# twitu/genome-assembly

Hardware: NVIDIA B200
Metric: canonical k-mers binned+pruned per second (higher is better)
Workload: dtype u64

## Files before the change

### genome-assembly_b200/binding.py

```python
from __future__ import annotations

import ctypes as C
import os
from dataclasses import dataclass

import numpy as np

_HERE = os.path.dirname(os.path.abspath(__file__))
LIB_PATH = os.path.join(_HERE, "libgbin.so")

GBIN_OK = 0
GBIN_E_INVALID_CONFIG = -1
GBIN_E_CUDA = -2
GBIN_E_NOMEM = -3
GBIN_E_NON_ACGT = -4
GBIN_E_STATE = -5
GBIN_E_TOO_LARGE = -6
GBIN_E_INVALID_ARG = -7
GBIN_E_IO = -8


class GbinError(RuntimeError):
    def __init__(self, code: int, msg: str):
        super().__init__(f"gbin error {code}: {msg}")
        self.code = code


class Config(C.Structure):
    _fields_ = [("kmer_size", C.c_int32), ("mmer_size", C.c_int32), ("abundance_cutoff", C.c_int32), ("device", C.c_int32)]


class CTable(C.Structure):
    _fields_ = [("kmer_size", C.c_int32), ("mmer_size", C.c_int32), ("abundance_cutoff", C.c_int32), ("kmer_words", C.c_int32),
                ("on_device", C.c_int32), ("ctx_owned", C.c_int32),
                ("n_instances", C.c_uint64), ("n_distinct", C.c_uint64), ("n_buckets", C.c_uint64), ("n_kmers", C.c_uint64),
                ("n_ids", C.c_uint64),
                ("mmer_codes", C.c_void_p), ("mmer_kmer_off", C.c_void_p), ("kmer_codes", C.c_void_p),
                ("kmer_id_off", C.c_void_p), ("read_ids", C.c_void_p)]


class CExpanded(C.Structure):
    _fields_ = [("kmer_size", C.c_int32), ("on_device", C.c_int32), ("n_lists", C.c_uint64), ("n_ids", C.c_uint64),
                ("list_off", C.c_void_p), ("ids", C.c_void_p)]


class CReads(C.Structure):
    _fields_ = [("data", C.c_void_p), ("data_bytes", C.c_uint64), ("n_reads", C.c_uint64), ("stride", C.c_uint64),
                ("read_len", C.c_uint32), ("id_base", C.c_int32), ("starts", C.c_void_p), ("lens", C.c_void_p),
                ("read_ids", C.c_void_p), ("max_read_len", C.c_uint32), ("reserved", C.c_uint32)]


class Timings(C.Structure):
    _fields_ = [("h2d_ms", C.c_float), ("scan_ms", C.c_float), ("sort_ms", C.c_float), ("group_ms", C.c_float),
                ("d2h_ms", C.c_float), ("total_ms", C.c_float), ("kernel_launches", C.c_uint32), ("sort_passes", C.c_uint32)]

    def as_dict(self):
        return {n: getattr(self, n) for n, _ in self._fields_}


class KernelProfile(C.Structure):
    _fields_ = [("ms", C.c_float * 12), ("launches", C.c_uint32 * 12)]


EXPORTS = [
    "gbin_strerror", "gbin_last_error", "gbin_version", "gbin_create", "gbin_destroy", "gbin_get_config",
    "gbin_bin_reads_host", "gbin_table_clone", "gbin_table_free", "gbin_pinned_alloc", "gbin_pinned_free",
    "gbin_bin_reads_device", "gbin_table_to_host", "gbin_table_to_pinned", "gbin_get_timings", "gbin_record_bytes",
    "gbin_set_kernel_profiling", "gbin_get_kernel_profile", "gbin_kernel_kind_name", "gbin_max_read_len", "gbin_multi_create", "gbin_multi_destroy", "gbin_multi_devices", "gbin_multi_context", "gbin_multi_last_error", "gbin_multi_bin_reads_host", "gbin_table_digest", "gbin_set_pipeline", "gbin_set_tuning", "gbin_donate_scratch", "gbin_get_pipeline_info", "gbin_get_run_stats",
    "gbin_count_instances_device", "gbin_scan_reads_device", "gbin_partition_records_device",
    "gbin_group_records_device", "gbin_owner_of", "gbin_xchg_create", "gbin_xchg_attach", "gbin_xchg_exchange_skr", "gbin_xchg_detach", "gbin_xchg_destroy", "gbin_skr_record_bytes", "gbin_scan_skr_device", "gbin_partition_skr_device", "gbin_group_skr_device",
    "gbin_split_reads_device", "gbin_copy_to_host", "gbin_bin_file_host", "gbin_read_file_fgets", "gbin_table_dump", "gbin_table_dump_reference_format", "gbin_table_dump_expanded_format",
    "gbin_expand_read_ids_device", "gbin_expanded_to_host", "gbin_expanded_free", "gbin_table_dump_expanded_lists",
    "getval", "getbp", "getscore", "process_read", "prune_data", "gbin_ref_configure", "gbin_ref_last_status",
    "gbin_ref_reset", "gbin_table_to_zhash", "gbin_zhash_release",
]

_lib = None


def load_library() -> C.CDLL:
    global _lib
    if _lib is not None:
        return _lib
    if not os.path.exists(LIB_PATH):
        raise ImportError(f"{LIB_PATH} is missing: build it with `make -C genome-assembly_b200` "
                          "(there is no CPU or PyTorch fallback for the binning path)")
    L = C.CDLL(LIB_PATH)
    vp, u64, u32, i32 = C.c_void_p, C.c_uint64, C.c_uint32, C.c_int32
    L.gbin_strerror.restype = C.c_char_p
    L.gbin_strerror.argtypes = [C.c_int]
    L.gbin_last_error.restype = C.c_char_p
    L.gbin_last_error.argtypes = [vp]
    L.gbin_create.argtypes = [C.POINTER(Config), C.POINTER(vp)]
    L.gbin_destroy.argtypes = [vp]
    L.gbin_destroy.restype = None
    L.gbin_get_config.argtypes = [vp, C.POINTER(Config)]
    L.gbin_bin_reads_host.argtypes = [vp, C.POINTER(CReads), C.POINTER(CTable)]
    L.gbin_bin_reads_device.argtypes = [vp, C.POINTER(CReads), vp, C.POINTER(CTable)]
    L.gbin_table_to_host.argtypes = [vp, C.POINTER(CTable), C.POINTER(CTable)]
    L.gbin_table_to_pinned.argtypes = [vp, C.POINTER(CTable), vp, C.POINTER(CTable)]
    L.gbin_table_clone.argtypes = [C.POINTER(CTable), C.POINTER(CTable)]
    L.gbin_table_free.argtypes = [C.POINTER(CTable)]
    L.gbin_table_free.restype = None
    L.gbin_pinned_alloc.argtypes = [C.c_size_t]
    L.gbin_pinned_alloc.restype = vp
    L.gbin_pinned_free.argtypes = [vp]
    L.gbin_pinned_free.restype = None
    L.gbin_get_timings.argtypes = [vp, C.POINTER(Timings)]
    L.gbin_get_run_stats.argtypes = [vp, C.POINTER(u64 * 6)]
    L.gbin_set_pipeline.argtypes = [vp, C.c_int]
    L.gbin_table_digest.argtypes = [vp, C.POINTER(CTable), vp, C.POINTER(u64)]
    L.gbin_set_tuning.argtypes = [vp, C.c_char_p, C.c_int]
    L.gbin_donate_scratch.argtypes = [vp, vp, C.c_uint64]
    L.gbin_get_pipeline_info.argtypes = [vp, C.POINTER(C.c_int), C.POINTER(C.c_int), C.POINTER(C.c_uint32)]
    L.gbin_set_kernel_profiling.argtypes = [vp, C.c_int]
    L.gbin_get_kernel_profile.argtypes = [vp, C.POINTER(KernelProfile)]
    L.gbin_kernel_kind_name.argtypes = [C.c_int]
    L.gbin_kernel_kind_name.restype = C.c_char_p
    L.gbin_record_bytes.argtypes = [vp]
    L.gbin_record_bytes.restype = u32
    L.gbin_max_read_len.restype = u32
    L.gbin_max_read_len.argtypes = []
    L.gbin_count_instances_device.argtypes = [vp, C.POINTER(CReads), vp, C.POINTER(u64)]
    L.gbin_scan_reads_device.argtypes = [vp, C.POINTER(CReads), u32, vp, u64, vp, C.POINTER(u64)]
    L.gbin_partition_records_device.argtypes = [vp, vp, u64, u32, vp, vp, C.POINTER(u64)]
    L.gbin_group_records_device.argtypes = [vp, vp, u64, vp, i32, vp, C.POINTER(CTable)]
    L.gbin_skr_record_bytes.argtypes = [vp]
    L.gbin_skr_record_bytes.restype = u32
    L.gbin_scan_skr_device.argtypes = [vp, C.POINTER(CReads), u32, vp, u64, vp, C.POINTER(u64), C.POINTER(u64)]
    L.gbin_partition_skr_device.argtypes = [vp, vp, u64, u32, vp, vp, C.POINTER(u64)]
    L.gbin_group_skr_device.argtypes = [vp, vp, u64, vp, i32, vp, C.POINTER(CTable), C.POINTER(C.c_int)]
    L.gbin_owner_of.argtypes = [u32, u32]
    L.gbin_owner_of.restype = u32
    L.gbin_xchg_create.argtypes = [vp, u32, u32, u64, vp]
    L.gbin_xchg_attach.argtypes = [vp, vp]
    L.gbin_xchg_exchange_skr.argtypes = [vp, vp, u64, vp, C.POINTER(vp), C.POINTER(u64), C.POINTER(u64)]
    L.gbin_xchg_destroy.argtypes = [vp]
    L.gbin_xchg_destroy.restype = None
    L.gbin_xchg_detach.argtypes = [vp]
    L.gbin_xchg_detach.restype = None
    L.gbin_split_reads_device.argtypes = [vp, vp, u64, C.c_int, vp, C.POINTER(CReads)]
    L.gbin_copy_to_host.argtypes = [vp, vp, vp, u64]
    L.gbin_bin_file_host.argtypes = [vp, C.c_char_p, C.c_int, C.POINTER(CTable)]
    L.gbin_read_file_fgets.argtypes = [C.c_char_p, C.c_int, C.POINTER(vp), C.POINTER(u64), C.POINTER(vp), C.POINTER(vp),
                                       C.POINTER(u64)]
    L.gbin_table_dump.argtypes = [C.POINTER(CTable), C.c_char_p]
    L.gbin_table_dump_reference_format.argtypes = [C.POINTER(CTable), C.c_char_p]
    L.gbin_table_dump_expanded_format.argtypes = [C.POINTER(CTable), C.c_char_p]
    L.gbin_expand_read_ids_device.argtypes = [C.c_void_p, C.POINTER(CTable), C.c_void_p, C.POINTER(CExpanded)]
    L.gbin_expanded_to_host.argtypes = [C.c_void_p, C.POINTER(CExpanded), C.POINTER(CExpanded)]
    L.gbin_expanded_free.argtypes = [C.POINTER(CExpanded)]
    L.gbin_expanded_free.restype = None
    L.gbin_table_dump_expanded_lists.argtypes = [C.POINTER(CTable), C.POINTER(CExpanded), C.c_char_p]
    L.getval.argtypes = [C.c_char]
    L.getval.restype = C.c_int
    L.getbp.argtypes = [C.c_int]
    L.getbp.restype = C.c_char
    L.getscore.argtypes = [C.c_char_p]
    L.getscore.restype = C.c_int
    L.process_read.argtypes = [vp, C.c_char_p, C.c_int]
    L.process_read.restype = vp
    L.prune_data.argtypes = [vp]
    L.prune_data.restype = vp
    L.gbin_ref_configure.argtypes = [C.c_int, C.c_int, C.c_int, C.c_int]
    L.gbin_ref_last_status.restype = C.c_int
    L.gbin_ref_reset.argtypes = [vp]
    L.gbin_ref_reset.restype = None
    L.gbin_table_to_zhash.argtypes = [C.POINTER(CTable), vp]
    L.gbin_zhash_release.argtypes = [vp]
    L.gbin_zhash_release.restype = None
    _lib = L
    return L


@dataclass
class HostTable:
    K: int
    M: int
    cutoff: int
    kw: int
    n_instances: int
    n_distinct: int
    mmer_codes: np.ndarray
    mmer_kmer_off: np.ndarray
    kmer_codes: np.ndarray
    kmer_id_off: np.ndarray
    read_ids: np.ndarray

    @property
    def n_buckets(self):
        return len(self.mmer_codes)

    @property
    def n_kmers(self):
        return len(self.kmer_id_off) - 1

    @property
    def n_ids(self):
        return len(self.read_ids)


def _np_from(ptr, n, dtype):
    if n == 0 or not ptr:
        return np.zeros(0, dtype=dtype)
    buf = (C.c_char * (n * np.dtype(dtype).itemsize)).from_address(ptr)
    return np.frombuffer(buf, dtype=dtype, count=n).copy()


def host_table_from_c(t: CTable) -> HostTable:
    assert not t.on_device
    return HostTable(K=t.kmer_size, M=t.mmer_size, cutoff=t.abundance_cutoff, kw=t.kmer_words,
                     n_instances=int(t.n_instances), n_distinct=int(t.n_distinct),
                     mmer_codes=_np_from(t.mmer_codes, t.n_buckets, np.uint32),
                     mmer_kmer_off=_np_from(t.mmer_kmer_off, t.n_buckets + 1, np.uint64),
                     kmer_codes=_np_from(t.kmer_codes, t.n_kmers * t.kmer_words, np.uint64),
                     kmer_id_off=_np_from(t.kmer_id_off, t.n_kmers + 1, np.uint64),
                     read_ids=_np_from(t.read_ids, t.n_ids, np.int32))


def owner_of(mmer_codes, parts: int) -> np.ndarray:
    m = np.asarray(mmer_codes).astype(np.uint64)
    return ((((m * np.uint64(0x9E3779B1)) & np.uint64(0xFFFFFFFF)) * np.uint64(parts)) >> np.uint64(32)).astype(np.int64)


CUDA_STREAM_LEGACY = 1


def stream_handle(torch_stream) -> int:
    h = int(torch_stream.cuda_stream)
    return h if h else CUDA_STREAM_LEGACY


def _ptr(x):
    if x is None:
        return None
    if isinstance(x, int):
        return x
    if isinstance(x, np.ndarray):
        return x.ctypes.data
    if hasattr(x, "data_ptr"):
        return x.data_ptr()
    raise TypeError(type(x))


class Binner:

    def __init__(self, k: int = 31, m: int = 4, cutoff: int = 1, device: int = 0, pipeline: int | None = None):
        self.lib = load_library()
        self.cfg = Config(k, m, cutoff, device)
        h = C.c_void_p()
        rc = self.lib.gbin_create(C.byref(self.cfg), C.byref(h))
        if rc != GBIN_OK:
            raise GbinError(rc, self.lib.gbin_strerror(rc).decode())
        self.h = h
        self.k, self.m, self.cutoff, self.device = k, m, cutoff, device
        if pipeline is not None:
            self.set_pipeline(pipeline)

    def close(self):
        if getattr(self, "h", None):
            self.lib.gbin_destroy(self.h)
            self.h = None

    def __del__(self):
        try:
            self.close()
        except Exception:
            pass

    def _check(self, rc):
        if rc != GBIN_OK:
            raise GbinError(rc, f"{self.lib.gbin_strerror(rc).decode()}: {self.lib.gbin_last_error(self.h).decode()}")

    @property
    def record_bytes(self) -> int:
        return int(self.lib.gbin_record_bytes(self.h))

    def timings(self) -> dict:
        t = Timings()
        self.lib.gbin_get_timings(self.h, C.byref(t))
        return t.as_dict()

    def set_pipeline(self, pipeline: int):
        self._check(self.lib.gbin_set_pipeline(self.h, pipeline))

    def table_digest(self, table: CTable, stream=None) -> int:
        d = C.c_uint64()
        self._check(self.lib.gbin_table_digest(self.h, C.byref(table), stream, C.byref(d)))
        return int(d.value)

    def expand_read_ids_device(self, dev_table: CTable, stream=None) -> CExpanded:
        x = CExpanded()
        self._check(self.lib.gbin_expand_read_ids_device(self.h, C.byref(dev_table), stream, C.byref(x)))
        return x

    def expanded_to_host(self, dev: CExpanded) -> CExpanded:
        h = CExpanded()
        self._check(self.lib.gbin_expanded_to_host(self.h, C.byref(dev), C.byref(h)))
        return h

    def donate_scratch(self, d_buf, nbytes: int):
        self._check(self.lib.gbin_donate_scratch(self.h, _ptr(d_buf), int(nbytes)))

    def set_tuning(self, name: str, value: int):
        self._check(self.lib.gbin_set_tuning(self.h, name.encode(), int(value)))

    def pipeline_info(self) -> dict:
        a, b, c = C.c_int(), C.c_int(), C.c_uint32()
        self._check(self.lib.gbin_get_pipeline_info(self.h, C.byref(a), C.byref(b), C.byref(c)))
        return {"configured": a.value, "last_used": b.value, "fallbacks": c.value}

    def run_stats(self) -> dict:
        a = (C.c_uint64 * 6)()
        self._check(self.lib.gbin_get_run_stats(self.h, C.byref(a)))
        return {"n_super_kmers": int(a[0]), "n_mmer_runs": int(a[1]), "n_units": int(a[2]), "n_lsd_kmers": int(a[3]),
                "key_nc": int(a[4]) & 0xffffffff, "key_h": int(a[4]) >> 32, "n_passes": int(a[5]) & 0xffffffff}

    def set_kernel_profiling(self, enable: bool):
        self._check(self.lib.gbin_set_kernel_profiling(self.h, int(enable)))

    def kernel_profile(self) -> dict:
        p = KernelProfile()
        self._check(self.lib.gbin_get_kernel_profile(self.h, C.byref(p)))
        out = {}
        for i in range(12):
            name = self.lib.gbin_kernel_kind_name(i).decode()
            if name:
                out[name] = {"ms": float(p.ms[i]), "launches": int(p.launches[i])}
        return out

    @staticmethod
    def _reads(data, data_bytes, n_reads, stride=0, read_len=0, starts=None, lens=None, read_ids=None, id_base=0, max_read_len=0):
        return CReads(_ptr(data), data_bytes, n_reads, stride, read_len, id_base, _ptr(starts), _ptr(lens), _ptr(read_ids),
                      max_read_len, 0)

    def bin_host_raw(self, reads: CReads) -> CTable:
        t = CTable()
        self._check(self.lib.gbin_bin_reads_host(self.h, C.byref(reads), C.byref(t)))
        return t

    def bin_host(self, data, n_reads, *, stride=0, read_len=0, starts=None, lens=None, read_ids=None, id_base=0) -> HostTable:
        if isinstance(data, (bytes, bytearray)):
            data = np.frombuffer(data, dtype=np.uint8)
        data = np.ascontiguousarray(data, dtype=np.uint8)
        keep = [data]
        if starts is not None:
            starts = np.ascontiguousarray(starts, dtype=np.uint64)
            lens = np.ascontiguousarray(lens, dtype=np.uint32)
            keep += [starts, lens]
        if read_ids is not None:
            read_ids = np.ascontiguousarray(read_ids, dtype=np.int32)
            keep.append(read_ids)
        rd = self._reads(data, data.size, n_reads, stride, read_len, starts, lens, read_ids, id_base)
        return host_table_from_c(self.bin_host_raw(rd))

    def bin_device_raw(self, reads: CReads, stream: int | None = None) -> CTable:
        t = CTable()
        self._check(self.lib.gbin_bin_reads_device(self.h, C.byref(reads), stream, C.byref(t)))
        return t

    def table_to_host(self, dev: CTable) -> HostTable:
        h = CTable()
        self._check(self.lib.gbin_table_to_host(self.h, C.byref(dev), C.byref(h)))
        try:
            return host_table_from_c(h)
        finally:
            self.lib.gbin_table_free(C.byref(h))

    def table_to_pinned_raw(self, dev: CTable, stream=None) -> CTable:
        h = CTable()
        self._check(self.lib.gbin_table_to_pinned(self.h, C.byref(dev), stream, C.byref(h)))
        return h

    def split_reads_device(self, d_data, data_bytes: int, read_length_define: int, stream=None) -> CReads:
        rd = CReads()
        self._check(self.lib.gbin_split_reads_device(self.h, _ptr(d_data), data_bytes, read_length_define, stream, C.byref(rd)))
        return rd

    def device_array(self, dev_ptr, n: int, dtype) -> np.ndarray:
        out = np.zeros(n, dtype=dtype)
        if n:
            self._check(self.lib.gbin_copy_to_host(self.h, out.ctypes.data, int(dev_ptr), out.nbytes))
        return out

    def bin_file_host(self, path: str, read_length_define: int) -> HostTable:
        t = CTable()
        self._check(self.lib.gbin_bin_file_host(self.h, path.encode(), read_length_define, C.byref(t)))
        return host_table_from_c(t)

    def count_instances_device(self, reads: CReads, stream=None) -> int:
        n = C.c_uint64()
        self._check(self.lib.gbin_count_instances_device(self.h, C.byref(reads), stream, C.byref(n)))
        return int(n.value)

    def scan_device(self, reads: CReads, arrival_base: int, d_records, capacity: int, stream=None) -> int:
        n = C.c_uint64()
        self._check(self.lib.gbin_scan_reads_device(self.h, C.byref(reads), arrival_base, _ptr(d_records), capacity, stream, C.byref(n)))
        return int(n.value)

    def partition_device(self, d_records, n: int, n_parts: int, d_out, stream=None) -> list[int]:
        counts = (C.c_uint64 * n_parts)()
        self._check(self.lib.gbin_partition_records_device(self.h, _ptr(d_records), n, n_parts, _ptr(d_out), stream, counts))
        return [int(c) for c in counts]

    @property
    def skr_record_bytes(self) -> int:
        return int(self.lib.gbin_skr_record_bytes(self.h))

    def scan_skr_device(self, reads: CReads, arrival_base: int, d_skr, capacity: int, stream=None):
        n, ni = C.c_uint64(), C.c_uint64()
        self._check(self.lib.gbin_scan_skr_device(self.h, C.byref(reads), arrival_base, _ptr(d_skr), capacity, stream, C.byref(n), C.byref(ni)))
        return int(n.value), int(ni.value)

    def partition_skr_device(self, d_skr, n: int, n_parts: int, d_out, stream=None) -> list[int]:
        counts = (C.c_uint64 * n_parts)()
        self._check(self.lib.gbin_partition_skr_device(self.h, _ptr(d_skr), n, n_parts, _ptr(d_out), stream, counts))
        return [int(c) for c in counts]

    def group_skr_device(self, d_skr, n_skr: int, d_ids_by_arrival=None, id_base: int = 0, stream=None) -> CTable:
        t = CTable()
        fb = C.c_int()
        self._check(self.lib.gbin_group_skr_device(self.h, _ptr(d_skr), n_skr, _ptr(d_ids_by_arrival), id_base, stream, C.byref(t), C.byref(fb)))
        return t

    XCHG_HANDLE_BYTES = 192

    def xchg_create(self, rank: int, world: int, capacity_records: int) -> bytes:
        buf = C.create_string_buffer(self.XCHG_HANDLE_BYTES)
        self._check(self.lib.gbin_xchg_create(self.h, rank, world, capacity_records, buf))
        return buf.raw

    def xchg_attach(self, all_handles: bytes):
        self._check(self.lib.gbin_xchg_attach(self.h, C.c_char_p(all_handles)))

    def xchg_exchange_skr(self, d_skr, n: int, world: int, stream=None):
        recv, n_in = C.c_void_p(), C.c_uint64()
        sent = (C.c_uint64 * 16)()
        self._check(self.lib.gbin_xchg_exchange_skr(self.h, _ptr(d_skr), n, stream, C.byref(recv), C.byref(n_in), sent))
        return int(recv.value or 0), int(n_in.value), [int(sent[i]) for i in range(world)]

    def xchg_detach(self):
        self.lib.gbin_xchg_detach(self.h)

    def xchg_destroy(self):
        self.lib.gbin_xchg_destroy(self.h)

    def group_device(self, d_records, n: int, d_ids_by_arrival=None, id_base: int = 0, stream=None) -> CTable:
        t = CTable()
        self._check(self.lib.gbin_group_records_device(self.h, _ptr(d_records), n, _ptr(d_ids_by_arrival), id_base, stream, C.byref(t)))
        return t


def read_file_fgets(path: str, read_length_define: int):
    L = load_library()
    data, starts, lens = C.c_void_p(), C.c_void_p(), C.c_void_p()
    nbytes, n = C.c_uint64(), C.c_uint64()
    rc = L.gbin_read_file_fgets(path.encode(), read_length_define, C.byref(data), C.byref(nbytes), C.byref(starts), C.byref(lens),
                                C.byref(n))
    if rc != GBIN_OK:
        raise GbinError(rc, L.gbin_strerror(rc).decode())
    libc = C.CDLL(None)
    libc.free.argtypes = [C.c_void_p]
    try:
        return (_np_from(data.value, nbytes.value, np.uint8), _np_from(starts.value, n.value, np.uint64),
                _np_from(lens.value, n.value, np.uint32))
    finally:
        for p in (data, starts, lens):
            libc.free(p)
```

### genome-assembly_b200/csrc/bin3.cu

```cuda
#include "bin3.cuh"
#include "gbin_device.cuh"
#include "gbin_internal.h"
#include "prefix_scan.cuh"

namespace gbin {


__device__ __forceinline__ uint32_t payload_bases(const uint32_t *pl, uint32_t nwords, uint32_t j, uint32_t h, bool rev) {
    const uint32_t bit = 2 * j, wi = bit >> 5, sh = bit & 31;
    const uint32_t a = wi < nwords ? pl[wi] : 0u, b = wi + 1 < nwords ? pl[wi + 1] : 0u;
    uint32_t x = __funnelshift_l(b, a, sh);
    if (rev) x = ~x;
    return h ? (x >> (32 - 2 * h)) : 0u;
}

template <int PW>
__global__ void __launch_bounds__(256)
    make_entries_kernel(const uint32_t *__restrict__ skr, uint64_t n_rec, KeyLayout kl, uint64_t *__restrict__ ent, uint16_t *__restrict__ piece_info,
                        unsigned long long *__restrict__ n_real) {
    constexpr int NW = SkrLayout<PW>::WORDS;
    const uint64_t i = (uint64_t)blockIdx.x * blockDim.x + threadIdx.x;
    uint32_t real = 0;
    if (i < n_rec) {
        const uint4 h = *reinterpret_cast<const uint4 *>(skr + i * NW);
// ... 43 lines not shown
    else make_entries_kernel<4><<<grid, 256, 0, st>>>(static_cast<const uint32_t *>(skr), n_rec, kl, ent, piece_info, n_real_dev);
    return 1;
}


struct EntCountAndHead {
    const uint64_t *ent;
    const uint16_t *info;
    __device__ __forceinline__ uint64_t operator()(uint64_t i) const {
        const uint64_t e = ent[i];
        const uint64_t head = (i == 0 || (e >> 32) != (ent[i - 1] >> 32)) ? 1ull : 0ull;
        return (uint64_t)(info[i] & 0xffu) | (head << 32);
    }
};

struct EntRunSink {
    const uint64_t *ent;
    uint32_t *inst_prefix, *run_start;
    __device__ __forceinline__ void operator()(uint64_t i, uint64_t b) const {
        inst_prefix[i] = (uint32_t)b;
        if (i == 0 || (ent[i] >> 32) != (ent[i - 1] >> 32)) run_start[b >> 32] = (uint32_t)i;
    }
};

__global__ void v3_run_totals_kernel(const uint64_t *__restrict__ total, uint64_t n, uint32_t *__restrict__ inst_prefix, uint32_t *__restrict__ run_start,
                                     uint32_t *__restrict__ n_inst_out, uint32_t *__restrict__ n_runs_out) {
    const uint64_t t = *total;
    inst_prefix[n] = (uint32_t)t;
    run_start[t >> 32] = (uint32_t)n;
    *n_inst_out = (uint32_t)t;
    *n_runs_out = (uint32_t)(t >> 32);
}

int v3_plan_runs(const uint64_t *ent, const uint16_t *sorted_info, uint64_t n_ent, uint32_t *inst_prefix, uint64_t *both64, uint32_t *run_start,
                 uint64_t *scratch64, uint32_t *n_inst_dev, uint32_t *n_runs_dev, cudaStream_t st) {
    if (n_ent == 0) {
        cudaMemsetAsync(n_inst_dev, 0, 4, st);
        cudaMemsetAsync(n_runs_dev, 0, 4, st);
        return 0;
    }
    int l = exclusive_scan_to<uint64_t, EntCountAndHead, EntRunSink>(EntCountAndHead{ent, sorted_info}, EntRunSink{ent, inst_prefix, run_start}, n_ent, scratch64,
                                                                     both64, st);
    v3_run_totals_kernel<<<1, 1, 0, st>>>(both64, n_ent, inst_prefix, run_start, n_inst_dev, n_runs_dev);
    return l + 1;
}

constexpr int PLAN_BLOCK = 64;
struct Plan3 {
    uint32_t cap, nb_max, ecap, max_rounds;
    uint32_t cap_s, nb_s, ecap_s;
};
struct RunView3 {
    const uint32_t *run_start;
    const uint32_t *inst_prefix;
    __device__ __forceinline__ uint32_t size(uint64_t r) const { return inst_prefix[run_start[r + 1]] - inst_prefix[run_start[r]]; }
};
__host__ __device__ inline uint32_t rounds_of(uint32_t c, const Plan3 &pp) {
    uint32_t r = 2 * ((c + pp.cap - 1) / pp.cap) + 1;
    return r < pp.max_rounds ? r : pp.max_rounds;
}

__global__ void v3_atoms_kernel(RunView3 rv, const uint64_t *__restrict__ ent, uint64_t n_runs, int mshift, uint32_t *__restrict__ atom_c,
                                uint32_t *__restrict__ atom_e, uint32_t *__restrict__ atom_mm) {
    const uint64_t r = (uint64_t)blockIdx.x * blockDim.x + threadIdx.x;
    if (r >= n_runs) return;
    const uint32_t a = rv.run_start[r], b = rv.run_start[r + 1];
    atom_c[r] = rv.inst_prefix[b] - rv.inst_prefix[a];
    atom_e[r] = b - a;
    atom_mm[r] = (uint32_t)(ent[a] >> 32) >> mshift;
}

constexpr uint64_t ATOM_ROUNDS = 1ull << 32;
constexpr uint32_t SPAN_MEMBER = 0xfffffffeu;
constexpr uint32_t SPAN_MEMBER_LONG = 0xffffffffu;
constexpr uint32_t SPAN_SHORT_MAX = 17;
__global__ void __launch_bounds__(128)
    v3_pack_kernel(const uint32_t *__restrict__ atom_c, const uint32_t *__restrict__ atom_e, const uint32_t *__restrict__ atom_mm, uint64_t n_runs, Plan3 pp,
                   uint64_t *__restrict__ nunits, uint32_t *__restrict__ spanlen) {
    const uint64_t t = (uint64_t)blockIdx.x * blockDim.x + threadIdx.x;
    uint64_t r = t * PLAN_BLOCK;
    const uint64_t stop = r + PLAN_BLOCK < n_runs ? r + PLAN_BLOCK : n_runs;
    if (r >= n_runs) return;
    if (r > 0)
        while (r < n_runs && atom_mm[r] == atom_mm[r - 1]) r++;
    uint32_t cur_c = 0, cur_e = 0, cur_b = 0;
    while (r < stop) {
        const uint32_t mm = atom_mm[r];
        uint64_t q = r;
        uint64_t cb = 0, eb = 0;
        do {
            cb += atom_c[q];
            eb += atom_e[q];
            q++;
        } while (q < n_runs && atom_mm[q] == mm);
        if (cb <= pp.cap && eb <= pp.ecap) {
            if (cb > pp.cap_s || eb > pp.ecap_s) {
                nunits[r] = 1ull;
                cur_b = 0;
            } else if (cur_b == 0 || cur_c + cb > pp.cap_s || cur_e + eb > pp.ecap_s || cur_b + 1 > pp.nb_s) {
                nunits[r] = 1ull;
                cur_c = (uint32_t)cb;
                cur_e = (uint32_t)eb;
                cur_b = 1;
            } else {
                nunits[r] = 0ull;
                cur_c += (uint32_t)cb;
                cur_e += (uint32_t)eb;
                cur_b++;
            }
            spanlen[r] = 0;
            for (uint64_t a = r + 1; a < q; a++) {
                nunits[a] = 0ull;
                spanlen[a] = 0;
            }
        } else {
            cur_b = 0;
            uint32_t L = 0, sc = 0, se = 0;
            bool open = false;
            for (uint64_t a = r; a < q; a++) {
                const uint32_t c = atom_c[a], e = atom_e[a];
                if (c > pp.cap) {
                    const uint32_t R = rounds_of(c, pp);
                    nunits[a] = (uint64_t)R | ATOM_ROUNDS;
                    L += R;
                    open = false;
                } else if (!open || sc + c > pp.cap || se + e > pp.ecap) {
                    nunits[a] = 1ull;
                    L++;
                    sc = c;
                    se = e;
                    open = true;
                } else {
                    nunits[a] = 0ull;
                    sc += c;
                    se += e;
                }
                spanlen[a] = SPAN_MEMBER;
            }
            spanlen[r] = L;
            if (L > SPAN_SHORT_MAX)
                for (uint64_t a = r + 1; a < q; a++) spanlen[a] = SPAN_MEMBER_LONG;
        }
        r = q;
    }
}

struct G3Counters {
    unsigned long long distinct;
    unsigned long long total_kmers, total_ids;
    unsigned int overflow;
    unsigned int n_units, n_spans;
    unsigned int pad;
    unsigned long long lsd_kmers, lsd_ids;
};

__global__ void v3_head_runs_kernel(const uint64_t *__restrict__ nunits, const uint64_t *__restrict__ base, uint64_t n_runs, uint32_t *__restrict__ head_run) {
    const uint64_t r = (uint64_t)blockIdx.x * blockDim.x + threadIdx.x;
    if (r >= n_runs) return;
    const uint32_t nu = (uint32_t)nunits[r];
    const uint32_t ub = (uint32_t)base[r];
    for (uint32_t j = 0; j < nu; j++) head_run[ub + j] = (uint32_t)r;
}

__global__ void v3_fill_units_kernel(RunView3 rv, const uint64_t *__restrict__ nunits, const uint32_t *__restrict__ spanlen, const uint64_t *__restrict__ base,
                                     const uint64_t *__restrict__ totals, uint64_t n_runs, const uint32_t *__restrict__ head_run, Unit3 *__restrict__ units,
                                     G3Counters *__restrict__ gc) {
    const uint32_t n_units = (uint32_t)*totals;
    const uint32_t u = blockIdx.x * blockDim.x + threadIdx.x;
    if (u == 0) {
        gc->n_units = n_units;
        gc->n_spans = (uint32_t)(*totals >> 32);
    }
    if (u >= n_units) return;
    const uint32_t r0 = head_run[u];
    const uint64_t nu = nunits[r0];
    const uint32_t ub = (uint32_t)base[r0];
    Unit3 un;
    un.drange = 0u | (63u << 8);
    un.ent_begin = rv.run_start[r0];
    un.ibase = rv.inst_prefix[un.ent_begin];
    if (nu & ATOM_ROUNDS) {
        un.ent_end = rv.run_start[r0 + 1];
        un.n_inst = rv.inst_prefix[un.ent_end] - un.ibase;
        un.round = u - ub;
        un.rounds = (uint32_t)nu;
    } else {
        const uint32_t r1 = (u + 1 < n_units) ? head_run[u + 1] : (uint32_t)n_runs;
        un.ent_end = rv.run_start[r1];
        un.n_inst = rv.inst_prefix[un.ent_end] - un.ibase;
        un.round = 0;
        un.rounds = 0;
    }
    const uint32_t sl = spanlen[r0];
    if (sl == 0 || sl == SPAN_MEMBER || sl == SPAN_MEMBER_LONG) un.span_len = sl;
    else un.span_len = u == ub ? sl : (sl > SPAN_SHORT_MAX ? SPAN_MEMBER_LONG : SPAN_MEMBER);
    units[u] = un;
}

__global__ void __launch_bounds__(128)
    v3_round_cuts_kernel(const uint16_t *__restrict__ info, Unit3 *__restrict__ units, G3Counters *__restrict__ gc, uint32_t cap) {
    __shared__ int s_hist[4][68];
    const uint32_t lane = threadIdx.x & 31, warp = threadIdx.x >> 5;
    int *dhist = s_hist[warp];
    const uint32_t n_units = gc->n_units;
    for (uint32_t u = blockIdx.x * 4 + warp; u < n_units; u += gridDim.x * 4) {
        const Unit3 un = units[u];
        if (un.rounds == 0 || un.round != 0) continue;
        dhist[lane] = 0;
        dhist[lane + 32] = 0;
        if (lane < 4) dhist[64 + lane] = 0;
        __syncwarp();
        const uint32_t n_ent = un.ent_end - un.ent_begin;
        for (uint32_t e = lane; e < n_ent; e += 32) {
            const uint32_t pi = info[un.ent_begin + e];
            const uint32_t np = pi & 0xffu, dlo = pi >> 8;
            if (np) {
                atomicAdd(&dhist[dlo], 1);
                atomicAdd(&dhist[dlo + np], -1);
            }
        }
        __syncwarp();
        const int a = dhist[2 * lane], b = dhist[2 * lane + 1];
        int incl = a + b;
#pragma unroll
        for (int d = 1; d < 32; d <<= 1) {
            const int o = __shfl_up_sync(0xffffffffu, incl, d);
            if (lane >= (uint32_t)d) incl += o;
        }
        __syncwarp();
        dhist[2 * lane] = incl - b;
        dhist[2 * lane + 1] = incl;
        __syncwarp();
        if (lane == 0) {
            uint32_t rnd = 0, acc = 0, before = 0;
            int lo = 0;
            bool bad = false;
            auto emit = [&](int hi) {
                if (rnd < un.rounds) {
                    Unit3 &w = units[u + rnd];
                    w.drange = (uint32_t)lo | ((uint32_t)hi << 8);
                    w.ibase = un.ibase + before;
                    w.n_inst = acc;
                } else {
                    bad = true;
                }
            };
            for (int d = 0; d < 64; d++) {
                const uint32_t c = (uint32_t)dhist[d];
                if (c > cap) bad = true;
                if (acc + c > cap) {
                    emit(d - 1);
                    rnd++;
                    lo = d;
                    before += acc;
                    acc = 0;
                }
                acc += c;
            }
            emit(63);
            for (uint32_t j = rnd + 1; j < un.rounds; j++) {
                units[u + j].n_inst = 0;
                units[u + j].ibase = un.ibase + un.n_inst;
            }
            if (bad) atomicExch(&gc->overflow, 1u);
        }
        __syncwarp();
    }
}


struct UnitOut3 {
    uint32_t ibase;
    uint32_t S, N;
    uint32_t pad;
};

struct G3Stage {
    uint64_t *codes;
    uint32_t *mmer;
    uint32_t *loff;
    int32_t *ids;
    UnitOut3 *unit_out;
    uint64_t kmer_cap, id_cap;
    uint32_t kdiv;
};

template <int PW>
struct Payload {
    uint64_t w[PW];
    __device__ __forceinline__ void set(const uint4 &a, const uint4 &b) {
        w[0] = ((uint64_t)a.x << 32) | a.y;
        w[1] = ((uint64_t)a.z << 32) | a.w;
        if (PW == 4) {
            w[PW - 2] = ((uint64_t)b.x << 32) | b.y;
            w[PW - 1] = ((uint64_t)b.z << 32) | b.w;
        }
    }
    __device__ __forceinline__ void advance(uint32_t bases) {
        const uint32_t sh = 2 * bases;
#pragma unroll
        for (int q = 0; q < PW - 1; q++) w[q] = (w[q] << sh) | (w[q + 1] >> (64 - sh));
        w[PW - 1] <<= sh;
    }
    __device__ __forceinline__ void skip(uint32_t bases) {
        while (bases >= 31) {
            advance(31);
// ... 312 lines not shown
            for (int j = 0; j < U; j++) {
                const uint32_t p = b0 + j * 32 + lane;
                const bool sv = leader[j] && (cutoff < 0 || c[j] > (uint32_t)cutoff);
                const unsigned lm = __ballot_sync(0xffffffffu, leader[j]), sm = __ballot_sync(0xffffffffu, sv);
                if (sv) surv[S + __popc(sm & lt_mask)] = (uint16_t)p;
                else if (leader[j]) cnt16[p] = 0xffffu;
                S += __popc(sm);
                D += __popc(lm);
                N += sv ? c[j] : 0u;
            }
        }
#pragma unroll
        for (int d = 16; d > 0; d >>= 1) N += __shfl_xor_sync(0xffffffffu, N, d);
        const uint64_t kbase = ibase / out.kdiv;
        const bool oob = (uint64_t)ibase + N > out.id_cap || kbase + S > out.kmer_cap;
        if (lane == 0) {
            out.unit_out[u_cur] = UnitOut3{ibase, oob ? 0u : S, oob ? 0u : N, 0u};
            atomicAdd(&gc->distinct, (unsigned long long)D);
            if (oob) atomicExch(&gc->overflow, 2u);
        }
        __syncwarp();
        if (oob) {
            u = __shfl_sync(0xffffffffu, u_next, 0);
            continue;
        }

        for (uint32_t x0 = 0; x0 < S; x0 += 32) {
            const uint32_t x = x0 + lane;
            if (x < S) {
                const uint32_t p = surv[x];
                uint32_t a = 0, a2 = S;
                if (n_bkt > 1) {
                    const uint32_t o = ebk[eix[p]];
                    const uint32_t blo = bstart[o], bhi = bstart[o + 1];
                    uint32_t b = S;
                    while (a < b) {
                        const uint32_t m = (a + b) >> 1;
                        if (surv[m] < blo) a = m + 1;
                        else b = m;
                    }
                    uint32_t b2 = S;
                    a2 = a;
                    while (a2 < b2) {
                        const uint32_t m = (a2 + b2) >> 1;
                        if (surv[m] < bhi) a2 = m + 1;
                        else b2 = m;
                    }
                }
                const uint64_t k0 = key0[p], k1 = (KW == 2) ? key1[p] : 0ull;
                uint32_t rank = a;
                for (uint32_t t = a; t < a2; t++) {
                    const uint32_t q = surv[t];
                    const uint64_t q0 = key0[q];
                    bool less = q0 < k0;
                    if constexpr (KW == 2) less = less || (q0 == k0 && key1[q] < k1);
                    rank += less ? 1u : 0u;
                }
                sorted[rank] = (uint16_t)p;
            }
        }
        __syncwarp();

        {
            uint32_t carry = 0;
            for (uint32_t x0 = 0; x0 < S; x0 += 32) {
                const uint32_t x = x0 + lane;
                const uint32_t p = x < S ? sorted[x] : 0u;
                const uint32_t c = x < S ? cnt16[p] : 0u;
                const uint32_t inc = warp_incl_scan_u32(c, lane);
                if (x < S) cnt16[p] = (uint16_t)(carry + inc);
                carry += __shfl_sync(0xffffffffu, inc, 31);
            }
        }
        __syncwarp();

        for (uint32_t x0 = 0; x0 < S; x0 += 32) {
            const uint32_t x = x0 + lane;
            if (x < S) {
                const uint32_t p = sorted[x];
                const uint32_t beg = x ? cnt16[sorted[x - 1]] : 0u;
                const uint64_t g = kbase + x;
                out.codes[g * KW] = key0[p];
                if (KW == 2) out.codes[g * KW + 1] = key1[p];
                out.mmer[g] = bmm[n_bkt > 1 ? ebk[eix[p]] : 0u];
                out.loff[g] = beg;
            }
        }
        __syncwarp();

        if (N) {
            if (packed) {
                for (uint32_t b0 = 0; b0 < n_inst; b0 += 32 * U) {
                    uint32_t end[U], r[U];
                    int32_t id[U];
#pragma unroll
                    for (int j = 0; j < U; j++) {
                        const uint32_t p = b0 + j * 32 + lane;
                        end[j] = 0xffffu;
                        r[j] = 0;
                        id[j] = 0;
                        if (p < n_inst) {
                            end[j] = cnt16[grp[p]];
                            r[j] = rk[p];
                            id[j] = eid[eix[p]];
                        }
                    }
#pragma unroll
                    for (int j = 0; j < U; j++)
                        if (end[j] != 0xffffu) idbuf[end[j] - 1u - r[j]] = id[j];
                }
            } else {
                uint32_t carry_pos = 0;
                for (uint32_t e0 = 0; e0 < n_ent; e0 += 32) {
                    const uint32_t e = e0 + lane;
                    uint32_t np = 0, arrival = 0;
                    if (e < n_ent) {
                        const uint32_t slot = (uint32_t)ent[un.ent_begin + e];
                        const uint32_t *rec = skr + (uint64_t)(slot >> kl.cshift) * NW;
                        const uint32_t meta = rec[2];
                        arrival = rec[0];
                        uint32_t t0;
                        piece_of(meta, slot & cls_mask, kl, &t0, &np);
                        if (is_round && np) {
                            const int so = (int)((meta >> 16) & 0xffu);
                            int a = so - dhi, b = so - dlo;
                            if (a < (int)t0) a = (int)t0;
                            if (b > (int)(t0 + np - 1)) b = (int)(t0 + np - 1);
                            np = (dlo > dhi || b < a) ? 0u : (uint32_t)(b - a + 1);
                        }
                    }
                    const uint32_t ps = warp_incl_scan_u32(np, lane);
                    const uint32_t pos0 = carry_pos + ps - np;
                    carry_pos += __shfl_sync(0xffffffffu, ps, 31);
                    if (np) {
                        const int32_t id = ids_by_arrival ? ids_by_arrival[arrival] : id_base + (int32_t)arrival;
                        for (uint32_t i = 0; i < np; i++) {
                            const uint32_t p = pos0 + i;
                            const uint32_t end = cnt16[grp[p]];
                            if (end != 0xffffu) idbuf[end - 1u - rk[p]] = id;
                        }
                    }
                }
            }
            __syncwarp();
            int32_t *dst = out.ids + ibase;
            for (uint32_t i = lane; i < N; i += 32) dst[i] = idbuf[i];
        }
        __syncwarp();
        u = __shfl_sync(0xffffffffu, u_next, 0);
    }
}


struct UnitSN {
    const UnitOut3 *uo;
    const uint32_t *chunk_bounds;
    uint32_t chunk;
    __device__ __forceinline__ uint64_t operator()(uint64_t u) const {
        if (u < chunk_bounds[chunk] || u >= chunk_bounds[chunk + 1]) return 0ull;
        return ((uint64_t)uo[u].S << 32) | uo[u].N;
    }
};

__global__ void v3_chunk_total_kernel(const uint64_t *__restrict__ chunk_sum, uint32_t chunk, unsigned long long *__restrict__ totals, G3Counters *__restrict__ gc,
                                      uint32_t n_chunks, int which) {
    const unsigned long long t = (chunk ? totals[chunk - 1] : 0ull) + *chunk_sum;
    totals[chunk] = t;
    if (chunk + 1 == n_chunks) {
        if (which == 0) {
            gc->total_kmers = t >> 32;
            gc->total_ids = t & 0xffffffffull;
        } else {
            gc->lsd_kmers = t >> 32;
            gc->lsd_ids = t & 0xffffffffull;
        }
    }
}

struct G3Final {
    uint64_t *kmer_codes;
    uint32_t *kmer_mmer;
    uint64_t *kmer_id_off;
    int32_t *read_ids;
    uint64_t id_off_base;
};

struct G3Lsd {
    const uint64_t *excl;
    void *rec;
    uint32_t *src_off;
    uint32_t *cnt;
    uint32_t *fidx;
    uint32_t *nadj;
    uint64_t cap;
};

struct UnitSNLong {
    const UnitOut3 *uo;
    const Unit3 *units;
    const uint32_t *chunk_bounds;
    uint32_t chunk;
    __device__ __forceinline__ uint64_t operator()(uint64_t u) const {
        if (u < chunk_bounds[chunk] || u >= chunk_bounds[chunk + 1]) return 0ull;
        const uint32_t sl = units[u].span_len;
        if (sl != SPAN_MEMBER_LONG && (sl <= SPAN_SHORT_MAX || sl == SPAN_MEMBER)) return 0ull;
        return ((uint64_t)uo[u].S << 32) | uo[u].N;
    }
};

template <int KW>
__device__ __forceinline__ void finalize3_unit(const Unit3 *__restrict__ units, const uint64_t *__restrict__ unit_excl, unsigned long long base,
                                               unsigned long long lsd_base, const G3Stage &st, const G3Final &fin, const G3Lsd &ls, G3Counters *gc, uint32_t u,
                                               uint32_t lane, bool only_long) {
    const uint32_t span_len = units[u].span_len;
    if (only_long && span_len != SPAN_MEMBER_LONG && (span_len <= SPAN_SHORT_MAX || span_len == SPAN_MEMBER)) return;
    const uint64_t ex = unit_excl[u];
    const UnitOut3 uo = st.unit_out[u];
    const uint64_t Sb = (base >> 32) + (ex >> 32), Nb = (base & 0xffffffffull) + (ex & 0xffffffffull);
    if (span_len == 0) {
        const uint64_t kb = uo.ibase / st.kdiv;
        for (uint32_t x0 = 0; x0 < uo.S; x0 += 128) {
            uint64_t c0[4], c1[4];
            uint32_t mm[4], lo[4];
#pragma unroll
            for (int q = 0; q < 4; q++) {
                const uint32_t x = x0 + q * 32 + lane;
                if (x < uo.S) {
                    c0[q] = st.codes[(kb + x) * KW];
                    if (KW == 2) c1[q] = st.codes[(kb + x) * KW + 1];
                    mm[q] = st.mmer[kb + x];
                    lo[q] = st.loff[kb + x];
                }
            }
#pragma unroll
            for (int q = 0; q < 4; q++) {
                const uint32_t x = x0 + q * 32 + lane;
                if (x < uo.S) {
                    fin.kmer_codes[(Sb + x) * KW] = c0[q];
                    if (KW == 2) fin.kmer_codes[(Sb + x) * KW + 1] = c1[q];
                    fin.kmer_mmer[Sb + x] = mm[q];
                    fin.kmer_id_off[Sb + x] = fin.id_off_base + Nb + lo[q];
                }
            }
        }
        const int32_t *src = st.ids + uo.ibase;
        int32_t *dst = fin.read_ids + Nb;
        for (uint32_t i0 = 0; i0 < uo.N; i0 += 256) {
            int32_t v[8];
#pragma unroll
            for (int q = 0; q < 8; q++) {
                const uint32_t i = i0 + q * 32 + lane;
                if (i < uo.N) v[q] = __ldcs(src + i);
            }
#pragma unroll
            for (int q = 0; q < 8; q++) {
                const uint32_t i = i0 + q * 32 + lane;
                if (i < uo.N) dst[i] = v[q];
            }
        }
        return;
    }
    if (span_len == SPAN_MEMBER_LONG || (span_len > SPAN_SHORT_MAX && span_len != SPAN_MEMBER)) {
        const uint64_t lx = ls.excl[u];
        const uint64_t q0 = (lsd_base >> 32) + (lx >> 32), nq0 = (lsd_base & 0xffffffffull) + (lx & 0xffffffffull);
        if (q0 + uo.S > ls.cap) {
            if (lane == 0) atomicExch(&gc->overflow, 6u);
            return;
        }
        const uint64_t kb = uo.ibase / st.kdiv;
        Rec<KW> *rec = static_cast<Rec<KW> *>(ls.rec);
        for (uint32_t x = lane; x < uo.S; x += 32) {
            const uint64_t p = q0 + x;
            Rec<KW> r;
            r.k[0] = st.codes[(kb + x) * KW];
            if (KW == 2) r.k[KW - 1] = st.codes[(kb + x) * KW + 1];
            r.mmer = st.mmer[kb + x];
            r.arrival = (uint32_t)p;
            store_rec<KW>(rec + p, r);
            const uint32_t lo = st.loff[kb + x];
            ls.src_off[p] = uo.ibase + lo;
            ls.cnt[p] = (x + 1 < uo.S ? st.loff[kb + x + 1] : uo.N) - lo;
            ls.fidx[p] = (uint32_t)(Sb + x);
            ls.nadj[p] = (uint32_t)(Nb - nq0);
        }
        return;
    }
    uint32_t h = u;
    while (units[h].span_len == SPAN_MEMBER) h--;
    const uint32_t R = units[h].span_len;
    const uint64_t exh = unit_excl[h];
    const uint64_t Sh = (base >> 32) + (exh >> 32), Nh = (base & 0xffffffffull) + (exh & 0xffffffffull);
    if (uo.S == 0) return;
    const uint32_t j = u - h;
    const uint64_t kbj = uo.ibase / st.kdiv;
    const uint32_t mmer = st.mmer[kbj];
    for (uint32_t x0 = 0; x0 < uo.S; x0 += 32) {
        const uint32_t x = x0 + lane;
        uint32_t lo = 0, cnt = 0;
        uint64_t idoff = 0;
        if (x < uo.S) {
            const uint64_t k0 = st.codes[(kbj + x) * KW], k1 = KW == 2 ? st.codes[(kbj + x) * KW + 1] : 0ull;
            lo = st.loff[kbj + x];
            cnt = (x + 1 < uo.S ? st.loff[kbj + x + 1] : uo.N) - lo;
            uint32_t rank = x;
            idoff = lo;
            for (uint32_t j2 = 0; j2 < R; j2++) {
                if (j2 == j) continue;
                const UnitOut3 u2 = st.unit_out[h + j2];
                const uint64_t kb2 = u2.ibase / st.kdiv;
                uint32_t a = 0, b = u2.S;
                while (a < b) {
                    const uint32_t m = (a + b) >> 1;
                    const uint64_t q0 = st.codes[(kb2 + m) * KW];
                    bool less = q0 < k0;
                    if constexpr (KW == 2) less = less || (q0 == k0 && st.codes[(kb2 + m) * KW + 1] < k1);
                    if (less) a = m + 1;
                    else b = m;
                }
                rank += a;
                idoff += a < u2.S ? st.loff[kb2 + a] : u2.N;
            }
            fin.kmer_codes[(Sh + rank) * KW] = k0;
            if (KW == 2) fin.kmer_codes[(Sh + rank) * KW + 1] = k1;
            fin.kmer_mmer[Sh + rank] = mmer;
            fin.kmer_id_off[Sh + rank] = fin.id_off_base + Nh + idoff;
        }
        const uint32_t nl = min(32u, uo.S - x0);
        for (uint32_t l0 = 0; l0 < nl; l0 += 4) {
            const uint32_t l = l0 + (lane >> 3);
            const uint32_t c = __shfl_sync(0xffffffffu, cnt, l & 31);
            const uint32_t so = __shfl_sync(0xffffffffu, lo, l & 31);
            const uint64_t d = __shfl_sync(0xffffffffu, idoff, l & 31);
            if (l < nl) {
                const int32_t *src = st.ids + uo.ibase + so;
                int32_t *dst = fin.read_ids + Nh + d;
                for (uint32_t i = lane & 7u; i < c; i += 8) dst[i] = src[i];
            }
        }
    }
}

template <int KW>
__global__ void __launch_bounds__(128, 12)
    finalize3_kernel(const Unit3 *__restrict__ units, const uint64_t *__restrict__ unit_excl, const unsigned long long *__restrict__ totals,
                     const unsigned long long *__restrict__ lsd_totals, G3Stage st, G3Final fin, G3Lsd ls, G3Counters *__restrict__ gc,
                     const uint32_t *__restrict__ chunk_bounds, uint32_t chunk, bool only_long) {
    const uint32_t lane = threadIdx.x & 31;
    const uint32_t unit_begin = chunk_bounds[chunk], unit_end = chunk_bounds[chunk + 1];
    const unsigned long long base = chunk ? totals[chunk - 1] : 0ull;
    const unsigned long long lsd_base = chunk ? lsd_totals[chunk - 1] : 0ull;
    for (uint32_t u = unit_begin + blockIdx.x * 4 + (threadIdx.x >> 5); u < unit_end; u += gridDim.x * 4)
        finalize3_unit<KW>(units, unit_excl, base, lsd_base, st, fin, ls, gc, u, lane, only_long);
}

template <int KW>
struct LsdCnt {
    const Rec<KW> *rec;
    const uint32_t *cnt;
    __device__ __forceinline__ uint64_t operator()(uint64_t q) const { return cnt[rec[q].arrival]; }
};

template <int KW>
__global__ void lsd_place_kernel(const Rec<KW> *__restrict__ rec, uint64_t n, const uint64_t *__restrict__ dnew, G3Lsd ls, G3Final fin) {
    const uint64_t q = (uint64_t)blockIdx.x * blockDim.x + threadIdx.x;
    if (q >= n) return;
    const Rec<KW> r = load_rec<KW>(rec + q);
    const uint64_t f = ls.fidx[q];
    fin.kmer_codes[f * KW] = r.k[0];
    if (KW == 2) fin.kmer_codes[f * KW + 1] = r.k[KW - 1];
    fin.kmer_mmer[f] = r.mmer;
    fin.kmer_id_off[f] = fin.id_off_base + dnew[q] + ls.nadj[q];
}

template <int KW>
__global__ void __launch_bounds__(256)
    lsd_lists_kernel(const Rec<KW> *__restrict__ rec, uint64_t n, const uint64_t *__restrict__ dnew, G3Lsd ls, const int32_t *__restrict__ stg_ids, G3Final fin) {
    const uint64_t q = ((uint64_t)blockIdx.x * blockDim.x + threadIdx.x) >> 3;
    if (q >= n) return;
    const uint32_t p = rec[q].arrival;
    const uint32_t c = ls.cnt[p];
    const int32_t *src = stg_ids + ls.src_off[p];
    int32_t *dst = fin.read_ids + dnew[q] + ls.nadj[q];
    for (uint32_t i = threadIdx.x & 7u; i < c; i += 8) dst[i] = src[i];
}

__global__ void v3_chunk_bounds_kernel(const Unit3 *__restrict__ units, const G3Counters *__restrict__ gc, uint32_t n_chunks, uint32_t *__restrict__ chunk_bounds) {
    const uint32_t nu = gc->n_units;
    for (uint32_t c = 0; c <= n_chunks; c++) {
        uint32_t b = (uint32_t)(((uint64_t)nu * c) / n_chunks);
        if (c == n_chunks) b = nu;
        else {
            while (b > 0 && b < nu && (units[b].span_len == SPAN_MEMBER || units[b].span_len == SPAN_MEMBER_LONG)) b--;
        }
        chunk_bounds[c] = b;
    }
}


static bool v3_hybrid(const KeyLayout &kl, int cap_i) {
    static int on = -1;
    if (on < 0) {
        const char *e = getenv("GBIN_V3_HYBRID");
        on = e ? atoi(e) : 1;
    }
    return on && cap_i != 512 && kl.K <= 32;
}
static Plan3 v3_plan_params(const KeyLayout &kl, int cap_i) {
    const uint32_t cap = cap_i == 512 ? 512u : 1024u;
    Plan3 pp{cap, cap / 8, cap / 4, (uint32_t)(kl.K - kl.M + 1), cap, cap / 8, cap / 4};
    if (v3_hybrid(kl, cap_i)) {
        pp.cap_s = G3_SMALL_INST;
        pp.nb_s = G3_SMALL_NB;
        pp.ecap_s = G3_SMALL_ENT;
    }
    return pp;
}

uint64_t v3_max_units(uint64_t n_inst, uint64_t n_runs, int cap) {
    const uint64_t c = cap == 512 ? 512 : 1024;
    return n_runs + 5 * (n_inst / c) + 16;
}
size_t v3_unit_bytes() { return sizeof(Unit3); }
size_t v3_unit_out_bytes() { return sizeof(UnitOut3); }

struct PtrIn64 {
    const uint64_t *p;
    __device__ __forceinline__ uint64_t operator()(uint64_t j) const { return p[j]; }
};

int v3_plan_units(const uint16_t *sorted_info, const uint64_t *ent, const KeyLayout &kl, int cap, const uint32_t *inst_prefix, const uint32_t *run_start, uint64_t n_runs,
                  uint64_t *nunits64, uint64_t *base64, uint32_t *atom3, uint32_t *spanlen, uint32_t *head_run, void *scratch, void *units, uint64_t max_units,
                  void *gc_dev, uint32_t n_chunks, uint32_t *chunk_bounds, cudaStream_t st) {
    RunView3 rv{run_start, inst_prefix};
    const Plan3 pp = v3_plan_params(kl, cap);
    G3Counters *gc = static_cast<G3Counters *>(gc_dev);
    cudaMemsetAsync(gc, 0, sizeof(G3Counters), st);
    int l = 0;
    if (n_runs) {
        uint32_t *atom_c = atom3, *atom_e = atom3 + n_runs, *atom_mm = atom3 + 2 * n_runs;
        v3_atoms_kernel<<<(unsigned)((n_runs + 255) / 256), 256, 0, st>>>(rv, ent, n_runs, kl.mshift, atom_c, atom_e, atom_mm);
        const uint64_t walkers = (n_runs + PLAN_BLOCK - 1) / PLAN_BLOCK;
        v3_pack_kernel<<<(unsigned)((walkers + 127) / 128), 128, 0, st>>>(atom_c, atom_e, atom_mm, n_runs, pp, nunits64, spanlen);
        l += 2 + exclusive_scan<uint64_t, PtrIn64>(PtrIn64{nunits64}, base64, n_runs, static_cast<uint64_t *>(scratch), base64 + n_runs, st);
        v3_head_runs_kernel<<<(unsigned)((n_runs + 255) / 256), 256, 0, st>>>(nunits64, base64, n_runs, head_run);
        v3_fill_units_kernel<<<(unsigned)((max_units + 255) / 256), 256, 0, st>>>(rv, nunits64, spanlen, base64, base64 + n_runs, n_runs, head_run, static_cast<Unit3 *>(units), gc);
        v3_round_cuts_kernel<<<592, 128, 0, st>>>(sorted_info, static_cast<Unit3 *>(units), gc, pp.cap);
        l += 3;
    }
    v3_chunk_bounds_kernel<<<1, 1, 0, st>>>(static_cast<const Unit3 *>(units), gc, n_chunks, chunk_bounds);
    return l + 1;
}

size_t v3_group_smem_bytes(int KW, int cap) {
    const size_t per_warp = cap == 512 ? (KW == 1 ? WarpLayout<512, 1>::BYTES : WarpLayout<512, 2>::BYTES)
                                       : (KW == 1 ? WarpLayout<1024, 1>::BYTES : WarpLayout<1024, 2>::BYTES);
    return per_warp * G3_WARPS;
}

int v3_group_launch(const void *skr, const uint64_t *ent, const void *units, const KeyLayout &kl, int cap, int cutoff, const int32_t *ids_by_arrival, int32_t id_base,
                    const V3Out &o, uint64_t max_units, uint64_t *unit_excl, uint64_t *lsd_excl, void *scan_scratch, void *gc_dev, const V3Chunks &ch, const V3Lsd &lsd,
                    bool finalize_only, int sm_count, KernelProf *prof, cudaStream_t st) {
    const int KW = kl.K <= 32 ? 1 : 2;
    constexpr int WARPS = G3_WARPS;
    const size_t smem = v3_group_smem_bytes(KW, cap);
    cudaMemsetAsync(ch.tickets, 0, sizeof(uint32_t) * 2 * ch.n, st);
    const uint32_t kdiv = cutoff >= 0 ? (uint32_t)cutoff + 1u : 1u;
    G3Stage stg{o.stg_codes, o.stg_mmer, o.stg_loff, o.stg_ids, static_cast<UnitOut3 *>(o.unit_out), o.kmer_cap, o.id_cap, kdiv};
    G3Final fin{o.kmer_codes, o.kmer_mmer, o.kmer_id_off, o.read_ids, o.id_off_base};
    G3Lsd ls{lsd_excl, lsd.rec, lsd.src_off, lsd.cnt, lsd.fidx, lsd.nadj, lsd.cap};
    G3Counters *gc = static_cast<G3Counters *>(gc_dev);
    const uint32_t *sk = static_cast<const uint32_t *>(skr);
    const Unit3 *un = static_cast<const Unit3 *>(units);
    int per_sm = (int)((size_t)(227 * 1024) / (smem + 1024));
    if (per_sm < 1) per_sm = 1;
    const bool hybrid = v3_hybrid(kl, cap);
    const size_t smem_s = v3_group_smem_bytes(KW, 512);
    int per_sm_s = (int)((size_t)(227 * 1024) / (smem_s + 1024));
    if (per_sm_s < 1) per_sm_s = 1;
    int launches = 0;
    static int sbs = -1, l_per_sm = 2;
    if (sbs < 0) {
        const char *e = getenv("GBIN_V3_SBS");
        sbs = e ? atoi(e) : 1;
        const char *f = getenv("GBIN_V3_LPS");
        l_per_sm = f ? atoi(f) : 2;
        if (l_per_sm < 1 || l_per_sm > 2) l_per_sm = 2;
    }
    const bool side_by_side = sbs && ch.aux && ch.ev_fork && ch.ev_join;
    auto launch = [&](auto kern, auto kern_small, auto fin_kern) {
        cudaFuncSetAttribute(kern, cudaFuncAttributeMaxDynamicSharedMemorySize, (int)smem);
        if (hybrid) cudaFuncSetAttribute(kern_small, cudaFuncAttributeMaxDynamicSharedMemorySize, (int)smem_s);
        for (uint32_t c = 0; c < ch.n; c++) {
            if (!finalize_only) {
                bool on = prof && prof->begin(KK_SKR_GROUP, st);
                if (!hybrid) {
                    kern<<<sm_count * per_sm, WARPS * 32, smem, st>>>(sk, ent, un, kl, cutoff, ids_by_arrival, id_base, stg, gc, ch.bounds, c, ch.tickets, 0u);
                } else if (!side_by_side) {
                    kern<<<sm_count * per_sm, WARPS * 32, smem, st>>>(sk, ent, un, kl, cutoff, ids_by_arrival, id_base, stg, gc, ch.bounds, c, ch.tickets, 2u);
                    kern_small<<<sm_count * per_sm_s, WARPS * 32, smem_s, st>>>(sk, ent, un, kl, cutoff, ids_by_arrival, id_base, stg, gc, ch.bounds, c, ch.tickets + ch.n, 1u);
                } else {
                    cudaEventRecord(ch.ev_fork, st);
                    cudaStreamWaitEvent(ch.aux, ch.ev_fork, 0);
                    kern<<<sm_count * l_per_sm, WARPS * 32, smem, st>>>(sk, ent, un, kl, cutoff, ids_by_arrival, id_base, stg, gc, ch.bounds, c, ch.tickets, 2u);
                    kern_small<<<sm_count * per_sm_s, WARPS * 32, smem_s, ch.aux>>>(sk, ent, un, kl, cutoff, ids_by_arrival, id_base, stg, gc, ch.bounds, c, ch.tickets + ch.n, 1u);
                    cudaEventRecord(ch.ev_join, ch.aux);
                    cudaStreamWaitEvent(st, ch.ev_join, 0);
                }
                if (prof) prof->end(on, hybrid ? 2 : 1, st);
                launches += hybrid ? 2 : 1;
            }
            bool on = prof && prof->begin(KK_V3_SPAN, st);
            int l = exclusive_scan<uint64_t, UnitSN>(UnitSN{stg.unit_out, ch.bounds, c}, unit_excl, max_units, static_cast<uint64_t *>(scan_scratch), ch.chunk_sum, st);
            v3_chunk_total_kernel<<<1, 1, 0, st>>>(ch.chunk_sum, c, ch.totals_dev, gc, ch.n, 0);
            l += exclusive_scan<uint64_t, UnitSNLong>(UnitSNLong{stg.unit_out, un, ch.bounds, c}, lsd_excl, max_units, static_cast<uint64_t *>(scan_scratch), ch.chunk_sum, st);
            v3_chunk_total_kernel<<<1, 1, 0, st>>>(ch.chunk_sum, c, ch.lsd_totals_dev, gc, ch.n, 1);
            fin_kern<<<sm_count * 12, 128, 0, st>>>(un, unit_excl, ch.totals_dev, ch.lsd_totals_dev, stg, fin, ls, gc, ch.bounds, c, finalize_only);
            if (prof) prof->end(on, l + 3, st);
            launches += l + 3;
            if (ch.totals_host) {
                cudaMemcpyAsync(ch.totals_host + c, ch.totals_dev + c, sizeof(unsigned long long), cudaMemcpyDeviceToHost, st);
                cudaMemcpyAsync(ch.lsd_totals_host + c, ch.lsd_totals_dev + c, sizeof(unsigned long long), cudaMemcpyDeviceToHost, st);
            }
            if (ch.done) cudaEventRecord(ch.done[c], st);
        }
    };
    static int uu = 0;
    if (!uu) {
        const char *e = getenv("GBIN_V3_U");
        uu = e ? atoi(e) : 0;
        if (uu != 1 && uu != 2 && uu != 4) uu = -1;
    }
    const int u_sel = uu > 0 ? uu : (cap == 512 ? 2 : 4);
#define G3_LAUNCH(PW_, KW_, CAP_) \
    (u_sel == 1 ? launch(group3_kernel<PW_, KW_, CAP_, WARPS, 1>, group3_kernel<PW_, KW_, 512, WARPS, 2>, finalize3_kernel<KW_>) \
             : (u_sel == 2 ? launch(group3_kernel<PW_, KW_, CAP_, WARPS, 2>, group3_kernel<PW_, KW_, 512, WARPS, 2>, finalize3_kernel<KW_>) \
                           : launch(group3_kernel<PW_, KW_, CAP_, WARPS, 4>, group3_kernel<PW_, KW_, 512, WARPS, 2>, finalize3_kernel<KW_>)))
    if (KW == 1) {
        if (cap == 512) G3_LAUNCH(2, 1, 512);
        else G3_LAUNCH(2, 1, 1024);
    } else {
        if (cap == 512) G3_LAUNCH(4, 2, 512);
        else G3_LAUNCH(4, 2, 1024);
    }
#undef G3_LAUNCH
    return launches;
}

template <int KW>
struct RecHead {
    const Rec<KW> *rec;
    __device__ __forceinline__ uint32_t operator()(uint64_t p) const { return (p == 0 || rec[p].mmer != rec[p - 1].mmer) ? 1u : 0u; }
};
template <int KW>
__global__ void span_starts_kernel(const Rec<KW> *__restrict__ rec, uint64_t n, const uint32_t *__restrict__ idx, uint32_t *__restrict__ starts,
                                   uint32_t *__restrict__ n_spans, uint32_t *__restrict__ flag) {
    const uint64_t p = (uint64_t)blockIdx.x * blockDim.x + threadIdx.x;
    if (p >= n) return;
    const bool head = p == 0 || rec[p].mmer != rec[p - 1].mmer;
    if (head) starts[idx[p]] = (uint32_t)p;
    if (p == n - 1) {
        const uint32_t total = idx[p] + (head ? 1u : 0u);
        starts[total] = (uint32_t)n;
        *n_spans = total;
        *flag = 0u;
    }
}

constexpr int SS_RMAX = 1024;
template <int KW, int CAP, int THREADS>
__global__ void __launch_bounds__(THREADS)
    span_sort_kernel(Rec<KW> *__restrict__ rec, const uint32_t *__restrict__ starts, const uint32_t *__restrict__ n_spans_ptr, uint32_t m_min, uint32_t m_max,
                     uint32_t *__restrict__ too_big) {
    extern __shared__ __align__(16) uint8_t ss_smem[];
    uint64_t *ka = reinterpret_cast<uint64_t *>(ss_smem);
    uint64_t *kb = ka + KW * CAP;
    uint16_t *sa = reinterpret_cast<uint16_t *>(kb + KW * CAP);
    uint16_t *sb = sa + CAP;
    uint16_t *ra = sb + CAP;
    uint16_t *rb = ra + SS_RMAX + 2;
    __shared__ uint32_t s_nruns;
    const uint32_t tid = threadIdx.x, lane = tid & 31;
    const uint32_t n_spans = *n_spans_ptr;
    for (uint32_t s = blockIdx.x; s < n_spans; s += gridDim.x) {
        const uint32_t b = starts[s], m = starts[s + 1] - b;
        if (m < m_min) continue;
        if (m > m_max) continue;
        const uint32_t mmer = rec[b].mmer;
        for (uint32_t i = tid; i < m; i += THREADS) {
            const Rec<KW> r = load_rec<KW>(rec + b + i);
            ka[i] = r.k[0];
            if (KW == 2) ka[CAP + i] = r.k[KW - 1];
            sa[i] = (uint16_t)i;
        }
        __syncthreads();
        if (tid < 32) {
            uint32_t nr = 0;
            for (uint32_t i0 = 0; i0 < m; i0 += 32) {
                const uint32_t i = i0 + lane;
                bool head = false;
                if (i < m) {
                    head = i == 0 || ka[i] < ka[i - 1];
                    if (KW == 2 && i && ka[i] == ka[i - 1]) head = ka[CAP + i] < ka[CAP + i - 1];
                }
                const unsigned bal = __ballot_sync(0xffffffffu, head);
                if (head) {
                    const uint32_t pos = nr + __popc(bal & ((1u << lane) - 1u));
                    if (pos < (uint32_t)SS_RMAX) ra[pos] = (uint16_t)i;
                }
                nr += __popc(bal);
            }
            if (lane == 0) {
                s_nruns = nr;
                if (nr <= (uint32_t)SS_RMAX) ra[nr] = (uint16_t)m;
            }
        }
        __syncthreads();
        uint32_t nr = s_nruns;
        if (nr > (uint32_t)SS_RMAX) {
            if (tid == 0) atomicExch(too_big, 1u);
            __syncthreads();
            continue;
        }
        uint64_t *src_k = ka, *dst_k = kb;
        uint16_t *src_s = sa, *dst_s = sb, *src_r = ra, *dst_r = rb;
        while (nr > 1) {
            for (uint32_t i = tid; i < m; i += THREADS) {
                uint32_t lo = 0, hi = nr;
                while (hi - lo > 1) {
                    const uint32_t mid = (lo + hi) >> 1;
                    if (src_r[mid] <= i) lo = mid;
                    else hi = mid;
                }
                const uint32_t a = lo, sib = a ^ 1u;
                const uint32_t pair0 = src_r[a & ~1u];
                uint32_t place;
                if (sib >= nr) {
                    place = i;
                } else {
                    const uint64_t k0 = src_k[i], k1 = KW == 2 ? src_k[CAP + i] : 0ull;
                    uint32_t l = src_r[sib], h = src_r[sib + 1];
                    const uint32_t sib0 = l;
                    while (l < h) {
                        const uint32_t mid = (l + h) >> 1;
                        const uint64_t q0 = src_k[mid];
                        bool less = q0 < k0;
                        if constexpr (KW == 2) less = less || (q0 == k0 && src_k[CAP + mid] < k1);
                        if (less) l = mid + 1;
                        else h = mid;
                    }
                    place = pair0 + (i - src_r[a]) + (l - sib0);
                }
                dst_k[place] = src_k[i];
                if (KW == 2) dst_k[CAP + place] = src_k[CAP + i];
                dst_s[place] = src_s[i];
            }
            const uint32_t nr2 = (nr + 1) >> 1;
            for (uint32_t a = tid; a <= nr2; a += THREADS) dst_r[a] = a < nr2 ? src_r[2 * a] : (uint16_t)m;
            __syncthreads();
            uint64_t *tk = src_k;
            src_k = dst_k;
            dst_k = tk;
            uint16_t *ts = src_s;
            src_s = dst_s;
            dst_s = ts;
            uint16_t *tr = src_r;
            src_r = dst_r;
            dst_r = tr;
            nr = nr2;
        }
        if (s_nruns > 1) {
            for (uint32_t i = tid; i < m; i += THREADS) {
                Rec<KW> r;
                r.k[0] = src_k[i];
                if (KW == 2) r.k[KW - 1] = src_k[CAP + i];
                r.mmer = mmer;
                r.arrival = b + src_s[i];
                store_rec<KW>(rec + b + i, r);
            }
        }
        __syncthreads();
    }
}

constexpr int SS_RMAX_G = 8192;
template <int KW>
__device__ __forceinline__ bool rec_less(const Rec<KW> *a, uint64_t k0, uint64_t k1) {
    const uint64_t q0 = __ldcg(reinterpret_cast<const unsigned long long *>(&a->k[0]));
    if (KW == 1) return q0 < k0;
    if (q0 != k0) return q0 < k0;
    return __ldcg(reinterpret_cast<const unsigned long long *>(&a->k[KW - 1])) < k1;
}
template <int KW>
__global__ void __launch_bounds__(1024)
    span_sort_global_kernel(Rec<KW> *__restrict__ rec, Rec<KW> *__restrict__ rec2, const uint32_t *__restrict__ starts, const uint32_t *__restrict__ n_spans_ptr,
                            uint32_t m_min, uint32_t *__restrict__ too_big) {
    extern __shared__ __align__(16) uint8_t ssg_smem[];
    uint32_t *ra = reinterpret_cast<uint32_t *>(ssg_smem);
    uint32_t *rb = ra + SS_RMAX_G + 2;
    __shared__ uint32_t s_cnt[33];
    const uint32_t tid = threadIdx.x, lane = tid & 31, warp = tid >> 5;
    const uint32_t n_spans = *n_spans_ptr;
    for (uint32_t s = blockIdx.x; s < n_spans; s += gridDim.x) {
        const uint32_t b = starts[s], m = starts[s + 1] - b;
        if (m < m_min) continue;
        const uint32_t per = (m + 31) / 32, c0 = warp * per, c1 = min(m, c0 + per);
        auto is_head = [&](uint32_t i) {
            if (i == 0) return true;
            const Rec<KW> *pr = rec + b + i - 1;
            const uint64_t k0 = __ldcg(reinterpret_cast<const unsigned long long *>(&rec[b + i].k[0]));
            const uint64_t k1 = KW == 2 ? __ldcg(reinterpret_cast<const unsigned long long *>(&rec[b + i].k[KW - 1])) : 0ull;
            return !rec_less<KW>(pr, k0, k1);
        };
        uint32_t cnt = 0;
        for (uint32_t i0 = c0; i0 < c1; i0 += 32) {
            const uint32_t i = i0 + lane;
            cnt += __popc(__ballot_sync(0xffffffffu, i < c1 && is_head(i)));
        }
        if (lane == 0) s_cnt[warp] = cnt;
        __syncthreads();
        if (tid == 0) {
            uint32_t acc = 0;
            for (int w = 0; w < 32; w++) {
                const uint32_t c = s_cnt[w];
                s_cnt[w] = acc;
                acc += c;
            }
            s_cnt[32] = acc;
        }
        __syncthreads();
        uint32_t nr = s_cnt[32];
        if (nr > (uint32_t)SS_RMAX_G) {
            if (tid == 0) atomicExch(too_big, 1u);
            __syncthreads();
            continue;
        }
        {
            uint32_t at = s_cnt[warp];
            for (uint32_t i0 = c0; i0 < c1; i0 += 32) {
                const uint32_t i = i0 + lane;
                const bool head = i < c1 && is_head(i);
                const unsigned bal = __ballot_sync(0xffffffffu, head);
                if (head) ra[at + __popc(bal & ((1u << lane) - 1u))] = i;
                at += __popc(bal);
            }
            if (tid == 0) ra[nr] = m;
        }
        __syncthreads();
        Rec<KW> *src = rec + b, *dst = rec2 + b;
        uint32_t *src_r = ra, *dst_r = rb;
        const uint32_t nr0 = nr;
        while (nr > 1) {
            for (uint32_t i = tid; i < m; i += 1024) {
                uint32_t lo = 0, hi = nr;
                while (hi - lo > 1) {
                    const uint32_t mid = (lo + hi) >> 1;
                    if (src_r[mid] <= i) lo = mid;
                    else hi = mid;
                }
                const uint32_t a = lo, sib = a ^ 1u;
                Rec<KW> r;
                r.k[0] = __ldcg(reinterpret_cast<const unsigned long long *>(&src[i].k[0]));
                if (KW == 2) r.k[KW - 1] = __ldcg(reinterpret_cast<const unsigned long long *>(&src[i].k[KW - 1]));
                r.mmer = __ldcg(&src[i].mmer);
                r.arrival = __ldcg(&src[i].arrival);
                uint32_t place = i;
                if (sib < nr) {
                    uint32_t l = src_r[sib], h = src_r[sib + 1];
                    const uint32_t sib0 = l;
                    while (l < h) {
                        const uint32_t mid = (l + h) >> 1;
                        if (rec_less<KW>(src + mid, r.k[0], KW == 2 ? r.k[KW - 1] : 0ull)) l = mid + 1;
                        else h = mid;
                    }
                    place = src_r[a & ~1u] + (i - src_r[a]) + (l - sib0);
                }
                dst[place] = r;
            }
            const uint32_t nr2 = (nr + 1) >> 1;
            for (uint32_t a = tid; a <= nr2; a += 1024) dst_r[a] = a < nr2 ? src_r[2 * a] : m;
            __threadfence();
            __syncthreads();
            Rec<KW> *t = src;
            src = dst;
            dst = t;
            uint32_t *tr = src_r;
            src_r = dst_r;
            dst_r = tr;
            nr = nr2;
        }
        if (nr0 > 1 && src != rec + b) {
            for (uint32_t i = tid; i < m; i += 1024) {
                Rec<KW> r;
                r.k[0] = __ldcg(reinterpret_cast<const unsigned long long *>(&src[i].k[0]));
                if (KW == 2) r.k[KW - 1] = __ldcg(reinterpret_cast<const unsigned long long *>(&src[i].k[KW - 1]));
                r.mmer = __ldcg(&src[i].mmer);
                r.arrival = __ldcg(&src[i].arrival);
                rec[b + i] = r;
            }
        }
        __threadfence();
        __syncthreads();
    }
}

constexpr int SS_CAP_SMALL = 2048, SS_CAP_BIG = 8192;
template <int KW, int CAP>
constexpr size_t ss_smem_bytes() {
    return (size_t)2 * KW * CAP * 8 + (size_t)2 * CAP * 2 + (size_t)2 * (SS_RMAX + 2) * 2;
}

template <int KW>
static int v3_span_sort(void *rec_v, void *rec2_v, uint64_t n, uint32_t *work32, void *scan_scratch, int sm_count, cudaStream_t st) {
    Rec<KW> *rec = static_cast<Rec<KW> *>(rec_v);
    uint32_t *idx = work32, *starts = work32 + n, *n_spans = work32 + 2 * n + 2, *flag = work32 + 2 * n + 3;
    int l = exclusive_scan<uint32_t, RecHead<KW>>(RecHead<KW>{rec}, idx, n, static_cast<uint32_t *>(scan_scratch), nullptr, st);
    span_starts_kernel<KW><<<(unsigned)((n + 255) / 256), 256, 0, st>>>(rec, n, idx, starts, n_spans, flag);
    constexpr int CS = SS_CAP_SMALL / KW, CB = SS_CAP_BIG / KW;
    constexpr size_t smem_s = ss_smem_bytes<KW, CS>(), smem_b = ss_smem_bytes<KW, CB>();
    cudaFuncSetAttribute(span_sort_kernel<KW, CS, 256>, cudaFuncAttributeMaxDynamicSharedMemorySize, (int)smem_s);
    cudaFuncSetAttribute(span_sort_kernel<KW, CB, 1024>, cudaFuncAttributeMaxDynamicSharedMemorySize, (int)smem_b);
    const int per_sm = (int)((size_t)(227 * 1024) / (smem_s + 1024));
    span_sort_kernel<KW, CS, 256><<<sm_count * (per_sm < 1 ? 1 : per_sm), 256, smem_s, st>>>(rec, starts, n_spans, 2u, (uint32_t)CS, flag);
    span_sort_kernel<KW, CB, 1024><<<sm_count, 1024, smem_b, st>>>(rec, starts, n_spans, (uint32_t)CS + 1u, (uint32_t)CB, flag);
    constexpr size_t smem_g = (size_t)2 * (SS_RMAX_G + 2) * 4;
    cudaFuncSetAttribute(span_sort_global_kernel<KW>, cudaFuncAttributeMaxDynamicSharedMemorySize, (int)smem_g);
    span_sort_global_kernel<KW><<<sm_count * 2, 1024, smem_g, st>>>(rec, static_cast<Rec<KW> *>(rec2_v), starts, n_spans, (uint32_t)CB + 1u, flag);
    return l + 4;
}

int v3_lsd_finish(const KeyLayout &kl, uint64_t n, void *rec_a, void *rec_b, void *radix_scratch, uint64_t *dnew, void *scan_scratch, const V3Out &o, const V3Lsd &lsd,
                  int sm_count, KernelProf *prof, cudaStream_t st) {
    if (n == 0) return 0;
    const int KW = kl.K <= 32 ? 1 : 2;
    bool in_b = false;
    int passes = 0;
    int l = 0;
    static int span_sort_on = -1;
    if (span_sort_on < 0) {
        const char *e = getenv("GBIN_V3_SPAN_SORT");
        span_sort_on = e ? atoi(e) : 1;
    }
    bool need_global = true;
    if (span_sort_on && n < (1ull << 31)) {
        uint32_t *work32 = reinterpret_cast<uint32_t *>(dnew);
        bool on = prof && prof->begin(KK_V3_SPAN, st);
        const int ls_ = KW == 1 ? v3_span_sort<1>(rec_a, rec_b, n, work32, scan_scratch, sm_count, st) : v3_span_sort<2>(rec_a, rec_b, n, work32, scan_scratch, sm_count, st);
        if (prof) prof->end(on, ls_, st);
        l += ls_;
        uint32_t flag = 1;
        cudaMemcpyAsync(&flag, work32 + 2 * n + 3, sizeof flag, cudaMemcpyDeviceToHost, st);
        if (cudaStreamSynchronize(st) == cudaSuccess) need_global = flag != 0;
    }
    if (need_global) l += radix_sort_records(rec_a, rec_b, n, KW, kl.K, kl.M, radix_scratch, &in_b, &passes, prof, st);
    const void *sorted = in_b ? rec_b : rec_a;
    G3Final fin{o.kmer_codes, o.kmer_mmer, o.kmer_id_off, o.read_ids, o.id_off_base};
    G3Lsd ls{nullptr, nullptr, lsd.src_off, lsd.cnt, lsd.fidx, lsd.nadj, lsd.cap};
    bool on = prof && prof->begin(KK_V3_SPAN, st);
    int l2 = 0;
    if (KW == 1) {
        const Rec<1> *r = static_cast<const Rec<1> *>(sorted);
        l2 += exclusive_scan<uint64_t, LsdCnt<1>>(LsdCnt<1>{r, lsd.cnt}, dnew, n, static_cast<uint64_t *>(scan_scratch), nullptr, st);
        lsd_place_kernel<1><<<(unsigned)((n + 255) / 256), 256, 0, st>>>(r, n, dnew, ls, fin);
        lsd_lists_kernel<1><<<(unsigned)((n * 8 + 255) / 256), 256, 0, st>>>(r, n, dnew, ls, o.stg_ids, fin);
    } else {
        const Rec<2> *r = static_cast<const Rec<2> *>(sorted);
        l2 += exclusive_scan<uint64_t, LsdCnt<2>>(LsdCnt<2>{r, lsd.cnt}, dnew, n, static_cast<uint64_t *>(scan_scratch), nullptr, st);
        lsd_place_kernel<2><<<(unsigned)((n + 255) / 256), 256, 0, st>>>(r, n, dnew, ls, fin);
        lsd_lists_kernel<2><<<(unsigned)((n * 8 + 255) / 256), 256, 0, st>>>(r, n, dnew, ls, o.stg_ids, fin);
    }
    if (prof) prof->end(on, l2 + 2, st);
    return l + l2 + 2;
}

constexpr uint32_t PASS_TILE = 1u << 16;
__global__ void pass_tile_sums_kernel(const uint16_t *__restrict__ info, uint64_t n_ent, unsigned long long *__restrict__ sums) {
    const uint64_t base = (uint64_t)blockIdx.x * PASS_TILE;
    unsigned long long acc = 0;
    for (uint64_t i = base + threadIdx.x; i < base + PASS_TILE && i < n_ent; i += blockDim.x) acc += info[i] & 0xffu;
#pragma unroll
    for (int d = 16; d > 0; d >>= 1) acc += __shfl_xor_sync(0xffffffffu, acc, d);
    __shared__ unsigned long long s[8];
    if ((threadIdx.x & 31) == 0) s[threadIdx.x >> 5] = acc;
    __syncthreads();
    if (threadIdx.x == 0) {
        unsigned long long t = 0;
        for (int w = 0; w < (int)(blockDim.x >> 5); w++) t += s[w];
        sums[blockIdx.x] = t;
    }
}
__global__ void pass_bounds_kernel(const uint64_t *__restrict__ ent, uint64_t n_ent, int mshift, unsigned long long *__restrict__ bounds, uint32_t n_bounds) {
    const uint32_t i = blockIdx.x * blockDim.x + threadIdx.x;
    if (i >= n_bounds) return;
    unsigned long long b = bounds[i];
    if (b == 0 || b >= n_ent) return;
    const uint32_t mm = (uint32_t)(ent[b - 1] >> 32) >> mshift;
    while (b < n_ent && ((uint32_t)(ent[b] >> 32) >> mshift) == mm) b++;
    bounds[i] = b;
}
uint32_t v3_pass_tiles(uint64_t n_ent) { return (uint32_t)((n_ent + PASS_TILE - 1) / PASS_TILE); }
uint32_t v3_pass_tile_entries() { return PASS_TILE; }
int v3_pass_tile_sums(const uint16_t *sorted_info, uint64_t n_ent, unsigned long long *sums_dev, cudaStream_t st) {
    if (n_ent == 0) return 0;
    pass_tile_sums_kernel<<<v3_pass_tiles(n_ent), 256, 0, st>>>(sorted_info, n_ent, sums_dev);
    return 1;
}
int v3_pass_bounds(const uint64_t *ent, uint64_t n_ent, int mshift, unsigned long long *bounds_dev, uint32_t n_bounds, cudaStream_t st) {
    if (n_bounds == 0) return 0;
    pass_bounds_kernel<<<(n_bounds + 63) / 64, 64, 0, st>>>(ent, n_ent, mshift, bounds_dev, n_bounds);
    return 1;
}

__global__ void mmer_bitmap_kernel(const uint32_t *__restrict__ skr, int skr_words, uint64_t n_rec, uint32_t *__restrict__ bitmap) {
    const uint64_t i = (uint64_t)blockIdx.x * blockDim.x + threadIdx.x;
    if (i >= n_rec) return;
    const uint32_t mm = skr[i * skr_words + 1];
    const uint32_t bit = 1u << (mm & 31u);
    if (!(bitmap[mm >> 5] & bit)) atomicOr(&bitmap[mm >> 5], bit);
}
__global__ void bitmap_count_kernel(const uint32_t *__restrict__ bitmap, uint64_t words, unsigned long long *__restrict__ count) {
    uint32_t c = 0;
    for (uint64_t i = (uint64_t)blockIdx.x * blockDim.x + threadIdx.x; i < words; i += (uint64_t)gridDim.x * blockDim.x) c += __popc(bitmap[i]);
#pragma unroll
    for (int d = 16; d > 0; d >>= 1) c += __shfl_xor_sync(0xffffffffu, c, d);
    if ((threadIdx.x & 31) == 0 && c) atomicAdd(count, (unsigned long long)c);
}
size_t v3_mmer_bitmap_bytes(int M) { return ((size_t)1 << (2 * M)) / 8 + 64; }
int v3_count_mmers(const void *skr, int skr_words, uint64_t n_rec, int M, uint32_t *bitmap, unsigned long long *count_dev, cudaStream_t st) {
    const uint64_t words = ((uint64_t)1 << (2 * M)) / 32;
    cudaMemsetAsync(bitmap, 0, words * 4, st);
    cudaMemsetAsync(count_dev, 0, sizeof(unsigned long long), st);
    if (n_rec == 0) return 0;
    mmer_bitmap_kernel<<<(unsigned)((n_rec + 255) / 256), 256, 0, st>>>(static_cast<const uint32_t *>(skr), skr_words, n_rec, bitmap);
    bitmap_count_kernel<<<592, 256, 0, st>>>(bitmap, words, count_dev);
    return 2;
}

}
```

### genome-assembly_b200/csrc/capi.cu

```cuda
#include <cstdarg>
#include <cstdio>
#include <cstdlib>
#include <cstring>
#include <condition_variable>
#include <mutex>
#include <new>
#include <string>
#include <thread>
#include <vector>

#include "../../include/gbin.h"
#include "gbin_internal.h"
#include "prefix_scan.cuh"

using namespace gbin;

namespace {

struct DevBuf {
    void *p = nullptr;
    size_t cap = 0;
    DevBuf() = default;
    DevBuf(const DevBuf &) = delete;
    DevBuf &operator=(const DevBuf &) = delete;
    ~DevBuf() { release(); }
    cudaError_t ensure(size_t bytes) {
        if (bytes <= cap) return cudaSuccess;
        if (p) cudaFree(p);
        p = nullptr;
        cap = 0;
        size_t want = bytes + bytes / 16 + 256;
        cudaError_t e = cudaMalloc(&p, want);
        if (e != cudaSuccess) {
            (void)cudaGetLastError();
            e = cudaMalloc(&p, bytes);
            want = bytes;
        }
        if (e == cudaSuccess) cap = want;
        return e;
    }
    cudaError_t ensure_keep(size_t bytes, size_t keep, cudaStream_t st) {
        if (bytes <= cap) return cudaSuccess;
        if (!p || keep == 0) return ensure(bytes);
        void *q = nullptr;
        const size_t want = bytes + bytes / 16 + 256;
        cudaError_t e = cudaMalloc(&q, want);
        if (e != cudaSuccess) return e;
        e = cudaMemcpyAsync(q, p, keep, cudaMemcpyDeviceToDevice, st);
        if (e == cudaSuccess) e = cudaStreamSynchronize(st);
        cudaFree(p);
        p = q;
        cap = want;
        return e;
    }
    void release() {
        if (p) cudaFree(p);
        p = nullptr;
        cap = 0;
    }
    template <typename T>
    T *as() const { return static_cast<T *>(p); }
};

struct HostBuf {
    void *p = nullptr;
    size_t cap = 0;
    HostBuf() = default;
    HostBuf(const HostBuf &) = delete;
    HostBuf &operator=(const HostBuf &) = delete;
    ~HostBuf() { release(); }
    cudaError_t ensure(size_t bytes) {
        if (bytes <= cap) return cudaSuccess;
        if (p) cudaFreeHost(p);
        p = nullptr;
        cap = 0;
        const size_t want = bytes + bytes / 8 + 4096;
        cudaError_t e = cudaMallocHost(&p, want);
        if (e == cudaSuccess) cap = want;
        return e;
    }
    void release() {
        if (p) cudaFreeHost(p);
        p = nullptr;
        cap = 0;
    }
};

struct Misc {
    struct {
        GroupCounts counts;
        unsigned long long bad_bases;
    } grp;
    struct {
        unsigned long long total_windows;
        unsigned int max_len;
    } reads;
    uint64_t part_counts[256];
    unsigned long long skr_counters[4];
    uint32_t skr_ticket, n_buckets_dev;
    struct {
        uint32_t n_inst, n_runs;
    } plan;
    unsigned long long chunk_totals[SKR_MAX_CHUNKS];
    SkrGroupCounters gc;
    uint32_t chunk_tickets[SKR_MAX_CHUNKS];
    V3Counters gc3;
    unsigned long long n_mmers;
    unsigned long long n_real_entries;
    uint32_t chunk_bounds[SKR_MAX_CHUNKS + 1];
    uint32_t v3_tickets[2 * SKR_MAX_CHUNKS];
    unsigned long long lsd_totals[SKR_MAX_CHUNKS];
    uint64_t v3_chunk_sum;
    uint32_t split_n_nl, split_n_reads;
    char last_byte;
    unsigned long long digest;
};

struct HostFeed {
    const char *src;
    char *dst;
    uint64_t bytes;
    int chunks;
};
struct HostSink {
    uint64_t *kmer_codes, *kmer_id_off;
    int32_t *read_ids;
    uint64_t kmer_cap, id_cap;
    uint64_t kmers_done, ids_done;
    int chunks;
};

enum : int { EV_START, EV_READS_ON_DEVICE, EV_SCANNED, EV_SORTED, EV_GROUPED, EV_TABLE_ON_HOST, EV_COUNT };

}

struct gbin_ctx {
    gbin_config cfg;
    int KW;
    int sm_count;
    cudaStream_t stream;
    cudaStream_t st_h2d, st_d2h;
    cudaEvent_t ev_feed[SKR_MAX_CHUNKS], ev_chunk[SKR_MAX_CHUNKS], ev_copy;
    cudaStream_t st_aux;
    cudaEvent_t ev_fork, ev_join;
    int host_chunks;
    char err[512];
    gbin_timings tm;
    cudaEvent_t ev[EV_COUNT];
    DevBuf d_reads, d_starts, d_lens, d_ids;
    DevBuf rec_a, rec_b, radix_scratch, win_counts, rec_off, scan_scratch;
    DevBuf group_of, run_start, surv_index, id_offset, surv_group, bucket_of;
    DevBuf misc;
    DevBuf skr_a, skr_b, tile_state, inst_prefix, run_excl, skr_run_start, small_prefix, unit_base, units, unit_state, o_kmer_mmer, bucket_excl, big_list, big_k0, big_k1, big_arr, stg_ids, stg_codes, stg_mmer, stg_off, skr_side;
    DevBuf ent_a, ent_b, piece_n, sorted_info, v3_base64, v3_head_run, v3_unit_out, v3_unit_excl, v3_atoms, v3_lsd_aux, v3_bitmap;
    DevBuf x_list_off, x_ids;
    void *donated = nullptr;
    uint64_t donated_bytes = 0;
    bool v3_lsd_seen = false;
    uint64_t v3_lsd_cap_seen = 0;
    uint64_t v3_pass_max = 2000000000ull;
    uint64_t v3_auto_n = 0;
    int v3_auto_h = 0, v3_auto_nc = 1;
    int v3_h, v3_nc, v3_cap;
    int v3_cap_eff;
    int xchg_timeout_ms = 120000;
    int pipeline;
    int last_pipeline;
    uint32_t fallbacks;
    gbin_run_stats rs;
    struct {
        bool created = false, attached = false;
        uint32_t rank = 0, world = 0, epoch = 0;
        uint64_t cap = 0;
        void *recv = nullptr;
        XchgShared *sh = nullptr;
        char **dst_tab = nullptr;
        XchgResult *result = nullptr;
        XchgPlan plan;
        void *opened[2 * XCHG_MAX_WORLD];
        int n_opened = 0;
    } xg;
    DevBuf o_mmer_codes, o_mmer_kmer_off, o_kmer_codes, o_kmer_id_off, o_read_ids;
    HostBuf h_misc, h_result, h_kmer_codes, h_kmer_id_off, h_read_ids, h_file;
    DevBuf split_nl, split_tiles_buf, split_base;
    KernelProf prof;
};

namespace {

int fail(gbin_ctx *ctx, int code, const char *fmt, ...) {
    if (ctx) {
        va_list ap;
        va_start(ap, fmt);
        vsnprintf(ctx->err, sizeof ctx->err, fmt, ap);
        va_end(ap);
    }
    return code;
}

#define CU(call)                                                                                              \
    do {                                                                                                      \
        cudaError_t e__ = (call);                                                                             \
        if (e__ != cudaSuccess) {                                                                             \
            (void)cudaGetLastError();                                                                         \
            return fail(ctx, e__ == cudaErrorMemoryAllocation ? GBIN_E_NOMEM : GBIN_E_CUDA, "%s: %s (%s:%d)", \
                        #call, cudaGetErrorString(e__), __FILE__, __LINE__);                                  \
        }                                                                                                     \
    } while (0)

int check_config(const gbin_config *c) {
    if (!c) return GBIN_E_INVALID_ARG;
    const int K = c->kmer_size, M = c->mmer_size;
    if (M < 2 || M > 15) return GBIN_E_INVALID_CONFIG;
    if (K < 2 * M || K > 64) return GBIN_E_INVALID_CONFIG;
    return GBIN_OK;
}

cudaError_t begin_call(gbin_ctx *ctx, void *stream, cudaStream_t *st) {
    *st = stream ? static_cast<cudaStream_t>(stream) : ctx->stream;
    return cudaSetDevice(ctx->cfg.device);
}

template <typename T>
cudaError_t read_back(gbin_ctx *ctx, T Misc::*field, cudaStream_t st) {
    Misc *dm = ctx->misc.as<Misc>();
    Misc *hm = static_cast<Misc *>(ctx->h_misc.p);
    const cudaError_t e = cudaMemcpyAsync(&(hm->*field), &(dm->*field), sizeof(T), cudaMemcpyDeviceToHost, st);
    return e == cudaSuccess ? cudaStreamSynchronize(st) : e;
}

gbin_table device_table(const gbin_ctx *ctx, uint64_t n_instances, uint64_t n_distinct, uint64_t S, uint64_t NS, uint64_t B) {
    gbin_table t;
    memset(&t, 0, sizeof t);
    t.kmer_size = ctx->cfg.kmer_size;
    t.mmer_size = ctx->cfg.mmer_size;
    t.abundance_cutoff = ctx->cfg.abundance_cutoff;
    t.kmer_words = ctx->KW;
    t.on_device = 1;
    t.ctx_owned = 1;
    t.n_instances = n_instances;
    t.n_distinct = n_distinct;
    t.n_kmers = S;
    t.n_ids = NS;
    t.n_buckets = B;
    t.mmer_codes = ctx->o_mmer_codes.as<uint32_t>();
    t.mmer_kmer_off = ctx->o_mmer_kmer_off.as<uint64_t>();
    t.kmer_codes = ctx->o_kmer_codes.as<uint64_t>();
    t.kmer_id_off = ctx->o_kmer_id_off.as<uint64_t>();
    t.read_ids = ctx->o_read_ids.as<int32_t>();
    return t;
}

int emit_bucket_directory(gbin_ctx *ctx, uint64_t S, uint64_t NS, cudaStream_t st, int *launches, uint64_t *B) {
    Misc *dm = ctx->misc.as<Misc>();
    Misc *hm = static_cast<Misc *>(ctx->h_misc.p);
    CU(ctx->bucket_excl.ensure((S + 1) * 4));
    CU(ctx->o_mmer_codes.ensure((S + 1) * sizeof(uint32_t)));
    CU(ctx->o_mmer_kmer_off.ensure((S + 2) * sizeof(uint64_t)));
    CU(ctx->scan_scratch.ensure(group_scan_scratch_bytes(S + 1024)));
    const bool on = ctx->prof.begin(KK_EMIT, st);
    const int lp = skr_emit_buckets(ctx->o_kmer_mmer.as<uint32_t>(), S, NS, ctx->bucket_excl.as<uint32_t>(), ctx->scan_scratch.as<uint32_t>(),
                                    ctx->o_mmer_codes.as<uint32_t>(), ctx->o_mmer_kmer_off.as<uint64_t>(), ctx->o_kmer_id_off.as<uint64_t>(),
                                    &dm->n_buckets_dev, st);
    ctx->prof.end(on, lp, st);
    *launches += lp;
    CU(cudaGetLastError());
    CU(read_back(ctx, &Misc::n_buckets_dev, st));
    *B = hm->n_buckets_dev;
    return GBIN_OK;
}

int stream_finished_chunks(gbin_ctx *ctx, HostSink *sink, uint32_t n, const unsigned long long *totals_host, int shift,
                           const unsigned long long *lsd_totals_host) {
    const int KW = ctx->KW;
    for (uint32_t c = 0; c < n; c++) {
        CU(cudaEventSynchronize(ctx->ev_chunk[c]));
        if (lsd_totals_host && lsd_totals_host[c]) break;
        const unsigned long long tot = totals_host[c];
        const uint64_t s1 = tot >> shift, n1 = tot & ((1ull << shift) - 1);
        if (s1 > sink->kmer_cap || n1 > sink->id_cap || s1 < sink->kmers_done || n1 < sink->ids_done) break;
        const uint64_t s0 = sink->kmers_done, n0 = sink->ids_done;
        if (s1 > s0) {
            CU(cudaMemcpyAsync(sink->kmer_codes + s0 * KW, ctx->o_kmer_codes.as<uint64_t>() + s0 * KW, (s1 - s0) * KW * sizeof(uint64_t), cudaMemcpyDeviceToHost, ctx->st_d2h));
            CU(cudaMemcpyAsync(sink->kmer_id_off + s0, ctx->o_kmer_id_off.as<uint64_t>() + s0, (s1 - s0) * sizeof(uint64_t), cudaMemcpyDeviceToHost, ctx->st_d2h));
        }
        if (n1 > n0) CU(cudaMemcpyAsync(sink->read_ids + n0, ctx->o_read_ids.as<int32_t>() + n0, (n1 - n0) * sizeof(int32_t), cudaMemcpyDeviceToHost, ctx->st_d2h));
        sink->kmers_done = s1;
        sink->ids_done = n1;
    }
    return GBIN_OK;
}

int abandon_sink(gbin_ctx *ctx, HostSink *sink) {
    if (!sink) return GBIN_OK;
    CU(cudaStreamSynchronize(ctx->st_d2h));
    sink->kmers_done = sink->ids_done = 0;
    return GBIN_OK;
}

template <typename Launch>
int partition_by_owner(gbin_ctx *ctx, uint64_t n, uint32_t n_parts, void *stream, uint64_t *counts_host, Launch launch) {
    if (!ctx || !counts_host || n_parts == 0 || n_parts > 256) return GBIN_E_INVALID_ARG;
    if (n >= (1ull << 32) - 8192) return fail(ctx, GBIN_E_TOO_LARGE, "too many records in one partition call");
    cudaStream_t st;
    CU(begin_call(ctx, stream, &st));
    CU(ctx->radix_scratch.ensure(radix_scratch_bytes(n)));
    const int launches = launch(ctx->radix_scratch.p, ctx->misc.as<Misc>()->part_counts, st);
// ... 216 lines not shown
    CU(cudaEventRecord(ctx->ev[EV_SORTED], st));

    CU(ctx->inst_prefix.ensure((n_skr + 2) * 4));
    CU(ctx->run_excl.ensure((n_skr + 2) * 8));
    CU(ctx->skr_run_start.ensure((n_skr + 2) * 4));
    CU(ctx->scan_scratch.ensure(group_scan_scratch_bytes(n_skr)));
    bool on = ctx->prof.begin(KK_SKR_PLAN, st);
    int lp = skr_plan_runs(ctx->skr_side.as<uint64_t>(), n_skr, ctx->inst_prefix.as<uint32_t>(), ctx->run_excl.as<uint64_t>(), ctx->skr_run_start.as<uint32_t>(),
                           ctx->scan_scratch.as<uint64_t>(), &dm->plan.n_inst, &dm->plan.n_runs, st);
    ctx->prof.end(on, lp, st);
    *launches += lp;
    CU(cudaGetLastError());
    CU(read_back(ctx, &Misc::plan, st));
    const uint64_t n_runs = hm->plan.n_runs, n = hm->plan.n_inst;
    *n_inst_out = n;
    ctx->rs.n_super_kmers = n_skr;
    ctx->rs.n_mmer_runs = n_runs;
    const uint64_t max_units = skr_max_units(n, n_runs);
    CU(ctx->small_prefix.ensure((n_runs + 1) * 4));
    CU(ctx->unit_base.ensure((n_runs + 1) * 4));
    CU(ctx->units.ensure(max_units * skr_unit_bytes()));
    CU(ctx->unit_state.ensure(max_units * 8));
    CU(ctx->big_list.ensure(skr_max_big_runs(n) * 8));
    CU(ctx->big_k0.ensure((n + 1) * 8));
    if (KW == 2) CU(ctx->big_k1.ensure((n + 1) * 8));
    CU(ctx->big_arr.ensure((n + 1) * 4));
    CU(ctx->scan_scratch.ensure(group_scan_scratch_bytes(n / 2 + n_runs + 1024)));
    on = ctx->prof.begin(KK_SKR_PLAN, st);
    lp = skr_plan_units(sorted, K, ctx->inst_prefix.as<uint32_t>(), ctx->skr_run_start.as<uint32_t>(), n_runs, ctx->small_prefix.as<uint32_t>(),
                        ctx->unit_base.as<uint32_t>(), ctx->scan_scratch.as<uint32_t>(), ctx->units.p, max_units, &dm->gc, ctx->big_list.as<uint32_t>(),
                        ctx->big_k0.as<uint64_t>(), ctx->big_k1.as<uint64_t>(), ctx->big_arr.as<uint32_t>(), ctx->sm_count, st);
    ctx->prof.end(on, lp, st);
    *launches += lp;
    CU(cudaGetLastError());

    const uint64_t kmer_cap = cutoff >= 0 ? n / ((uint64_t)cutoff + 1) + 1 : n + 1;
    CU(ctx->o_kmer_codes.ensure((kmer_cap * KW + 1) * sizeof(uint64_t)));
    CU(ctx->o_kmer_mmer.ensure((kmer_cap + 1) * sizeof(uint32_t)));
    CU(ctx->o_kmer_id_off.ensure((kmer_cap + 2) * sizeof(uint64_t)));
    CU(ctx->o_read_ids.ensure((n + 1) * sizeof(int32_t)));
    CU(ctx->stg_ids.ensure((n + 1) * sizeof(int32_t)));
    CU(ctx->stg_codes.ensure((kmer_cap * KW + 1) * sizeof(uint64_t)));
    CU(ctx->stg_mmer.ensure((kmer_cap + 1) * sizeof(uint32_t)));
    CU(ctx->stg_off.ensure((kmer_cap + 1) * sizeof(uint32_t)));
    on = ctx->prof.begin(KK_SKR_GROUP, st);
    SkrGroupChunks ch{1u, dm->chunk_tickets, nullptr, nullptr, nullptr};
    if (sink && sink->chunks > 1) {
        ch.n = (uint32_t)sink->chunks;
        ch.totals_dev = dm->chunk_totals;
        ch.totals_host = hm->chunk_totals;
        ch.done = ctx->ev_chunk;
    }
    lp = skr_group_launch(sorted, K, cutoff, ctx->inst_prefix.as<uint32_t>(), ctx->units.p, ctx->unit_state.as<unsigned long long>(), max_units, ch,
                          &dm->gc, ctx->big_k0.as<uint64_t>(), ctx->big_k1.as<uint64_t>(), ctx->big_arr.as<uint32_t>(), d_ids, id_base, ctx->o_kmer_codes.as<uint64_t>(), ctx->o_kmer_mmer.as<uint32_t>(),
                          ctx->o_kmer_id_off.as<uint64_t>(), ctx->o_read_ids.as<int32_t>(), kmer_cap, n, ctx->stg_ids.as<int32_t>(), ctx->stg_codes.as<uint64_t>(),
                          ctx->stg_mmer.as<uint32_t>(), ctx->stg_off.as<uint32_t>(), ctx->sm_count, st);
    ctx->prof.end(on, lp, st);
    *launches += lp;
    CU(cudaGetLastError());
    if (ch.done) {
        const int rc = stream_finished_chunks(ctx, sink, ch.n, hm->chunk_totals, 31, nullptr);
        if (rc) return rc;
    }
    CU(read_back(ctx, &Misc::gc, st));
    ctx->rs.n_units = hm->gc.n_units;
    if (hm->gc.overflow) {
        ctx->fallbacks++;
        return GBIN_OK;
    }
    const uint64_t S = hm->gc.total_kmers, NS = hm->gc.total_ids;
    uint64_t B = 0;
    const int rc = emit_bucket_directory(ctx, S, NS, st, launches, &B);
    if (rc) return rc;
    *out = device_table(ctx, n, hm->gc.distinct, S, NS, B);
    *done = true;
    return GBIN_OK;
}


int v3_choose_layout(gbin_ctx *ctx, const void *skr, uint64_t n_skr, cudaStream_t st, KeyLayout *out, int *launches) {
    const int K = ctx->cfg.kmer_size, M = ctx->cfg.mmer_size;
    auto set_cap = [&](const KeyLayout &kl) { ctx->v3_cap_eff = ctx->v3_cap ? ctx->v3_cap : ((ctx->KW == 2 || kl.nc == 2) ? 512 : 1024); };
    if (ctx->v3_nc != 0) {
        *out = make_key_layout(K, M, ctx->v3_h, ctx->v3_nc);
        set_cap(*out);
        return GBIN_OK;
    }
    if (2 * M + 2 > 31 || M > 13 || n_skr == 0) {
        *out = make_key_layout(K, M, 0, 1);
        set_cap(*out);
        return GBIN_OK;
    }
    if (ctx->v3_auto_n && n_skr >= ctx->v3_auto_n / 2 && n_skr <= ctx->v3_auto_n * 2) {
        *out = make_key_layout(K, M, ctx->v3_auto_h, ctx->v3_auto_nc);
        set_cap(*out);
        return GBIN_OK;
    }
    Misc *dm = ctx->misc.as<Misc>();
    Misc *hm = static_cast<Misc *>(ctx->h_misc.p);
    CU(ctx->v3_bitmap.ensure(v3_mmer_bitmap_bytes(M)));
    *launches += v3_count_mmers(skr, K <= 32 ? 8 : 12, n_skr, M, ctx->v3_bitmap.as<uint32_t>(), &dm->n_mmers, st);
    CU(cudaGetLastError());
    CU(read_back(ctx, &Misc::n_mmers, st));
    const double buckets = hm->n_mmers ? (double)hm->n_mmers : 1.0;
    const double mean_inst = (double)n_skr / buckets * ((K - M + 2) / 2.0);
    int nc = 1, h = 0;
    const int cap1 = ctx->v3_cap ? ctx->v3_cap : 1024, cap2 = ctx->v3_cap ? ctx->v3_cap : 512;
    if (mean_inst > cap1 / 2.5) {
        nc = 2;
        double per = mean_inst / 2.0;
        while (per > cap2 / 8.0 && h < 15) {
            per /= 4.0;
            h++;
        }
    }
    *out = make_key_layout(K, M, h, nc);
    set_cap(*out);
    ctx->v3_auto_n = n_skr;
    ctx->v3_auto_h = out->h;
    ctx->v3_auto_nc = out->nc;
    return GBIN_OK;
}

int run_v3_pass(gbin_ctx *ctx, const void *skr, const uint64_t *ent, const uint16_t *sorted_info, uint64_t n_ent, const KeyLayout &kl, const int32_t *d_ids, int32_t id_base, cudaStream_t st,
                uint64_t S_off, uint64_t N_off, bool single_pass, HostSink *sink, int *launches, bool *ok, uint64_t *n_inst, uint64_t *distinct, uint64_t *S_out,
                uint64_t *N_out) {
    *ok = false;
    const int cutoff = ctx->cfg.abundance_cutoff, KW = ctx->KW;
    Misc *dm = ctx->misc.as<Misc>();
    Misc *hm = static_cast<Misc *>(ctx->h_misc.p);
    CU(ctx->inst_prefix.ensure((n_ent + 2) * 4));
    CU(ctx->run_excl.ensure((n_ent + 2) * 8));
    CU(ctx->skr_run_start.ensure((n_ent + 2) * 4));
    CU(ctx->scan_scratch.ensure(group_scan_scratch_bytes(n_ent)));
    bool on = ctx->prof.begin(KK_SKR_PLAN, st);
    int lp = v3_plan_runs(ent, sorted_info, n_ent, ctx->inst_prefix.as<uint32_t>(), ctx->run_excl.as<uint64_t>(), ctx->skr_run_start.as<uint32_t>(),
                          ctx->scan_scratch.as<uint64_t>(), &dm->plan.n_inst, &dm->plan.n_runs, st);
    ctx->prof.end(on, lp, st);
    *launches += lp;
    CU(cudaGetLastError());
    CU(read_back(ctx, &Misc::plan, st));
    const uint64_t n_runs = hm->plan.n_runs, n = hm->plan.n_inst;
    *n_inst = n;
    ctx->rs.n_mmer_runs += n_runs;
    const uint64_t max_units = v3_max_units(n, n_runs, ctx->v3_cap_eff);
    CU(ctx->small_prefix.ensure((n_runs + 2) * 8));
    CU(ctx->v3_base64.ensure((n_runs + 2) * 8));
    CU(ctx->v3_atoms.ensure((4 * n_runs + 8) * 4));
    CU(ctx->v3_head_run.ensure((max_units + 1) * 4));
    CU(ctx->units.ensure(max_units * v3_unit_bytes()));
    CU(ctx->v3_unit_out.ensure(max_units * v3_unit_out_bytes()));
    CU(ctx->v3_unit_excl.ensure((2 * max_units + 2) * 8));
    CU(ctx->scan_scratch.ensure(group_scan_scratch_bytes(n_runs + max_units + 1024)));
    V3Chunks ch{1u, dm->v3_tickets, dm->chunk_bounds, &dm->v3_chunk_sum, dm->chunk_totals, dm->lsd_totals, nullptr, nullptr, nullptr};
    ch.aux = ctx->st_aux;
    ch.ev_fork = ctx->ev_fork;
    ch.ev_join = ctx->ev_join;
    if (single_pass && sink && sink->chunks > 1) {
        ch.n = (uint32_t)sink->chunks;
        ch.totals_host = hm->chunk_totals;
        ch.lsd_totals_host = hm->lsd_totals;
        ch.done = ctx->ev_chunk;
    }
    on = ctx->prof.begin(KK_SKR_PLAN, st);
    lp = v3_plan_units(sorted_info, ent, kl, ctx->v3_cap_eff, ctx->inst_prefix.as<uint32_t>(), ctx->skr_run_start.as<uint32_t>(), n_runs, ctx->small_prefix.as<uint64_t>(),
                       ctx->v3_base64.as<uint64_t>(), ctx->v3_atoms.as<uint32_t>(), ctx->v3_atoms.as<uint32_t>() + 3 * n_runs, ctx->v3_head_run.as<uint32_t>(),
                       ctx->scan_scratch.p, ctx->units.p, max_units, &dm->gc3, ch.n, dm->chunk_bounds, st);
    ctx->prof.end(on, lp, st);
    *launches += lp;
    CU(cudaGetLastError());

    const uint64_t kmer_cap = cutoff >= 0 ? n / ((uint64_t)cutoff + 1) + 1 : n + 1;
    CU(ctx->o_kmer_codes.ensure_keep(((S_off + kmer_cap) * KW + 1) * sizeof(uint64_t), S_off * KW * sizeof(uint64_t), st));
    CU(ctx->o_kmer_mmer.ensure_keep((S_off + kmer_cap + 1) * sizeof(uint32_t), S_off * sizeof(uint32_t), st));
    CU(ctx->o_kmer_id_off.ensure_keep((S_off + kmer_cap + 2) * sizeof(uint64_t), S_off * sizeof(uint64_t), st));
    CU(ctx->o_read_ids.ensure_keep((N_off + n + 1) * sizeof(int32_t), N_off * sizeof(int32_t), st));
    CU(ctx->stg_ids.ensure((n + 1) * sizeof(int32_t)));
    CU(ctx->stg_codes.ensure((kmer_cap * KW + 1) * sizeof(uint64_t)));
    CU(ctx->stg_mmer.ensure((kmer_cap + 1) * sizeof(uint32_t)));
    CU(ctx->stg_off.ensure((kmer_cap + 1) * sizeof(uint32_t)));
    V3Out vo{ctx->o_kmer_codes.as<uint64_t>() + S_off * KW, ctx->o_kmer_mmer.as<uint32_t>() + S_off, ctx->o_kmer_id_off.as<uint64_t>() + S_off,
             ctx->o_read_ids.as<int32_t>() + N_off, kmer_cap, n, ctx->stg_codes.as<uint64_t>(), ctx->stg_mmer.as<uint32_t>(), ctx->stg_off.as<uint32_t>(),
             ctx->stg_ids.as<int32_t>(), ctx->v3_unit_out.p, N_off};
    const size_t rb = sizeof(uint64_t) * KW + 8;
    auto lsd_arrays = [&](uint64_t cap) -> int {
        if (cap == 0) return GBIN_OK;
        CU(ctx->rec_a.ensure((cap + 1) * rb));
        CU(ctx->rec_b.ensure((cap + 1) * rb));
        CU(ctx->v3_lsd_aux.ensure((cap + 1) * 16));
        return GBIN_OK;
    };
    uint64_t lsd_cap = (kl.nc == 2 || ctx->v3_lsd_seen) ? (kmer_cap < (1u << 22) ? kmer_cap : kmer_cap / 4) : 0;
    if (lsd_cap && lsd_cap < ctx->v3_lsd_cap_seen && ctx->v3_lsd_cap_seen <= kmer_cap) lsd_cap = ctx->v3_lsd_cap_seen;
    int rc = lsd_arrays(lsd_cap);
    if (rc) return rc;
    auto lsd_view = [&](uint64_t cap) {
        uint32_t *aux = ctx->v3_lsd_aux.as<uint32_t>();
        return cap ? V3Lsd{ctx->rec_a.p, aux, aux + (cap + 1), aux + 2 * (cap + 1), aux + 3 * (cap + 1), cap} : V3Lsd{nullptr, nullptr, nullptr, nullptr, nullptr, 0};
    };
    uint64_t *unit_excl = ctx->v3_unit_excl.as<uint64_t>(), *lsd_excl = unit_excl + max_units + 1;
    lp = v3_group_launch(skr, ent, ctx->units.p, kl, ctx->v3_cap_eff, cutoff, d_ids, id_base, vo, max_units, unit_excl, lsd_excl, ctx->scan_scratch.p, &dm->gc3, ch,
                         lsd_view(lsd_cap), false, ctx->sm_count, &ctx->prof, st);
    *launches += lp;
    CU(cudaGetLastError());
    if (ch.done) {
        rc = stream_finished_chunks(ctx, sink, ch.n, hm->chunk_totals, 32, hm->lsd_totals);
        if (rc) return rc;
    }
    CU(read_back(ctx, &Misc::gc3, st));
    if (hm->gc3.overflow == 6u && hm->gc3.lsd_kmers > lsd_cap) {
        ctx->v3_lsd_seen = true;
        lsd_cap = hm->gc3.lsd_kmers + hm->gc3.lsd_kmers / 16 + 1024;
        if (lsd_cap > kmer_cap) lsd_cap = kmer_cap;
        ctx->v3_lsd_cap_seen = lsd_cap;
        rc = lsd_arrays(lsd_cap);
        if (rc) return rc;
        CU(cudaMemsetAsync(&dm->gc3.overflow, 0, sizeof(unsigned int), st));
        V3Chunks ch1 = ch;
        ch1.totals_host = ch1.lsd_totals_host = nullptr;
        ch1.done = nullptr;
        lp = v3_group_launch(skr, ent, ctx->units.p, kl, ctx->v3_cap_eff, cutoff, d_ids, id_base, vo, max_units, unit_excl, lsd_excl, ctx->scan_scratch.p, &dm->gc3, ch1,
                             lsd_view(lsd_cap), true, ctx->sm_count, &ctx->prof, st);
        *launches += lp;
        CU(cudaGetLastError());
        CU(read_back(ctx, &Misc::gc3, st));
    }
    ctx->rs.n_units += hm->gc3.n_units;
    ctx->rs.n_lsd_kmers += hm->gc3.lsd_kmers;
    if (hm->gc3.overflow) {
        snprintf(ctx->err, sizeof ctx->err, "pipeline 3 gave the batch up (code %u: a (bucket, d) class larger than a unit)", hm->gc3.overflow);
        return GBIN_OK;
    }
    if (hm->gc3.lsd_kmers) {
        const uint64_t nl = hm->gc3.lsd_kmers;
        CU(ctx->radix_scratch.ensure(radix_scratch_bytes(nl)));
        CU(ctx->run_excl.ensure((nl + 2) * 8));
        CU(ctx->scan_scratch.ensure(group_scan_scratch_bytes(nl + 1024)));
        lp = v3_lsd_finish(kl, nl, ctx->rec_a.p, ctx->rec_b.p, ctx->radix_scratch.p, ctx->run_excl.as<uint64_t>(), ctx->scan_scratch.p, vo, lsd_view(lsd_cap), ctx->sm_count, &ctx->prof,
                           st);
        *launches += lp;
        CU(cudaGetLastError());
    }
    *distinct = hm->gc3.distinct;
    *S_out = hm->gc3.total_kmers;
    *N_out = hm->gc3.total_ids;
    *ok = true;
    return GBIN_OK;
}

int run_v3_group(gbin_ctx *ctx, const void *skr, uint64_t n_skr, const int32_t *d_ids, int32_t id_base, cudaStream_t st, gbin_table *out, int *launches,
                 bool *done, uint64_t *n_inst_out, HostSink *sink = nullptr) {
    *done = false;
    const int K = ctx->cfg.kmer_size, M = ctx->cfg.mmer_size;
    Misc *dm = ctx->misc.as<Misc>();
    Misc *hm = static_cast<Misc *>(ctx->h_misc.p);
    KeyLayout kl;
    int rc = v3_choose_layout(ctx, skr, n_skr, st, &kl, launches);
    if (rc) return rc;
    if (n_skr >= (1ull << (32 - kl.cshift))) return GBIN_OK;
    memset(&ctx->rs, 0, sizeof ctx->rs);
    ctx->rs.n_super_kmers = n_skr;
    ctx->rs.key_nc = (uint32_t)kl.nc;
    ctx->rs.key_h = (uint32_t)kl.h;

    const uint64_t n_slots = n_skr << kl.cshift;
    const uint64_t ent_bytes = ((n_slots + 2) * 8 + 255) & ~255ull;
    uint64_t *ent_a_p, *ent_b_p;
    if (ctx->donated && ctx->donated_bytes >= 2 * ent_bytes && (reinterpret_cast<uintptr_t>(ctx->donated) & 15u) == 0) {
        ent_a_p = static_cast<uint64_t *>(ctx->donated);
        ent_b_p = ent_a_p + ent_bytes / 8;
        if (ctx->ent_a.cap + ctx->ent_b.cap > (1ull << 30)) {
            ctx->ent_a.release();
            ctx->ent_b.release();
        }
    } else {
        CU(ctx->ent_a.ensure(ent_bytes));
        CU(ctx->ent_b.ensure(ent_bytes));
        ent_a_p = ctx->ent_a.as<uint64_t>();
        ent_b_p = ctx->ent_b.as<uint64_t>();
    }
    ctx->donated = nullptr;
    ctx->donated_bytes = 0;
    CU(ctx->piece_n.ensure((n_slots + 16) * 2));
    CU(ctx->sorted_info.ensure((n_slots + 16) * 2));
    bool on = ctx->prof.begin(KK_V3_ENTRIES, st);
    int lp = v3_make_entries(skr, n_skr, kl, ent_a_p, ctx->piece_n.as<uint16_t>(), &dm->n_real_entries, st);
    ctx->prof.end(on, lp, st);
    *launches += lp;
    CU(cudaGetLastError());
    CU(ctx->radix_scratch.ensure(radix_scratch_bytes(n_slots)));
    bool in_b = false;
    int passes = 0;
    *launches += radix_sort_entries(ent_a_p, ent_b_p, n_slots, kl.key_bits, ctx->radix_scratch.p, &in_b, &passes, ctx->piece_n.as<uint16_t>(),
                                    ctx->sorted_info.as<uint16_t>(), &ctx->prof, st, kl.nc == 2 ? &dm->n_real_entries : nullptr);
    CU(cudaGetLastError());
    ctx->tm.sort_passes = (uint32_t)passes;
    const uint64_t *ent = in_b ? ent_b_p : ent_a_p;
    CU(cudaEventRecord(ctx->ev[EV_SORTED], st));
    uint64_t n_ent = n_slots;
    if (kl.nc == 2) {
        CU(read_back(ctx, &Misc::n_real_entries, st));
        n_ent = hm->n_real_entries;
    }

    std::vector<uint64_t> bounds{0, n_ent};
    const uint64_t pass_max = ctx->v3_pass_max;
    if (n_skr * (uint64_t)(K - M + 1) > pass_max) {
        const uint32_t nt = v3_pass_tiles(n_ent);
        CU(ctx->scan_scratch.ensure((size_t)nt * 8 + 64));
        unsigned long long *sums_dev = ctx->scan_scratch.as<unsigned long long>();
        *launches += v3_pass_tile_sums(ctx->sorted_info.as<uint16_t>(), n_ent, sums_dev, st);
        std::vector<unsigned long long> sums(nt);
        CU(cudaMemcpyAsync(sums.data(), sums_dev, (size_t)nt * 8, cudaMemcpyDeviceToHost, st));
        CU(cudaStreamSynchronize(st));
        std::vector<unsigned long long> cuts;
        unsigned long long acc = 0, all = 0;
        for (uint32_t t = 0; t < nt; t++) all += sums[t];
        const uint64_t pass_max = all > 2 * ctx->v3_pass_max ? ctx->v3_pass_max / 2 : ctx->v3_pass_max;
        for (uint32_t t = 0; t < nt; t++) {
            if (acc && acc + sums[t] > pass_max) {
                cuts.push_back((unsigned long long)t * v3_pass_tile_entries());
                acc = 0;
            }
            acc += sums[t];
        }
        if (!cuts.empty()) {
            CU(cudaMemcpyAsync(sums_dev, cuts.data(), cuts.size() * 8, cudaMemcpyHostToDevice, st));
            *launches += v3_pass_bounds(ent, n_ent, kl.mshift, sums_dev, (uint32_t)cuts.size(), st);
            CU(cudaMemcpyAsync(cuts.data(), sums_dev, cuts.size() * 8, cudaMemcpyDeviceToHost, st));
            CU(cudaStreamSynchronize(st));
            bounds.assign(1, 0);
            for (unsigned long long c : cuts)
                if (c > bounds.back() && c < n_ent) bounds.push_back(c);
            bounds.push_back(n_ent);
        }
    }
    const bool single = bounds.size() == 2;
    uint64_t S_off = 0, N_off = 0, n_total = 0, distinct = 0;
    for (size_t p = 0; p + 1 < bounds.size(); p++) {
        bool ok = false;
        uint64_t n_p = 0, d_p = 0, S_p = 0, N_p = 0;
        rc = run_v3_pass(ctx, skr, ent + bounds[p], ctx->sorted_info.as<uint16_t>() + bounds[p], bounds[p + 1] - bounds[p], kl, d_ids, id_base, st, S_off, N_off, single, sink, launches, &ok, &n_p, &d_p, &S_p, &N_p);
        if (rc) return rc;
        if (!ok) return GBIN_OK;
        S_off += S_p;
        N_off += N_p;
        n_total += n_p;
        distinct += d_p;
    }
    *n_inst_out = n_total;
    ctx->rs.n_passes = (uint32_t)(bounds.size() - 1);
    const uint64_t S = S_off, NS = N_off;
    if (S >= (1ull << 32)) return fail(ctx, GBIN_E_TOO_LARGE, "%llu surviving k-mers in one batch (limit 2^32)", (unsigned long long)S);
    uint64_t B = 0;
    rc = emit_bucket_directory(ctx, S, NS, st, launches, &B);
    if (rc) return rc;
    *out = device_table(ctx, n_total, distinct, S, NS, B);
    *done = true;
    return GBIN_OK;
}

int run_skr_group(gbin_ctx *ctx, void *skr, uint64_t n_skr, const int32_t *d_ids, int32_t id_base, cudaStream_t st, gbin_table *out, int *launches, bool *done,
                  uint64_t *n_inst_out, HostSink *sink, int *used) {
    *done = false;
    const int NW = ctx->cfg.kmer_size <= 32 ? 8 : 12;
    if (ctx->pipeline >= 3) {
        int rc = run_v3_group(ctx, skr, n_skr, d_ids, id_base, st, out, launches, done, n_inst_out, sink);
        if (rc) return rc;
        if (*done) {
            *used = 3;
            return GBIN_OK;
        }
        ctx->fallbacks++;
        rc = abandon_sink(ctx, sink);
        if (rc) return rc;
    }
    if (n_skr * (uint64_t)(ctx->cfg.kmer_size - ctx->cfg.mmer_size + 1) >= (1ull << 31))
        return fail(ctx, GBIN_E_TOO_LARGE, "the batch is too large for pipeline 2 (%llu super-k-mer records) and pipeline 3 %s", (unsigned long long)n_skr,
                    ctx->pipeline >= 3 ? "gave it up" : "is switched off");
    CU(ctx->skr_b.ensure((n_skr + 1) * NW * 4));
    int rc = run_v2_group(ctx, skr, ctx->skr_b.p, n_skr, d_ids, id_base, st, out, launches, done, n_inst_out, sink);
    if (rc) return rc;
    if (*done) *used = 2;
    return GBIN_OK;
}

int run_skr_pipelines(gbin_ctx *ctx, const gbin_reads *rd, uint64_t n, uint32_t max_len, cudaStream_t st, gbin_table *out, int *launches, bool *done,
                      const HostFeed *feed, HostSink *sink, int *used) {
    *done = false;
    if (n == 0 || (ctx->pipeline < 3 && n >= (1ull << 31))) return GBIN_OK;
    uint64_t n_skr = 0, n_chk = 0;
    int rc = run_skr_scan(ctx, rd, n, max_len, 0, nullptr, 0, st, &n_skr, launches, feed);
// ... 1116 lines not shown
```

### genome-assembly_b200/csrc/gbin_internal.h

```cpp
#pragma once
#include <cstdint>
#include <cuda_runtime.h>

#include "bin3.cuh"
#include "gbin_device.cuh"

namespace gbin {

enum KernelKind { KK_SCAN = 0, KK_RADIX_HIST, KK_RADIX_TILESCAN, KK_RADIX_SCATTER, KK_RUNS, KK_PRUNE, KK_EMIT, KK_SKR_SCAN, KK_SKR_PLAN, KK_SKR_GROUP, KK_V3_ENTRIES, KK_V3_SPAN, KK_COUNT };
struct KernelProf {
    static constexpr int MAX_REGIONS = 256;
    bool enabled = false;
    bool created = false;
    int n = 0;
    cudaEvent_t a[MAX_REGIONS], b[MAX_REGIONS];
    unsigned char kind[MAX_REGIONS];
    float ms[KK_COUNT];
    unsigned launches[KK_COUNT];
    void reset() {
        n = 0;
        for (int i = 0; i < KK_COUNT; i++) { ms[i] = 0.f; launches[i] = 0; }
    }
    bool begin(int k, cudaStream_t st) {
        if (!enabled || n >= MAX_REGIONS) return false;
        if (!created) {
            for (int i = 0; i < MAX_REGIONS; i++) { cudaEventCreate(&a[i]); cudaEventCreate(&b[i]); }
            created = true;
        }
        kind[n] = (unsigned char)k;
        cudaEventRecord(a[n], st);
        return true;
    }
    void end(bool on, int nlaunch, cudaStream_t st) {
        if (!on) return;
        cudaEventRecord(b[n], st);
        launches[kind[n]] += (unsigned)nlaunch;
        n++;
    }
    void collect() {
        for (int i = 0; i < n; i++) {
            float t = 0.f;
            if (cudaEventElapsedTime(&t, a[i], b[i]) == cudaSuccess) ms[kind[i]] += t;
            else (void)cudaGetLastError();
        }
        n = 0;
    }
    void destroy() {
        if (created) for (int i = 0; i < MAX_REGIONS; i++) { cudaEventDestroy(a[i]); cudaEventDestroy(b[i]); }
        created = false;
    }
};

int launch_count_windows(const ReadsView &rv, int K, uint32_t *counts, cudaStream_t st);
int launch_scan_reads(const ReadsView &rv, const uint64_t *rec_off, int K, int M, int KW, uint32_t arrival_base, uint32_t max_len,
                      void *out, unsigned long long *bad_bases, int sm_count, cudaStream_t st);
uint32_t scan_reads_max_len();

size_t radix_scratch_bytes(uint64_t n);
int radix_sort_records(void *a, void *b, uint64_t n, int KW, int K, int M, void *scratch, bool *result_in_b, int *passes_out,
                       KernelProf *prof, cudaStream_t st);
int radix_partition_by_owner(const void *in, void *out, uint64_t n, int KW, uint32_t n_parts, void *scratch, uint64_t *d_counts,
                             cudaStream_t st);

constexpr int XCHG_MAX_WORLD = 16;
struct XchgShared {
    unsigned long long counts[XCHG_MAX_WORLD * XCHG_MAX_WORLD];
    unsigned int count_flag[XCHG_MAX_WORLD];
    unsigned int done_flag[XCHG_MAX_WORLD];
};
struct XchgResult {
    unsigned long long n_in;
    unsigned long long sent[XCHG_MAX_WORLD];
    unsigned int status;
    unsigned int pad;
};
struct XchgPlan {
    uint32_t rank, world, epoch, pad;
    XchgShared *peer_sh[XCHG_MAX_WORLD];
    void *peer_recv[XCHG_MAX_WORLD];
    unsigned long long cap[XCHG_MAX_WORLD];
    char **dst_tab;
    XchgResult *result;
    long long timeout_cycles;
};
int radix_exchange_skr_by_owner(const void *in, uint64_t n, int skr_words, void *scratch, const XchgPlan &xp, cudaStream_t st);

int radix_sort_skr_by_mmer(void *a, void *b, uint64_t n, int skr_words, int M, void *scratch, bool *result_in_b, int *passes_out,
                           uint64_t *side_out, KernelProf *prof, cudaStream_t st);
int radix_partition_skr_by_owner(const void *in, void *out, uint64_t n, int skr_words, uint32_t n_parts, void *scratch, uint64_t *d_counts,
                                 cudaStream_t st);

int launch_skr_scan(const ReadsView &rv, uint64_t read_begin, uint64_t read_end, int K, int M, uint32_t arrival_base, uint32_t max_len,
                    void *out, uint64_t capacity, unsigned long long *tile_state, uint32_t *ticket, unsigned long long *counters, int sm_count,
                    cudaStream_t st);
uint32_t skr_scan_tiles(uint64_t n_reads, int K, int M, uint32_t max_len);

struct SkrGroupCounters {
    unsigned long long distinct;
    unsigned long long total_kmers, total_ids;
    unsigned int overflow, ticket, n_units, n_big, big_inst, pad[3];
};
size_t skr_group_smem_bytes(int KW);
uint64_t skr_max_units(uint64_t n_inst, uint64_t n_runs);
uint64_t skr_max_big_runs(uint64_t n_inst);
int skr_plan_runs(const uint64_t *side, uint64_t n_skr, uint32_t *inst_prefix, uint64_t *both64, uint32_t *run_start,
                  uint64_t *scratch64, uint32_t *n_inst_dev, uint32_t *n_runs_dev, cudaStream_t st);
size_t skr_unit_bytes();
int skr_plan_units(const void *skr_sorted, int K, const uint32_t *inst_prefix, const uint32_t *run_start, uint64_t n_runs,
                   uint32_t *small_prefix, uint32_t *unit_base, uint32_t *scratch, void *units, uint64_t max_units, void *gc_dev,
                   uint32_t *big_list, uint64_t *big_k0, uint64_t *big_k1, uint32_t *big_arr, int sm_count, cudaStream_t st);
constexpr int SKR_MAX_CHUNKS = 16;
struct SkrGroupChunks {
    uint32_t n;
    uint32_t *tickets;
    unsigned long long *totals_dev;
    unsigned long long *totals_host;
    cudaEvent_t *done;
};
int skr_group_launch(const void *skr_sorted, int K, int cutoff, const uint32_t *inst_prefix, const void *units, unsigned long long *unit_state,
                     uint64_t max_units, const SkrGroupChunks &ch, void *gc_dev, uint64_t *big_k0, uint64_t *big_k1, uint32_t *big_arr, const int32_t *ids_by_arrival, int32_t id_base, uint64_t *kmer_codes,
                     uint32_t *kmer_mmer, uint64_t *kmer_id_off, int32_t *read_ids, uint64_t kmer_cap, uint64_t id_cap, int32_t *stg_ids, uint64_t *stg_codes,
                     uint32_t *stg_mmer, uint32_t *stg_off, int sm_count, cudaStream_t st);
int skr_emit_buckets(const uint32_t *kmer_mmer, uint64_t n_kmers, uint64_t n_ids, uint32_t *bucket_excl, uint32_t *scratch,
                     uint32_t *mmer_codes, uint64_t *mmer_kmer_off, uint64_t *kmer_id_off, uint32_t *n_buckets_dev, cudaStream_t st);

int radix_sort_entries(void *a, void *b, uint64_t n, int key_bits, void *scratch, bool *result_in_b, int *passes_out, const uint16_t *slot_info,
                       uint16_t *sorted_info, KernelProf *prof, cudaStream_t st, const unsigned long long *n_real_dev = nullptr);
int expand_ids_device(const uint64_t *id_off, const int32_t *ids, uint64_t n_kmers, uint32_t K, uint64_t *list_off, int32_t *exp_ids, int sm_count,
                      cudaStream_t st);
int v3_make_entries(const void *skr, uint64_t n_rec, const KeyLayout &kl, uint64_t *ent, uint16_t *piece_info, unsigned long long *n_real_dev,
                    cudaStream_t st);
int v3_plan_runs(const uint64_t *ent, const uint16_t *sorted_info, uint64_t n_ent, uint32_t *inst_prefix, uint64_t *both64, uint32_t *run_start,
                 uint64_t *scratch64, uint32_t *n_inst_dev, uint32_t *n_runs_dev, cudaStream_t st);
uint64_t v3_max_units(uint64_t n_inst, uint64_t n_runs, int cap);
size_t v3_unit_bytes();
size_t v3_unit_out_bytes();
struct V3Counters {
    unsigned long long distinct, total_kmers, total_ids;
    unsigned int overflow, n_units, n_spans, pad;
    unsigned long long lsd_kmers, lsd_ids;
};
int v3_plan_units(const uint16_t *sorted_info, const uint64_t *ent, const KeyLayout &kl, int cap, const uint32_t *inst_prefix, const uint32_t *run_start, uint64_t n_runs,
                  uint64_t *nunits64, uint64_t *base64, uint32_t *atom3, uint32_t *spanlen, uint32_t *head_run, void *scratch, void *units, uint64_t max_units,
                  void *gc_dev, uint32_t n_chunks, uint32_t *chunk_bounds, cudaStream_t st);
struct V3Out {
    uint64_t *kmer_codes;
    uint32_t *kmer_mmer;
    uint64_t *kmer_id_off;
    int32_t *read_ids;
    uint64_t kmer_cap, id_cap;
    uint64_t *stg_codes;
    uint32_t *stg_mmer;
    uint32_t *stg_loff;
    int32_t *stg_ids;
    void *unit_out;
    uint64_t id_off_base;
};
struct V3Lsd {
    void *rec;
    uint32_t *src_off, *cnt, *fidx, *nadj;
    uint64_t cap;
};
struct V3Chunks {
    uint32_t n;
    uint32_t *tickets;
    uint32_t *bounds;
    uint64_t *chunk_sum;
    unsigned long long *totals_dev;
    unsigned long long *lsd_totals_dev;
    unsigned long long *totals_host, *lsd_totals_host;
    cudaEvent_t *done;
    cudaStream_t aux = nullptr;
    cudaEvent_t ev_fork = nullptr, ev_join = nullptr;
};
size_t v3_group_smem_bytes(int KW, int cap);
int v3_group_launch(const void *skr, const uint64_t *ent, const void *units, const KeyLayout &kl, int cap, int cutoff, const int32_t *ids_by_arrival, int32_t id_base,
                    const V3Out &o, uint64_t max_units, uint64_t *unit_excl, uint64_t *lsd_excl, void *scan_scratch, void *gc_dev, const V3Chunks &ch, const V3Lsd &lsd,
                    bool finalize_only, int sm_count, KernelProf *prof, cudaStream_t st);
int v3_lsd_finish(const KeyLayout &kl, uint64_t n, void *rec_a, void *rec_b, void *radix_scratch, uint64_t *dnew, void *scan_scratch, const V3Out &o, const V3Lsd &lsd,
                  int sm_count, KernelProf *prof, cudaStream_t st);
uint32_t v3_pass_tiles(uint64_t n_ent);
uint32_t v3_pass_tile_entries();
int v3_pass_tile_sums(const uint16_t *sorted_info, uint64_t n_ent, unsigned long long *sums_dev, cudaStream_t st);
int v3_pass_bounds(const uint64_t *ent, uint64_t n_ent, int mshift, unsigned long long *bounds_dev, uint32_t n_bounds, cudaStream_t st);
size_t v3_mmer_bitmap_bytes(int M);
int v3_count_mmers(const void *skr, int skr_words, uint64_t n_rec, int M, uint32_t *bitmap, unsigned long long *count_dev, cudaStream_t st);

}
struct gbin_table;
namespace gbin {
int table_digest_device(const ::gbin_table *t, unsigned long long *out_dev, cudaStream_t st);
uint64_t table_digest_host(const ::gbin_table *t);

uint32_t split_tiles(uint64_t n);
int split_find_newlines(const uint8_t *data, uint64_t n, uint32_t *tile_counts, uint32_t *scan_scratch, uint64_t *nl, uint32_t *n_nl_dev,
                        bool emit, cudaStream_t st);
int split_count_reads(const uint64_t *nl, uint64_t n_nl, uint64_t size, uint32_t cap, uint64_t n_lines, uint32_t *read_base, uint32_t *scan_scratch,
                      uint32_t *n_reads_dev, cudaStream_t st);
int split_emit_reads(const uint64_t *nl, uint64_t n_nl, uint64_t size, uint32_t cap, uint64_t n_lines, const uint32_t *read_base, uint64_t *starts,
                     uint32_t *lens, cudaStream_t st);

struct GroupCounts {
    uint32_t n_distinct, n_kmers, n_buckets, pad;
    uint64_t n_ids;
};
struct GroupWorkspace {
    uint32_t *group_of;
    uint32_t *run_start;
    uint32_t *surv_index;
    uint64_t *id_offset;
    uint32_t *surv_group;
    uint32_t *bucket_of;
    void *scan_scratch;
    GroupCounts *counts;
    int cutoff;
};
size_t group_scan_scratch_bytes(uint64_t n);
int group_find_runs(const void *sorted, uint64_t n, int KW, GroupWorkspace &ws, cudaStream_t st);
int group_prune_offsets(uint64_t n, uint64_t n_distinct, int cutoff, GroupWorkspace &ws, cudaStream_t st);
int group_mark_buckets(const void *sorted, int KW, uint64_t n_distinct, uint64_t n_kmers, GroupWorkspace &ws, cudaStream_t st);
struct TableOut {
    uint32_t *mmer_codes;
    uint64_t *mmer_kmer_off;
    uint64_t *kmer_codes;
    uint64_t *kmer_id_off;
    int32_t *read_ids;
};
int group_emit(const void *sorted, uint64_t n, int KW, uint64_t n_distinct, uint64_t n_kmers, uint64_t n_ids, uint64_t n_buckets,
               const int32_t *ids_by_arrival, int32_t id_base, GroupWorkspace &ws, const TableOut &out, cudaStream_t st);

}
```

### genome-assembly_b200/csrc/prefix_scan.cuh

```cuda
#pragma once
#include <cstdint>
#include <cuda_runtime.h>

namespace gbin {

constexpr int SCAN_THREADS = 256;
constexpr int SCAN_ITEMS = 16;
constexpr int SCAN_TILE = SCAN_THREADS * SCAN_ITEMS;

template <typename T>
__device__ __forceinline__ T warp_inclusive_scan(T v) {
    const unsigned lane = threadIdx.x & 31;
#pragma unroll
    for (int d = 1; d < 32; d <<= 1) {
        T o = __shfl_up_sync(0xffffffffu, v, d);
        if (lane >= (unsigned)d) v += o;
    }
    return v;
}

template <typename T>
__device__ __forceinline__ T block_exclusive_scan(T v, T *total) {
    __shared__ T warp_sums[SCAN_THREADS / 32];
    __shared__ T block_total;
    const unsigned lane = threadIdx.x & 31, warp = threadIdx.x >> 5;
    T inc = warp_inclusive_scan(v);
    if (lane == 31) warp_sums[warp] = inc;
    __syncthreads();
    if (warp == 0) {
        T s = lane < SCAN_THREADS / 32 ? warp_sums[lane] : T(0);
        T si = warp_inclusive_scan(s);
        if (lane < SCAN_THREADS / 32) warp_sums[lane] = si - s;
        if (lane == SCAN_THREADS / 32 - 1) block_total = si;
    }
    __syncthreads();
    T res = inc - v + warp_sums[warp];
    *total = block_total;
    __syncthreads();
    return res;
}

template <typename TOut>
__device__ __forceinline__ uint32_t scan_pad(uint32_t p) {
    return p + (sizeof(TOut) == 8 ? (p >> 4) : (p >> 5));
}

template <typename TOut, typename InOp>
__global__ void __launch_bounds__(SCAN_THREADS) scan_reduce_kernel(InOp in, TOut *__restrict__ block_sums, uint64_t n) {
    const uint64_t base = (uint64_t)blockIdx.x * SCAN_TILE;
    TOut s = 0;
#pragma unroll
    for (int i = 0; i < SCAN_ITEMS; i++) {
        const uint64_t j = base + (uint64_t)i * SCAN_THREADS + threadIdx.x;
        if (j < n) s += (TOut)in(j);
    }
    TOut total;
    (void)block_exclusive_scan<TOut>(s, &total);
    if (threadIdx.x == 0) block_sums[blockIdx.x] = total;
}

template <typename TOut, typename InOp>
__global__ void __launch_bounds__(SCAN_THREADS)
    scan_apply_kernel(InOp in, TOut *__restrict__ out, const TOut *__restrict__ block_offsets, uint64_t n, TOut *__restrict__ total_out) {
    __shared__ TOut ex[SCAN_TILE + SCAN_TILE / 16 + 1];
    const uint64_t base = (uint64_t)blockIdx.x * SCAN_TILE;
#pragma unroll
    for (int i = 0; i < SCAN_ITEMS; i++) {
        const uint32_t p = (uint32_t)i * SCAN_THREADS + threadIdx.x;
        const uint64_t j = base + p;
        ex[scan_pad<TOut>(p)] = j < n ? (TOut)in(j) : TOut(0);
    }
    __syncthreads();
    TOut v[SCAN_ITEMS];
    TOut s = 0;
#pragma unroll
    for (int i = 0; i < SCAN_ITEMS; i++) {
        v[i] = ex[scan_pad<TOut>(threadIdx.x * SCAN_ITEMS + i)];
        s += v[i];
    }
    TOut total;
    TOut run = block_exclusive_scan<TOut>(s, &total) + (block_offsets ? block_offsets[blockIdx.x] : TOut(0));
#pragma unroll
    for (int i = 0; i < SCAN_ITEMS; i++) {
        ex[scan_pad<TOut>(threadIdx.x * SCAN_ITEMS + i)] = run;
        run += v[i];
    }
    if (total_out && blockIdx.x == gridDim.x - 1 && threadIdx.x == SCAN_THREADS - 1) *total_out = run;
    __syncthreads();
#pragma unroll
    for (int i = 0; i < SCAN_ITEMS; i++) {
        const uint32_t p = (uint32_t)i * SCAN_THREADS + threadIdx.x;
        const uint64_t j = base + p;
        if (j < n) out[j] = ex[scan_pad<TOut>(p)];
    }
}

template <typename TOut, typename InOp, typename OutOp>
__global__ void __launch_bounds__(SCAN_THREADS)
    scan_apply_to_kernel(InOp in, OutOp out, const TOut *__restrict__ block_offsets, uint64_t n, TOut *__restrict__ total_out) {
    __shared__ TOut ex[SCAN_TILE + SCAN_TILE / 16 + 1];
    const uint64_t base = (uint64_t)blockIdx.x * SCAN_TILE;
#pragma unroll
    for (int i = 0; i < SCAN_ITEMS; i++) {
        const uint32_t p = (uint32_t)i * SCAN_THREADS + threadIdx.x;
        const uint64_t j = base + p;
        ex[scan_pad<TOut>(p)] = j < n ? (TOut)in(j) : TOut(0);
    }
    __syncthreads();
    TOut v[SCAN_ITEMS];
    TOut s = 0;
#pragma unroll
    for (int i = 0; i < SCAN_ITEMS; i++) {
        v[i] = ex[scan_pad<TOut>(threadIdx.x * SCAN_ITEMS + i)];
        s += v[i];
    }
    TOut total;
    TOut run = block_exclusive_scan<TOut>(s, &total) + (block_offsets ? block_offsets[blockIdx.x] : TOut(0));
#pragma unroll
    for (int i = 0; i < SCAN_ITEMS; i++) {
        ex[scan_pad<TOut>(threadIdx.x * SCAN_ITEMS + i)] = run;
        run += v[i];
    }
    if (total_out && blockIdx.x == gridDim.x - 1 && threadIdx.x == SCAN_THREADS - 1) *total_out = run;
    __syncthreads();
#pragma unroll
    for (int i = 0; i < SCAN_ITEMS; i++) {
        const uint32_t p = (uint32_t)i * SCAN_THREADS + threadIdx.x;
        const uint64_t j = base + p;
        if (j < n) out(j, ex[scan_pad<TOut>(p)]);
    }
}

template <typename T>
struct PtrIn {
    const T *p;
    __device__ __forceinline__ T operator()(uint64_t j) const { return p[j]; }
};

inline uint64_t scan_scratch_elems(uint64_t n) {
    uint64_t tot = 0;
    while (n > (uint64_t)SCAN_TILE) {
        n = (n + SCAN_TILE - 1) / SCAN_TILE;
        tot += n;
    }
    return tot + 1;
}

template <typename TOut, typename InOp>
int exclusive_scan(InOp in, TOut *out, uint64_t n, TOut *scratch, TOut *total_out, cudaStream_t st) {
    if (n == 0) {
        if (total_out) cudaMemsetAsync(total_out, 0, sizeof(TOut), st);
        return 0;
    }
    const uint64_t blocks = (n + SCAN_TILE - 1) / SCAN_TILE;
    if (blocks == 1) {
        scan_apply_kernel<TOut, InOp><<<1, SCAN_THREADS, 0, st>>>(in, out, nullptr, n, total_out);
        return 1;
    }
    int launches = 0;
    scan_reduce_kernel<TOut, InOp><<<(unsigned)blocks, SCAN_THREADS, 0, st>>>(in, scratch, n);
    launches++;
    launches += exclusive_scan<TOut, PtrIn<TOut>>(PtrIn<TOut>{scratch}, scratch, blocks, scratch + blocks, nullptr, st);
    scan_apply_kernel<TOut, InOp><<<(unsigned)blocks, SCAN_THREADS, 0, st>>>(in, out, scratch, n, total_out);
    return launches + 1;
}

template <typename TOut, typename InOp, typename OutOp>
int exclusive_scan_to(InOp in, OutOp out, uint64_t n, TOut *scratch, TOut *total_out, cudaStream_t st) {
    if (n == 0) {
        if (total_out) cudaMemsetAsync(total_out, 0, sizeof(TOut), st);
        return 0;
    }
    const uint64_t blocks = (n + SCAN_TILE - 1) / SCAN_TILE;
    if (blocks == 1) {
        scan_apply_to_kernel<TOut, InOp, OutOp><<<1, SCAN_THREADS, 0, st>>>(in, out, nullptr, n, total_out);
        return 1;
    }
    int launches = 0;
    scan_reduce_kernel<TOut, InOp><<<(unsigned)blocks, SCAN_THREADS, 0, st>>>(in, scratch, n);
    launches++;
    launches += exclusive_scan<TOut, PtrIn<TOut>>(PtrIn<TOut>{scratch}, scratch, blocks, scratch + blocks, nullptr, st);
    scan_apply_to_kernel<TOut, InOp, OutOp><<<(unsigned)blocks, SCAN_THREADS, 0, st>>>(in, out, scratch, n, total_out);
    return launches + 1;
}

}
```

### include/gbin.h

```cpp
#ifndef GBIN_H
#define GBIN_H

#include <stddef.h>
#include <stdint.h>

#ifdef __cplusplus
extern "C" {
#endif

#define GBIN_OK 0
#define GBIN_E_INVALID_CONFIG (-1)
#define GBIN_E_CUDA (-2)
#define GBIN_E_NOMEM (-3)
#define GBIN_E_NON_ACGT (-4)
#define GBIN_E_STATE (-5)
#define GBIN_E_TOO_LARGE (-6)
#define GBIN_E_INVALID_ARG (-7)
#define GBIN_E_IO (-8)

#define GBIN_MAX_READ_LEN 4096
uint32_t gbin_max_read_len(void);

typedef struct gbin_config {
    int32_t kmer_size;
    int32_t mmer_size;
    int32_t abundance_cutoff;
    int32_t device;
} gbin_config;

typedef struct gbin_table {
    int32_t kmer_size, mmer_size, abundance_cutoff;
    int32_t kmer_words;
    int32_t on_device;
    int32_t ctx_owned;
    uint64_t n_instances;
    uint64_t n_distinct;
    uint64_t n_buckets;
    uint64_t n_kmers;
    uint64_t n_ids;
    uint32_t *mmer_codes;
    uint64_t *mmer_kmer_off;
    uint64_t *kmer_codes;
    uint64_t *kmer_id_off;
    int32_t *read_ids;
} gbin_table;

typedef struct gbin_reads {
    const char *data;
    uint64_t data_bytes;
    uint64_t n_reads;
    uint64_t stride;
    uint32_t read_len;
    int32_t id_base;
    const uint64_t *starts;
    const uint32_t *lens;
    const int32_t *read_ids;
    uint32_t max_read_len;
    uint32_t reserved;
} gbin_reads;

typedef struct gbin_ctx gbin_ctx;

typedef struct gbin_timings {
    float h2d_ms, scan_ms, sort_ms, group_ms, d2h_ms, total_ms;
    uint32_t kernel_launches;
    uint32_t sort_passes;
} gbin_timings;

const char *gbin_strerror(int code);
const char *gbin_last_error(const gbin_ctx *ctx);
int gbin_version(void);

int gbin_create(const gbin_config *cfg, gbin_ctx **out);
void gbin_destroy(gbin_ctx *ctx);
int gbin_get_config(const gbin_ctx *ctx, gbin_config *out);

int gbin_bin_reads_host(gbin_ctx *ctx, const gbin_reads *reads, gbin_table *out);
int gbin_table_clone(const gbin_table *host, gbin_table *out);
void gbin_table_free(gbin_table *t);
void *gbin_pinned_alloc(size_t bytes);
void gbin_pinned_free(void *p);

int gbin_bin_reads_device(gbin_ctx *ctx, const gbin_reads *reads, void *stream, gbin_table *out);

int gbin_table_to_host(gbin_ctx *ctx, const gbin_table *dev, gbin_table *host);
int gbin_table_to_pinned(gbin_ctx *ctx, const gbin_table *dev, void *stream, gbin_table *host);

int gbin_table_digest(gbin_ctx *ctx, const gbin_table *table, void *stream, uint64_t *digest_out);

int gbin_get_timings(const gbin_ctx *ctx, gbin_timings *out);

typedef struct gbin_run_stats {
    uint64_t n_super_kmers;
    uint64_t n_mmer_runs;
    uint64_t n_units;
    uint64_t n_lsd_kmers;
    uint32_t key_nc, key_h;
    uint32_t n_passes;
    uint32_t reserved;
} gbin_run_stats;
int gbin_get_run_stats(const gbin_ctx *ctx, gbin_run_stats *out);
int gbin_set_pipeline(gbin_ctx *ctx, int pipeline);
int gbin_set_tuning(gbin_ctx *ctx, const char *name, int value);
int gbin_donate_scratch(gbin_ctx *ctx, void *d_ptr, uint64_t bytes);
int gbin_get_pipeline_info(const gbin_ctx *ctx, int *configured, int *last_used, uint32_t *fallbacks);

#define GBIN_KERNEL_KINDS 12
typedef struct gbin_kernel_profile {
    float ms[GBIN_KERNEL_KINDS];
    uint32_t launches[GBIN_KERNEL_KINDS];
} gbin_kernel_profile;
int gbin_set_kernel_profiling(gbin_ctx *ctx, int enable);
int gbin_get_kernel_profile(const gbin_ctx *ctx, gbin_kernel_profile *out);
const char *gbin_kernel_kind_name(int kind);


uint32_t gbin_record_bytes(const gbin_ctx *ctx);
int gbin_count_instances_device(gbin_ctx *ctx, const gbin_reads *reads, void *stream, uint64_t *n_out);
int gbin_scan_reads_device(gbin_ctx *ctx, const gbin_reads *reads, uint32_t arrival_base, void *d_records,
                           uint64_t capacity, void *stream, uint64_t *n_out);
uint32_t gbin_owner_of(uint32_t mmer_code, uint32_t n_parts);
int gbin_partition_records_device(gbin_ctx *ctx, const void *d_records, uint64_t n, uint32_t n_parts, void *d_out,
                                  void *stream, uint64_t *counts_host);
int gbin_group_records_device(gbin_ctx *ctx, void *d_records, uint64_t n, const int32_t *d_ids_by_arrival,
                              int32_t id_base, void *stream, gbin_table *out);

uint32_t gbin_skr_record_bytes(const gbin_ctx *ctx);
int gbin_scan_skr_device(gbin_ctx *ctx, const gbin_reads *reads, uint32_t arrival_base, void *d_skr, uint64_t capacity, void *stream,
                         uint64_t *n_skr_out, uint64_t *n_instances_out);
int gbin_partition_skr_device(gbin_ctx *ctx, const void *d_skr, uint64_t n, uint32_t n_parts, void *d_out, void *stream,
                              uint64_t *counts_host);
int gbin_group_skr_device(gbin_ctx *ctx, void *d_skr, uint64_t n_skr, const int32_t *d_ids_by_arrival, int32_t id_base, void *stream,
                          gbin_table *out, int *used_fallback);

#define GBIN_XCHG_HANDLE_BYTES 192
int gbin_xchg_create(gbin_ctx *ctx, uint32_t rank, uint32_t world, uint64_t capacity_records, void *handle_out);
int gbin_xchg_attach(gbin_ctx *ctx, const void *all_handles);
int gbin_xchg_exchange_skr(gbin_ctx *ctx, const void *d_skr, uint64_t n, void *stream, void **d_recv_out, uint64_t *n_recv_out,
                           uint64_t *sent_counts);
void gbin_xchg_detach(gbin_ctx *ctx);
void gbin_xchg_destroy(gbin_ctx *ctx);

typedef struct gbin_multi gbin_multi;
int gbin_multi_create(const gbin_config *cfg, const int *devices, int n_devices, gbin_multi **out);
void gbin_multi_destroy(gbin_multi *m);
int gbin_multi_devices(const gbin_multi *m);
gbin_ctx *gbin_multi_context(gbin_multi *m, int i);
const char *gbin_multi_last_error(const gbin_multi *m);
int gbin_multi_bin_reads_host(gbin_multi *m, const gbin_reads *reads, gbin_table *tables_out);

int gbin_split_reads_device(gbin_ctx *ctx, const char *d_data, uint64_t data_bytes, int read_length_define, void *stream, gbin_reads *out);
int gbin_copy_to_host(gbin_ctx *ctx, void *host_dst, const void *device_src, uint64_t bytes);
int gbin_bin_file_host(gbin_ctx *ctx, const char *path, int read_length_define, gbin_table *out);


int gbin_read_file_fgets(const char *path, int read_length_define, char **data_out, uint64_t *data_bytes_out,
                         uint64_t **starts_out, uint32_t **lens_out, uint64_t *n_reads_out);
int gbin_table_dump(const gbin_table *host, const char *path);
int gbin_table_dump_reference_format(const gbin_table *host, const char *path);
int gbin_table_dump_expanded_format(const gbin_table *host, const char *path);

typedef struct gbin_expanded {
    int32_t kmer_size;
    int32_t on_device;
    uint64_t n_lists, n_ids;
    uint64_t *list_off;
    int32_t *ids;
} gbin_expanded;
int gbin_expand_read_ids_device(gbin_ctx *ctx, const gbin_table *dev_table, void *stream, gbin_expanded *out);
int gbin_expanded_to_host(gbin_ctx *ctx, const gbin_expanded *dev, gbin_expanded *host);
void gbin_expanded_free(gbin_expanded *host);
int gbin_table_dump_expanded_lists(const gbin_table *table, const gbin_expanded *lists, const char *path);

struct ZHashTable;
int getval(char c);
char getbp(int bp);
int getscore(char *string);
struct ZHashTable *process_read(struct ZHashTable *hash_table, char *read, int read_id);
struct ZHashTable *prune_data(struct ZHashTable *hash_table);
int gbin_ref_configure(int kmer_size, int mmer_size, int abundance_cutoff, int device);
int gbin_ref_last_status(void);
void gbin_ref_reset(struct ZHashTable *hash_table);
int gbin_table_to_zhash(const gbin_table *host, struct ZHashTable *into);
void gbin_zhash_release(struct ZHashTable *table);

#ifdef __cplusplus
}
#endif
#endif
```

Baseline: 23.37 billion.

## Replace warp-per-unit finalize with per-k-mer tiled placement and fused dual scan

Replaces the warp-per-unit finalize kernel with a place kernel that assigns work per k-mer tile. It uses precomputed kmer_tile and id_tile maps plus a shared-memory search over unit prefixes, so skewed unit sizes no longer cause load imbalance. The all-unit and long-span prefix scans are fused into one scan over a two-field struct, and short-span binary searches are batched four at a time for memory-level parallelism. It adds extra tile-map arrays and scratch memory and more launches, and it exposes new per-category placement statistics.

```diff
diff --git a/genome-assembly_b200/binding.py b/genome-assembly_b200/binding.py
--- a/genome-assembly_b200/binding.py
+++ b/genome-assembly_b200/binding.py
@@ -107,7 +107,7 @@
     L.gbin_pinned_free.argtypes = [vp]
     L.gbin_pinned_free.restype = None
     L.gbin_get_timings.argtypes = [vp, C.POINTER(Timings)]
-    L.gbin_get_run_stats.argtypes = [vp, C.POINTER(u64 * 6)]
+    L.gbin_get_run_stats.argtypes = [vp, C.POINTER(u64 * 12)]
     L.gbin_set_pipeline.argtypes = [vp, C.c_int]
     L.gbin_table_digest.argtypes = [vp, C.POINTER(CTable), vp, C.POINTER(u64)]
     L.gbin_set_tuning.argtypes = [vp, C.c_char_p, C.c_int]
@@ -311,10 +311,12 @@
         return {"configured": a.value, "last_used": b.value, "fallbacks": c.value}
 
     def run_stats(self) -> dict:
-        a = (C.c_uint64 * 6)()
+        a = (C.c_uint64 * 12)()
         self._check(self.lib.gbin_get_run_stats(self.h, C.byref(a)))
         return {"n_super_kmers": int(a[0]), "n_mmer_runs": int(a[1]), "n_units": int(a[2]), "n_lsd_kmers": int(a[3]),
-                "key_nc": int(a[4]) & 0xffffffff, "key_h": int(a[4]) >> 32, "n_passes": int(a[5]) & 0xffffffff}
+                "key_nc": int(a[4]) & 0xffffffff, "key_h": int(a[4]) >> 32, "n_passes": int(a[5]) & 0xffffffff,
+                "n_kmers_plain": int(a[6]), "n_kmers_short": int(a[7]), "n_kmers_long": int(a[8]),
+                "n_ids_plain": int(a[9]), "n_ids_short": int(a[10]), "n_ids_long": int(a[11])}
 
     def set_kernel_profiling(self, enable: bool):
         self._check(self.lib.gbin_set_kernel_profiling(self.h, int(enable)))
diff --git a/genome-assembly_b200/csrc/bin3.cu b/genome-assembly_b200/csrc/bin3.cu
--- a/genome-assembly_b200/csrc/bin3.cu
+++ b/genome-assembly_b200/csrc/bin3.cu
@@ -219,6 +219,7 @@
     unsigned int n_units, n_spans;
     unsigned int pad;
     unsigned long long lsd_kmers, lsd_ids;
+    unsigned long long placed[4];
 };
 
 __global__ void v3_head_runs_kernel(const uint64_t *__restrict__ nunits, const uint64_t *__restrict__ base, uint64_t n_runs, uint32_t *__restrict__ head_run) {
@@ -837,28 +838,69 @@
 }
 
 
-struct UnitSN {
+__host__ __device__ inline bool span_is_long(uint32_t span_len) {
+    return span_len == SPAN_MEMBER_LONG || (span_len > SPAN_SHORT_MAX && span_len != SPAN_MEMBER);
+}
+
+struct SN2 {
+    uint64_t all, lsd;
+    SN2() = default;
+    __host__ __device__ constexpr SN2(int z) : all((uint64_t)z), lsd((uint64_t)z) {}
+    __host__ __device__ constexpr SN2(uint64_t a, uint64_t l) : all(a), lsd(l) {}
+    __device__ __forceinline__ SN2 &operator+=(const SN2 &o) {
+        all += o.all;
+        lsd += o.lsd;
+        return *this;
+    }
+};
+__device__ __forceinline__ SN2 operator+(SN2 a, const SN2 &b) { return a += b; }
+__device__ __forceinline__ SN2 operator-(const SN2 &a, const SN2 &b) { return SN2(a.all - b.all, a.lsd - b.lsd); }
+__device__ __forceinline__ SN2 __shfl_up_sync(unsigned mask, const SN2 &v, unsigned d) {
+    return SN2((uint64_t)::__shfl_up_sync(mask, (unsigned long long)v.all, d), (uint64_t)::__shfl_up_sync(mask, (unsigned long long)v.lsd, d));
+}
+
+constexpr int PL_THREADS = 256, PL_ITEMS = 4, PL_TILE = PL_THREADS * PL_ITEMS;
+constexpr int PL_UNITS = 2048;
+constexpr int GA_THREADS = 256, GA_ITEMS = 16, GA_TILE = GA_THREADS * GA_ITEMS;
+
+struct UnitSN2 {
+    const UnitOut3 *uo;
+    const Unit3 *units;
+    const uint32_t *chunk_bounds;
+    uint32_t chunk;
+    __device__ __forceinline__ SN2 operator()(uint64_t u) const {
+        if (u < chunk_bounds[chunk] || u >= chunk_bounds[chunk + 1]) return SN2(0);
+        const UnitOut3 o = uo[u];
+        const uint64_t sn = ((uint64_t)o.S << 32) | o.N;
+        return SN2(sn, span_is_long(units[u].span_len) ? sn : 0ull);
+    }
+};
+
+struct UnitExclSink {
+    SN2 *excl;
+    uint32_t *kmer_tile;
     const UnitOut3 *uo;
     const uint32_t *chunk_bounds;
     uint32_t chunk;
-    __device__ __forceinline__ uint64_t operator()(uint64_t u) const {
-        if (u < chunk_bounds[chunk] || u >= chunk_bounds[chunk + 1]) return 0ull;
-        return ((uint64_t)uo[u].S << 32) | uo[u].N;
+    __device__ __forceinline__ void operator()(uint64_t u, const SN2 &p) const {
+        excl[u] = p;
+        if (u < chunk_bounds[chunk] || u >= chunk_bounds[chunk + 1]) return;
+        const uint64_t a = p.all >> 32, e = a + uo[u].S;
+        for (uint64_t t = (a + PL_TILE - 1) / PL_TILE; t * PL_TILE < e; t++) kmer_tile[t] = (uint32_t)u;
     }
 };
 
-__global__ void v3_chunk_total_kernel(const uint64_t *__restrict__ chunk_sum, uint32_t chunk, unsigned long long *__restrict__ totals, G3Counters *__restrict__ gc,
-                                      uint32_t n_chunks, int which) {
-    const unsigned long long t = (chunk ? totals[chunk - 1] : 0ull) + *chunk_sum;
+__global__ void v3_chunk_total_kernel(const SN2 *__restrict__ chunk_sum, uint32_t chunk, unsigned long long *__restrict__ totals,
+                                      unsigned long long *__restrict__ lsd_totals, G3Counters *__restrict__ gc, uint32_t n_chunks) {
+    const SN2 s = *chunk_sum;
+    const unsigned long long t = (chunk ? totals[chunk - 1] : 0ull) + s.all, l = (chunk ? lsd_totals[chunk - 1] : 0ull) + s.lsd;
     totals[chunk] = t;
+    lsd_totals[chunk] = l;
     if (chunk + 1 == n_chunks) {
-        if (which == 0) {
-            gc->total_kmers = t >> 32;
-            gc->total_ids = t & 0xffffffffull;
-        } else {
-            gc->lsd_kmers = t >> 32;
-            gc->lsd_ids = t & 0xffffffffull;
-        }
+        gc->total_kmers = t >> 32;
+        gc->total_ids = t & 0xffffffffull;
+        gc->lsd_kmers = l >> 32;
+        gc->lsd_ids = l & 0xffffffffull;
     }
 }
 
@@ -868,10 +910,11 @@
     uint64_t *kmer_id_off;
     int32_t *read_ids;
     uint64_t id_off_base;
+    uint32_t *src_of;
+    uint32_t *id_tile;
 };
 
 struct G3Lsd {
-    const uint64_t *excl;
     void *rec;
     uint32_t *src_off;
     uint32_t *cnt;
@@ -880,162 +923,291 @@
     uint64_t cap;
 };
 
-struct UnitSNLong {
-    const UnitOut3 *uo;
-    const Unit3 *units;
-    const uint32_t *chunk_bounds;
-    uint32_t chunk;
-    __device__ __forceinline__ uint64_t operator()(uint64_t u) const {
-        if (u < chunk_bounds[chunk] || u >= chunk_bounds[chunk + 1]) return 0ull;
-        const uint32_t sl = units[u].span_len;
-        if (sl != SPAN_MEMBER_LONG && (sl <= SPAN_SHORT_MAX || sl == SPAN_MEMBER)) return 0ull;
-        return ((uint64_t)uo[u].S << 32) | uo[u].N;
-    }
+__device__ __forceinline__ void mark_id_tiles(uint32_t *id_tile, uint64_t beg, uint32_t cnt, uint64_t g) {
+    for (uint64_t t = (beg + GA_TILE - 1) / GA_TILE; t * GA_TILE < beg + cnt; t++) id_tile[t] = (uint32_t)g;
+}
+
+struct Place {
+    uint64_t g, beg;
 };
-
+constexpr int SS_GROUP = 4;
 template <int KW>
-__device__ __forceinline__ void finalize3_unit(const Unit3 *__restrict__ units, const uint64_t *__restrict__ unit_excl, unsigned long long base,
-                                               unsigned long long lsd_base, const G3Stage &st, const G3Final &fin, const G3Lsd &ls, G3Counters *gc, uint32_t u,
-                                               uint32_t lane, bool only_long) {
-    const uint32_t span_len = units[u].span_len;
-    if (only_long && span_len != SPAN_MEMBER_LONG && (span_len <= SPAN_SHORT_MAX || span_len == SPAN_MEMBER)) return;
-    const uint64_t ex = unit_excl[u];
-    const UnitOut3 uo = st.unit_out[u];
-    const uint64_t Sb = (base >> 32) + (ex >> 32), Nb = (base & 0xffffffffull) + (ex & 0xffffffffull);
-    if (span_len == 0) {
-        const uint64_t kb = uo.ibase / st.kdiv;
-        for (uint32_t x0 = 0; x0 < uo.S; x0 += 128) {
-            uint64_t c0[4], c1[4];
-            uint32_t mm[4], lo[4];
-#pragma unroll
-            for (int q = 0; q < 4; q++) {
-                const uint32_t x = x0 + q * 32 + lane;
-                if (x < uo.S) {
-                    c0[q] = st.codes[(kb + x) * KW];
-                    if (KW == 2) c1[q] = st.codes[(kb + x) * KW + 1];
-                    mm[q] = st.mmer[kb + x];
-                    lo[q] = st.loff[kb + x];
-                }
-            }
-#pragma unroll
-            for (int q = 0; q < 4; q++) {
-                const uint32_t x = x0 + q * 32 + lane;
-                if (x < uo.S) {
-                    fin.kmer_codes[(Sb + x) * KW] = c0[q];
-                    if (KW == 2) fin.kmer_codes[(Sb + x) * KW + 1] = c1[q];
-                    fin.kmer_mmer[Sb + x] = mm[q];
-                    fin.kmer_id_off[Sb + x] = fin.id_off_base + Nb + lo[q];
-                }
-            }
-        }
-        const int32_t *src = st.ids + uo.ibase;
-        int32_t *dst = fin.read_ids + Nb;
-        for (uint32_t i0 = 0; i0 < uo.N; i0 += 256) {
-            int32_t v[8];
-#pragma unroll
-            for (int q = 0; q < 8; q++) {
-                const uint32_t i = i0 + q * 32 + lane;
-                if (i < uo.N) v[q] = __ldcs(src + i);
-            }
-#pragma unroll
-            for (int q = 0; q < 8; q++) {
-                const uint32_t i = i0 + q * 32 + lane;
-                if (i < uo.N) dst[i] = v[q];
-            }
-        }
-        return;
-    }
-    if (span_len == SPAN_MEMBER_LONG || (span_len > SPAN_SHORT_MAX && span_len != SPAN_MEMBER)) {
-        const uint64_t lx = ls.excl[u];
-        const uint64_t q0 = (lsd_base >> 32) + (lx >> 32), nq0 = (lsd_base & 0xffffffffull) + (lx & 0xffffffffull);
-        if (q0 + uo.S > ls.cap) {
-            if (lane == 0) atomicExch(&gc->overflow, 6u);
-            return;
-        }
-        const uint64_t kb = uo.ibase / st.kdiv;
-        Rec<KW> *rec = static_cast<Rec<KW> *>(ls.rec);
-        for (uint32_t x = lane; x < uo.S; x += 32) {
-            const uint64_t p = q0 + x;
-            Rec<KW> r;
-            r.k[0] = st.codes[(kb + x) * KW];
-            if (KW == 2) r.k[KW - 1] = st.codes[(kb + x) * KW + 1];
-            r.mmer = st.mmer[kb + x];
-            r.arrival = (uint32_t)p;
-            store_rec<KW>(rec + p, r);
-            const uint32_t lo = st.loff[kb + x];
-            ls.src_off[p] = uo.ibase + lo;
-            ls.cnt[p] = (x + 1 < uo.S ? st.loff[kb + x + 1] : uo.N) - lo;
-            ls.fidx[p] = (uint32_t)(Sb + x);
-            ls.nadj[p] = (uint32_t)(Nb - nq0);
-        }
-        return;
-    }
-    uint32_t h = u;
-    while (units[h].span_len == SPAN_MEMBER) h--;
-    const uint32_t R = units[h].span_len;
-    const uint64_t exh = unit_excl[h];
-    const uint64_t Sh = (base >> 32) + (exh >> 32), Nh = (base & 0xffffffffull) + (exh & 0xffffffffull);
-    if (uo.S == 0) return;
-    const uint32_t j = u - h;
-    const uint64_t kbj = uo.ibase / st.kdiv;
-    const uint32_t mmer = st.mmer[kbj];
-    for (uint32_t x0 = 0; x0 < uo.S; x0 += 32) {
-        const uint32_t x = x0 + lane;
-        uint32_t lo = 0, cnt = 0;
-        uint64_t idoff = 0;
-        if (x < uo.S) {
-            const uint64_t k0 = st.codes[(kbj + x) * KW], k1 = KW == 2 ? st.codes[(kbj + x) * KW + 1] : 0ull;
-            lo = st.loff[kbj + x];
-            cnt = (x + 1 < uo.S ? st.loff[kbj + x + 1] : uo.N) - lo;
-            uint32_t rank = x;
-            idoff = lo;
-            for (uint32_t j2 = 0; j2 < R; j2++) {
-                if (j2 == j) continue;
+__device__ __forceinline__ Place short_span_place(const Unit3 *__restrict__ units, const SN2 *__restrict__ excl, uint64_t Sb0, uint64_t Nb0, const G3Stage &st,
+                                               uint32_t h, uint32_t u, uint32_t x, uint32_t lo, uint64_t k0, uint64_t k1) {
+    const uint32_t R = units[h].span_len, j = u - h;
+    const uint64_t exh = excl[h].all;
+    uint32_t rank = x;
+    uint64_t idoff = lo;
+    for (uint32_t j0 = 0; j0 < R; j0 += SS_GROUP) {
+        uint64_t kb[SS_GROUP];
+        uint32_t a[SS_GROUP], b[SS_GROUP], S[SS_GROUP], N[SS_GROUP];
+#pragma unroll
+        for (int r = 0; r < SS_GROUP; r++) {
+            const uint32_t j2 = j0 + r;
+            kb[r] = 0;
+            S[r] = N[r] = 0;
+            if (j2 < R && j2 != j) {
                 const UnitOut3 u2 = st.unit_out[h + j2];
-                const uint64_t kb2 = u2.ibase / st.kdiv;
-                uint32_t a = 0, b = u2.S;
-                while (a < b) {
-                    const uint32_t m = (a + b) >> 1;
-                    const uint64_t q0 = st.codes[(kb2 + m) * KW];
-                    bool less = q0 < k0;
-                    if constexpr (KW == 2) less = less || (q0 == k0 && st.codes[(kb2 + m) * KW + 1] < k1);
-                    if (less) a = m + 1;
-                    else b = m;
-                }
-                rank += a;
-                idoff += a < u2.S ? st.loff[kb2 + a] : u2.N;
-            }
-            fin.kmer_codes[(Sh + rank) * KW] = k0;
-            if (KW == 2) fin.kmer_codes[(Sh + rank) * KW + 1] = k1;
-            fin.kmer_mmer[Sh + rank] = mmer;
-            fin.kmer_id_off[Sh + rank] = fin.id_off_base + Nh + idoff;
-        }
-        const uint32_t nl = min(32u, uo.S - x0);
-        for (uint32_t l0 = 0; l0 < nl; l0 += 4) {
-            const uint32_t l = l0 + (lane >> 3);
-            const uint32_t c = __shfl_sync(0xffffffffu, cnt, l & 31);
-            const uint32_t so = __shfl_sync(0xffffffffu, lo, l & 31);
-            const uint64_t d = __shfl_sync(0xffffffffu, idoff, l & 31);
-            if (l < nl) {
-                const int32_t *src = st.ids + uo.ibase + so;
-                int32_t *dst = fin.read_ids + Nh + d;
-                for (uint32_t i = lane & 7u; i < c; i += 8) dst[i] = src[i];
-            }
-        }
-    }
+                kb[r] = u2.ibase / st.kdiv;
+                S[r] = u2.S;
+                N[r] = u2.N;
+            }
+            a[r] = 0;
+            b[r] = S[r];
+        }
+        bool more = true;
+        while (more) {
+            uint64_t q0[SS_GROUP], q1[SS_GROUP];
+#pragma unroll
+            for (int r = 0; r < SS_GROUP; r++) {
+                const uint64_t m = kb[r] + ((a[r] + b[r]) >> 1);
+                q0[r] = a[r] < b[r] ? st.codes[m * KW] : 0ull;
+                q1[r] = (KW == 2 && a[r] < b[r]) ? st.codes[m * KW + 1] : 0ull;
+            }
+            more = false;
+#pragma unroll
+            for (int r = 0; r < SS_GROUP; r++) {
+                if (a[r] < b[r]) {
+                    const uint32_t m = (a[r] + b[r]) >> 1;
+                    bool less = q0[r] < k0;
+                    if constexpr (KW == 2) less = less || (q0[r] == k0 && q1[r] < k1);
+                    if (less) a[r] = m + 1;
+                    else b[r] = m;
+                    more |= a[r] < b[r];
+                }
+            }
+        }
+#pragma unroll
+        for (int r = 0; r < SS_GROUP; r++) {
+            if (S[r] == 0) continue;
+            rank += a[r];
+            idoff += a[r] < S[r] ? st.loff[kb[r] + a[r]] : N[r];
+        }
+    }
+    return Place{Sb0 + (exh >> 32) + rank, Nb0 + (exh & 0xffffffffull) + idoff};
 }
 
 template <int KW>
-__global__ void __launch_bounds__(128, 12)
-    finalize3_kernel(const Unit3 *__restrict__ units, const uint64_t *__restrict__ unit_excl, const unsigned long long *__restrict__ totals,
-                     const unsigned long long *__restrict__ lsd_totals, G3Stage st, G3Final fin, G3Lsd ls, G3Counters *__restrict__ gc,
-                     const uint32_t *__restrict__ chunk_bounds, uint32_t chunk, bool only_long) {
+__global__ void __launch_bounds__(PL_THREADS)
+    place3_kernel(const Unit3 *__restrict__ units, const SN2 *__restrict__ excl, const uint32_t *__restrict__ kmer_tile, const unsigned long long *__restrict__ totals,
+                  const unsigned long long *__restrict__ lsd_totals, G3Stage st, G3Final fin, G3Lsd ls, G3Counters *__restrict__ gc,
+                  const uint32_t *__restrict__ chunk_bounds, uint32_t chunk, bool only_long) {
+    __shared__ uint32_t s_pre[PL_UNITS];
+    __shared__ unsigned long long s_cnt[4];
+    const uint32_t tid = threadIdx.x;
+    if (tid < 4) s_cnt[tid] = 0;
+    __syncthreads();
+    const uint32_t unit_end = chunk_bounds[chunk + 1];
+    const unsigned long long base = chunk ? totals[chunk - 1] : 0ull, lsd_base = chunk ? lsd_totals[chunk - 1] : 0ull;
+    const uint64_t Sb0 = base >> 32, Nb0 = base & 0xffffffffull;
+    const uint32_t nk = (uint32_t)((totals[chunk] >> 32) - Sb0);
+    unsigned long long n_plain = 0, i_plain = 0;
+    for (uint32_t k0 = blockIdx.x * PL_TILE; k0 < nk; k0 += gridDim.x * PL_TILE) {
+        const uint32_t t = k0 / PL_TILE;
+        const uint32_t u_lo = kmer_tile[t], u_hi = k0 + PL_TILE < nk ? kmer_tile[t + 1] : unit_end - 1;
+        const uint32_t nu = u_hi - u_lo + 1;
+        const bool in_smem = nu <= (uint32_t)PL_UNITS;
+        __syncthreads();
+        if (in_smem)
+            for (uint32_t j = tid; j < nu; j += PL_THREADS) s_pre[j] = (uint32_t)(excl[u_lo + j].all >> 32);
+        __syncthreads();
+        auto pre = [&](uint32_t j) { return in_smem ? s_pre[j] : (uint32_t)(excl[u_lo + j].all >> 32); };
+        uint32_t u[PL_ITEMS], x[PL_ITEMS];
+#pragma unroll
+        for (int q = 0; q < PL_ITEMS; q++) {
+            const uint32_t k = k0 + q * PL_THREADS + tid;
+            u[q] = 0xffffffffu;
+            x[q] = 0;
+            if (k < nk) {
+                uint32_t a = 0, b = nu, pa = pre(0);
+                while (b - a > 1) {
+                    const uint32_t m = (a + b) >> 1, pm = pre(m);
+                    if (pm <= k) {
+                        a = m;
+                        pa = pm;
+                    } else {
+                        b = m;
+                    }
+                }
+                u[q] = u_lo + a;
+                x[q] = k - pa;
+            }
+        }
+        uint32_t sl[PL_ITEMS], ib[PL_ITEMS], S[PL_ITEMS], N[PL_ITEMS];
+        SN2 ex[PL_ITEMS];
+#pragma unroll
+        for (int q = 0; q < PL_ITEMS; q++) {
+            if (u[q] != 0xffffffffu) {
+                sl[q] = units[u[q]].span_len;
+                const UnitOut3 o = st.unit_out[u[q]];
+                ib[q] = o.ibase;
+                S[q] = o.S;
+                N[q] = o.N;
+                ex[q] = excl[u[q]];
+            }
+        }
+        uint64_t c0[PL_ITEMS], c1[PL_ITEMS];
+        uint32_t mm[PL_ITEMS], lo[PL_ITEMS], cnt[PL_ITEMS];
+#pragma unroll
+        for (int q = 0; q < PL_ITEMS; q++) {
+            if (u[q] != 0xffffffffu) {
+                const uint64_t j = ib[q] / st.kdiv + x[q];
+                c0[q] = st.codes[j * KW];
+                c1[q] = KW == 2 ? st.codes[j * KW + 1] : 0ull;
+                mm[q] = st.mmer[j];
+                lo[q] = st.loff[j];
+                cnt[q] = (x[q] + 1 < S[q] ? st.loff[j + 1] : N[q]) - lo[q];
+            }
+        }
+#pragma unroll
+        for (int q = 0; q < PL_ITEMS; q++) {
+            if (u[q] == 0xffffffffu) continue;
+            const uint64_t Sb = Sb0 + (ex[q].all >> 32), Nb = Nb0 + (ex[q].all & 0xffffffffull);
+            if (span_is_long(sl[q])) {
+                const uint64_t q0 = (lsd_base >> 32) + (ex[q].lsd >> 32), nq0 = (lsd_base & 0xffffffffull) + (ex[q].lsd & 0xffffffffull);
+                if (q0 + S[q] > ls.cap) {
+                    if (x[q] == 0) atomicExch(&gc->overflow, 6u);
+                    continue;
+                }
+                const uint64_t p = q0 + x[q];
+                Rec<KW> r;
+                r.k[0] = c0[q];
+                if (KW == 2) r.k[KW - 1] = c1[q];
+                r.mmer = mm[q];
+                r.arrival = (uint32_t)p;
+                store_rec<KW>(static_cast<Rec<KW> *>(ls.rec) + p, r);
+                ls.src_off[p] = ib[q] + lo[q];
+                ls.cnt[p] = cnt[q];
+                ls.fidx[p] = (uint32_t)(Sb + x[q]);
+                ls.nadj[p] = (uint32_t)(Nb - nq0);
+                continue;
+            }
+            if (only_long || sl[q] != 0) continue;
+            const uint64_t g = Sb + x[q], beg = Nb + lo[q];
+            n_plain++;
+            i_plain += cnt[q];
+            fin.kmer_codes[g * KW] = c0[q];
+            if (KW == 2) fin.kmer_codes[g * KW + 1] = c1[q];
+            fin.kmer_mmer[g] = mm[q];
+            fin.kmer_id_off[g] = fin.id_off_base + beg;
+            fin.src_of[g] = ib[q] + lo[q];
+            mark_id_tiles(fin.id_tile, beg, cnt[q], g);
+        }
+    }
+    if (n_plain) atomicAdd(&s_cnt[0], n_plain);
+    if (i_plain) atomicAdd(&s_cnt[1], i_plain);
+    __syncthreads();
+    if (tid < 2 && s_cnt[tid]) atomicAdd(&gc->placed[tid], s_cnt[tid]);
+}
+
+template <int KW>
+__global__ void __launch_bounds__(128)
+    place_short_kernel(const Unit3 *__restrict__ units, const SN2 *__restrict__ excl, const unsigned long long *__restrict__ totals, G3Stage st, G3Final fin,
+                       G3Counters *__restrict__ gc, const uint32_t *__restrict__ chunk_bounds, uint32_t chunk) {
+    __shared__ unsigned long long s_cnt[2];
+    if (threadIdx.x < 2) s_cnt[threadIdx.x] = 0;
+    __syncthreads();
     const uint32_t lane = threadIdx.x & 31;
     const uint32_t unit_begin = chunk_bounds[chunk], unit_end = chunk_bounds[chunk + 1];
     const unsigned long long base = chunk ? totals[chunk - 1] : 0ull;
-    const unsigned long long lsd_base = chunk ? lsd_totals[chunk - 1] : 0ull;
-    for (uint32_t u = unit_begin + blockIdx.x * 4 + (threadIdx.x >> 5); u < unit_end; u += gridDim.x * 4)
-        finalize3_unit<KW>(units, unit_excl, base, lsd_base, st, fin, ls, gc, u, lane, only_long);
+    const uint64_t Sb0 = base >> 32, Nb0 = base & 0xffffffffull;
+    const uint32_t n_warps = gridDim.x * 4, w = blockIdx.x * 4 + (threadIdx.x >> 5);
+    unsigned long long n_short = 0, i_short = 0;
+    for (uint64_t u0 = unit_begin; u0 < unit_end; u0 += 32ull * n_warps) {
+        const uint64_t mine = u0 + (uint64_t)lane * n_warps + w;
+        bool is_short = false;
+        if (mine < unit_end) {
+            const uint32_t sl = units[mine].span_len;
+            is_short = sl != 0 && !span_is_long(sl);
+        }
+        for (unsigned todo = __ballot_sync(0xffffffffu, is_short); todo; todo &= todo - 1) {
+            const uint32_t u = (uint32_t)(u0 + (uint64_t)(__ffs(todo) - 1) * n_warps + w);
+            const bool member = units[u].span_len == SPAN_MEMBER;
+            const bool head = lane < SPAN_SHORT_MAX - 1 && u >= lane + 1u && units[u - 1 - lane].span_len != SPAN_MEMBER;
+            const unsigned hb = __ballot_sync(0xffffffffu, head);
+            const uint32_t h = member ? u - (uint32_t)__ffs(hb) : u;
+            const UnitOut3 uo = st.unit_out[u];
+            const uint64_t kb = uo.ibase / st.kdiv;
+            for (uint32_t x = lane; x < uo.S; x += 32) {
+                const uint64_t k0 = st.codes[(kb + x) * KW], k1 = KW == 2 ? st.codes[(kb + x) * KW + 1] : 0ull;
+                const uint32_t mm = st.mmer[kb + x], lo = st.loff[kb + x];
+                const uint32_t cnt = (x + 1 < uo.S ? st.loff[kb + x + 1] : uo.N) - lo;
+                const Place pl = short_span_place<KW>(units, excl, Sb0, Nb0, st, h, u, x, lo, k0, k1);
+                fin.kmer_codes[pl.g * KW] = k0;
+                if (KW == 2) fin.kmer_codes[pl.g * KW + 1] = k1;
+                fin.kmer_mmer[pl.g] = mm;
+                fin.kmer_id_off[pl.g] = fin.id_off_base + pl.beg;
+                fin.src_of[pl.g] = uo.ibase + lo;
+                mark_id_tiles(fin.id_tile, pl.beg, cnt, pl.g);
+                n_short++;
+                i_short += cnt;
+            }
+        }
+    }
+    if (n_short) atomicAdd(&s_cnt[0], n_short);
+    if (i_short) atomicAdd(&s_cnt[1], i_short);
+    __syncthreads();
+    if (threadIdx.x < 2 && s_cnt[threadIdx.x]) atomicAdd(&gc->placed[2 + threadIdx.x], s_cnt[threadIdx.x]);
+}
+
+__global__ void __launch_bounds__(GA_THREADS)
+    gather3_kernel(const unsigned long long *__restrict__ totals, const unsigned long long *__restrict__ lsd_totals, uint32_t chunk, bool after_lsd, G3Final fin,
+                   const int32_t *__restrict__ stg_ids, G3Counters *__restrict__ gc) {
+    __shared__ uint32_t s_beg[GA_TILE + 1], s_src[GA_TILE + 1];
+    __shared__ uint16_t s_own[GA_TILE];
+    const bool has_long = lsd_totals[chunk] != (chunk ? lsd_totals[chunk - 1] : 0ull);
+    if (has_long != after_lsd) return;
+    const unsigned long long t0 = chunk ? totals[chunk - 1] : 0ull, t1 = totals[chunk];
+    const uint64_t s0 = t0 >> 32, s1 = t1 >> 32, n0 = t0 & 0xffffffffull, n1 = t1 & 0xffffffffull;
+    const uint32_t tid = threadIdx.x;
+    for (uint64_t i0 = (n0 / GA_TILE + blockIdx.x) * GA_TILE; i0 < n1; i0 += (uint64_t)gridDim.x * GA_TILE) {
+        const uint64_t t = i0 / GA_TILE;
+        const uint64_t lo = i0 > n0 ? i0 : n0, hi = i0 + GA_TILE < n1 ? i0 + GA_TILE : n1;
+        const uint64_t g_lo = i0 >= n0 ? fin.id_tile[t] : s0;
+        const uint64_t g_hi = i0 + GA_TILE < n1 ? fin.id_tile[t + 1] : s1 - 1;
+        const uint32_t nk = (uint32_t)(g_hi - g_lo + 1);
+        if (nk > (uint32_t)GA_TILE + 1u) {
+            if (tid == 0) atomicExch(&gc->overflow, 7u);
+            continue;
+        }
+        __syncthreads();
+        for (uint32_t j = tid; j < nk; j += GA_THREADS) {
+            s_beg[j] = (uint32_t)(fin.kmer_id_off[g_lo + j] - fin.id_off_base);
+            s_src[j] = fin.src_of[g_lo + j];
+        }
+        __syncthreads();
+        {
+            const uint64_t p0 = i0 + (uint64_t)tid * GA_ITEMS;
+            const uint32_t first = (uint32_t)(p0 > lo ? p0 : lo);
+            if (first < hi && first < p0 + GA_ITEMS) {
+                uint32_t a = 0, b = nk;
+                while (b - a > 1) {
+                    const uint32_t m = (a + b) >> 1;
+                    if (s_beg[m] <= first) a = m;
+                    else b = m;
+                }
+                for (uint32_t i = first; i < hi && i < p0 + GA_ITEMS; i++) {
+                    while (a + 1 < nk && s_beg[a + 1] <= i) a++;
+                    s_own[i - i0] = (uint16_t)a;
+                }
+            }
+        }
+        __syncthreads();
+        int32_t v[GA_ITEMS];
+#pragma unroll
+        for (int q = 0; q < GA_ITEMS; q++) {
+            const uint64_t i = i0 + q * GA_THREADS + tid;
+            if (i >= lo && i < hi) {
+                const uint32_t a = s_own[i - i0];
+                v[q] = __ldcs(stg_ids + s_src[a] + ((uint32_t)i - s_beg[a]));
+            }
+        }
+#pragma unroll
+        for (int q = 0; q < GA_ITEMS; q++) {
+            const uint64_t i = i0 + q * GA_THREADS + tid;
+            if (i >= lo && i < hi) fin.read_ids[i] = v[q];
+        }
+    }
 }
 
 template <int KW>
@@ -1050,23 +1222,13 @@
     const uint64_t q = (uint64_t)blockIdx.x * blockDim.x + threadIdx.x;
     if (q >= n) return;
     const Rec<KW> r = load_rec<KW>(rec + q);
-    const uint64_t f = ls.fidx[q];
+    const uint64_t f = ls.fidx[q], beg = dnew[q] + ls.nadj[q];
     fin.kmer_codes[f * KW] = r.k[0];
     if (KW == 2) fin.kmer_codes[f * KW + 1] = r.k[KW - 1];
     fin.kmer_mmer[f] = r.mmer;
-    fin.kmer_id_off[f] = fin.id_off_base + dnew[q] + ls.nadj[q];
-}
-
-template <int KW>
-__global__ void __launch_bounds__(256)
-    lsd_lists_kernel(const Rec<KW> *__restrict__ rec, uint64_t n, const uint64_t *__restrict__ dnew, G3Lsd ls, const int32_t *__restrict__ stg_ids, G3Final fin) {
-    const uint64_t q = ((uint64_t)blockIdx.x * blockDim.x + threadIdx.x) >> 3;
-    if (q >= n) return;
-    const uint32_t p = rec[q].arrival;
-    const uint32_t c = ls.cnt[p];
-    const int32_t *src = stg_ids + ls.src_off[p];
-    int32_t *dst = fin.read_ids + dnew[q] + ls.nadj[q];
-    for (uint32_t i = threadIdx.x & 7u; i < c; i += 8) dst[i] = src[i];
+    fin.kmer_id_off[f] = fin.id_off_base + beg;
+    fin.src_of[f] = ls.src_off[r.arrival];
+    mark_id_tiles(fin.id_tile, beg, ls.cnt[r.arrival], f);
 }
 
 __global__ void v3_chunk_bounds_kernel(const Unit3 *__restrict__ units, const G3Counters *__restrict__ gc, uint32_t n_chunks, uint32_t *__restrict__ chunk_bounds) {
@@ -1136,6 +1298,19 @@
     return l + 1;
 }
 
+size_t v3_tile_words(uint64_t kmer_cap, uint64_t id_cap) { return kmer_cap / PL_TILE + id_cap / GA_TILE + 4; }
+size_t v3_unit_scan_scratch_bytes(uint64_t max_units) { return (scan_scratch_elems<SN2>(max_units) + 4) * sizeof(SN2); }
+
+static G3Final final_view(const V3Out &o) {
+    return G3Final{o.kmer_codes, o.kmer_mmer, o.kmer_id_off, o.read_ids, o.id_off_base, o.src_of, o.tiles + o.kmer_cap / PL_TILE + 2};
+}
+
+static unsigned gather_grid(int sm_count) {
+    int per_sm = 0;
+    cudaOccupancyMaxActiveBlocksPerMultiprocessor(&per_sm, gather3_kernel, GA_THREADS, 0);
+    return (unsigned)(sm_count * (per_sm > 0 ? per_sm : 1));
+}
+
 size_t v3_group_smem_bytes(int KW, int cap) {
     const size_t per_warp = cap == 512 ? (KW == 1 ? WarpLayout<512, 1>::BYTES : WarpLayout<512, 2>::BYTES)
                                        : (KW == 1 ? WarpLayout<1024, 1>::BYTES : WarpLayout<1024, 2>::BYTES);
@@ -1143,7 +1318,7 @@
 }
 
 int v3_group_launch(const void *skr, const uint64_t *ent, const void *units, const KeyLayout &kl, int cap, int cutoff, const int32_t *ids_by_arrival, int32_t id_base,
-                    const V3Out &o, uint64_t max_units, uint64_t *unit_excl, uint64_t *lsd_excl, void *scan_scratch, void *gc_dev, const V3Chunks &ch, const V3Lsd &lsd,
+                    const V3Out &o, uint64_t max_units, void *unit_excl, void *scan_scratch, void *gc_dev, const V3Chunks &ch, const V3Lsd &lsd,
                     bool finalize_only, int sm_count, KernelProf *prof, cudaStream_t st) {
     const int KW = kl.K <= 32 ? 1 : 2;
     constexpr int WARPS = G3_WARPS;
@@ -1151,8 +1326,11 @@
     cudaMemsetAsync(ch.tickets, 0, sizeof(uint32_t) * 2 * ch.n, st);
     const uint32_t kdiv = cutoff >= 0 ? (uint32_t)cutoff + 1u : 1u;
     G3Stage stg{o.stg_codes, o.stg_mmer, o.stg_loff, o.stg_ids, static_cast<UnitOut3 *>(o.unit_out), o.kmer_cap, o.id_cap, kdiv};
-    G3Final fin{o.kmer_codes, o.kmer_mmer, o.kmer_id_off, o.read_ids, o.id_off_base};
-    G3Lsd ls{lsd_excl, lsd.rec, lsd.src_off, lsd.cnt, lsd.fidx, lsd.nadj, lsd.cap};
+    const G3Final fin = final_view(o);
+    G3Lsd ls{lsd.rec, lsd.src_off, lsd.cnt, lsd.fidx, lsd.nadj, lsd.cap};
+    SN2 *excl = static_cast<SN2 *>(unit_excl);
+    uint32_t *kmer_tile = o.tiles;
+    const unsigned grid_g = gather_grid(sm_count);
     G3Counters *gc = static_cast<G3Counters *>(gc_dev);
     const uint32_t *sk = static_cast<const uint32_t *>(skr);
     const Unit3 *un = static_cast<const Unit3 *>(units);
@@ -1172,7 +1350,10 @@
         if (l_per_sm < 1 || l_per_sm > 2) l_per_sm = 2;
     }
     const bool side_by_side = sbs && ch.aux && ch.ev_fork && ch.ev_join;
-    auto launch = [&](auto kern, auto kern_small, auto fin_kern) {
+    auto launch = [&](auto kern, auto kern_small, auto place_kern, auto short_kern) {
+        int place_per_sm = 0;
+        cudaOccupancyMaxActiveBlocksPerMultiprocessor(&place_per_sm, place_kern, PL_THREADS, 0);
+        const unsigned grid_p = (unsigned)(sm_count * (place_per_sm > 0 ? place_per_sm : 1));
         cudaFuncSetAttribute(kern, cudaFuncAttributeMaxDynamicSharedMemorySize, (int)smem);
         if (hybrid) cudaFuncSetAttribute(kern_small, cudaFuncAttributeMaxDynamicSharedMemorySize, (int)smem_s);
         for (uint32_t c = 0; c < ch.n; c++) {
@@ -1195,13 +1376,28 @@
                 launches += hybrid ? 2 : 1;
             }
             bool on = prof && prof->begin(KK_V3_SPAN, st);
-            int l = exclusive_scan<uint64_t, UnitSN>(UnitSN{stg.unit_out, ch.bounds, c}, unit_excl, max_units, static_cast<uint64_t *>(scan_scratch), ch.chunk_sum, st);
-            v3_chunk_total_kernel<<<1, 1, 0, st>>>(ch.chunk_sum, c, ch.totals_dev, gc, ch.n, 0);
-            l += exclusive_scan<uint64_t, UnitSNLong>(UnitSNLong{stg.unit_out, un, ch.bounds, c}, lsd_excl, max_units, static_cast<uint64_t *>(scan_scratch), ch.chunk_sum, st);
-            v3_chunk_total_kernel<<<1, 1, 0, st>>>(ch.chunk_sum, c, ch.lsd_totals_dev, gc, ch.n, 1);
-            fin_kern<<<sm_count * 12, 128, 0, st>>>(un, unit_excl, ch.totals_dev, ch.lsd_totals_dev, stg, fin, ls, gc, ch.bounds, c, finalize_only);
-            if (prof) prof->end(on, l + 3, st);
-            launches += l + 3;
+            SN2 *chunk_sum = reinterpret_cast<SN2 *>(ch.chunk_sum);
+            int l = exclusive_scan_to<SN2>(UnitSN2{stg.unit_out, un, ch.bounds, c}, UnitExclSink{excl, kmer_tile, stg.unit_out, ch.bounds, c}, max_units,
+                                           static_cast<SN2 *>(scan_scratch), chunk_sum, st);
+            v3_chunk_total_kernel<<<1, 1, 0, st>>>(chunk_sum, c, ch.totals_dev, ch.lsd_totals_dev, gc, ch.n);
+            const bool beside = !finalize_only && ch.aux && ch.ev_fork && ch.ev_join;
+            if (beside) {
+                cudaEventRecord(ch.ev_fork, st);
+                cudaStreamWaitEvent(ch.aux, ch.ev_fork, 0);
+            }
+            if (!finalize_only) short_kern<<<sm_count * 12, 128, 0, beside ? ch.aux : st>>>(un, excl, ch.totals_dev, stg, fin, gc, ch.bounds, c);
+            place_kern<<<grid_p, PL_THREADS, 0, st>>>(un, excl, kmer_tile, ch.totals_dev, ch.lsd_totals_dev, stg, fin, ls, gc, ch.bounds, c, finalize_only);
+            if (beside) {
+                cudaEventRecord(ch.ev_join, ch.aux);
+                cudaStreamWaitEvent(st, ch.ev_join, 0);
+            }
+            l += finalize_only ? 2 : 3;
+            if (!finalize_only) {
+                gather3_kernel<<<grid_g, GA_THREADS, 0, st>>>(ch.totals_dev, ch.lsd_totals_dev, c, false, fin, stg.ids, gc);
+                l++;
+            }
+            if (prof) prof->end(on, l, st);
+            launches += l;
             if (ch.totals_host) {
                 cudaMemcpyAsync(ch.totals_host + c, ch.totals_dev + c, sizeof(unsigned long long), cudaMemcpyDeviceToHost, st);
                 cudaMemcpyAsync(ch.lsd_totals_host + c, ch.lsd_totals_dev + c, sizeof(unsigned long long), cudaMemcpyDeviceToHost, st);
@@ -1217,9 +1413,9 @@
     }
     const int u_sel = uu > 0 ? uu : (cap == 512 ? 2 : 4);
 #define G3_LAUNCH(PW_, KW_, CAP_) \
-    (u_sel == 1 ? launch(group3_kernel<PW_, KW_, CAP_, WARPS, 1>, group3_kernel<PW_, KW_, 512, WARPS, 2>, finalize3_kernel<KW_>) \
-             : (u_sel == 2 ? launch(group3_kernel<PW_, KW_, CAP_, WARPS, 2>, group3_kernel<PW_, KW_, 512, WARPS, 2>, finalize3_kernel<KW_>) \
-                           : launch(group3_kernel<PW_, KW_, CAP_, WARPS, 4>, group3_kernel<PW_, KW_, 512, WARPS, 2>, finalize3_kernel<KW_>)))
+    (u_sel == 1 ? launch(group3_kernel<PW_, KW_, CAP_, WARPS, 1>, group3_kernel<PW_, KW_, 512, WARPS, 2>, place3_kernel<KW_>, place_short_kernel<KW_>) \
+             : (u_sel == 2 ? launch(group3_kernel<PW_, KW_, CAP_, WARPS, 2>, group3_kernel<PW_, KW_, 512, WARPS, 2>, place3_kernel<KW_>, place_short_kernel<KW_>) \
+                           : launch(group3_kernel<PW_, KW_, CAP_, WARPS, 4>, group3_kernel<PW_, KW_, 512, WARPS, 2>, place3_kernel<KW_>, place_short_kernel<KW_>)))
     if (KW == 1) {
         if (cap == 512) G3_LAUNCH(2, 1, 512);
         else G3_LAUNCH(2, 1, 1024);
@@ -1514,7 +1710,7 @@
 }
 
 int v3_lsd_finish(const KeyLayout &kl, uint64_t n, void *rec_a, void *rec_b, void *radix_scratch, uint64_t *dnew, void *scan_scratch, const V3Out &o, const V3Lsd &lsd,
-                  int sm_count, KernelProf *prof, cudaStream_t st) {
+                  const V3Chunks &ch, void *gc_dev, int sm_count, KernelProf *prof, cudaStream_t st) {
     if (n == 0) return 0;
     const int KW = kl.K <= 32 ? 1 : 2;
     bool in_b = false;
@@ -1538,23 +1734,24 @@
     }
     if (need_global) l += radix_sort_records(rec_a, rec_b, n, KW, kl.K, kl.M, radix_scratch, &in_b, &passes, prof, st);
     const void *sorted = in_b ? rec_b : rec_a;
-    G3Final fin{o.kmer_codes, o.kmer_mmer, o.kmer_id_off, o.read_ids, o.id_off_base};
-    G3Lsd ls{nullptr, nullptr, lsd.src_off, lsd.cnt, lsd.fidx, lsd.nadj, lsd.cap};
+    const G3Final fin = final_view(o);
+    G3Lsd ls{nullptr, lsd.src_off, lsd.cnt, lsd.fidx, lsd.nadj, lsd.cap};
     bool on = prof && prof->begin(KK_V3_SPAN, st);
     int l2 = 0;
     if (KW == 1) {
         const Rec<1> *r = static_cast<const Rec<1> *>(sorted);
         l2 += exclusive_scan<uint64_t, LsdCnt<1>>(LsdCnt<1>{r, lsd.cnt}, dnew, n, static_cast<uint64_t *>(scan_scratch), nullptr, st);
         lsd_place_kernel<1><<<(unsigned)((n + 255) / 256), 256, 0, st>>>(r, n, dnew, ls, fin);
-        lsd_lists_kernel<1><<<(unsigned)((n * 8 + 255) / 256), 256, 0, st>>>(r, n, dnew, ls, o.stg_ids, fin);
     } else {
         const Rec<2> *r = static_cast<const Rec<2> *>(sorted);
         l2 += exclusive_scan<uint64_t, LsdCnt<2>>(LsdCnt<2>{r, lsd.cnt}, dnew, n, static_cast<uint64_t *>(scan_scratch), nullptr, st);
         lsd_place_kernel<2><<<(unsigned)((n + 255) / 256), 256, 0, st>>>(r, n, dnew, ls, fin);
-        lsd_lists_kernel<2><<<(unsigned)((n * 8 + 255) / 256), 256, 0, st>>>(r, n, dnew, ls, o.stg_ids, fin);
-    }
-    if (prof) prof->end(on, l2 + 2, st);
-    return l + l2 + 2;
+    }
+    const unsigned grid_g = gather_grid(sm_count);
+    for (uint32_t c = 0; c < ch.n; c++)
+        gather3_kernel<<<grid_g, GA_THREADS, 0, st>>>(ch.totals_dev, ch.lsd_totals_dev, c, true, fin, o.stg_ids, static_cast<G3Counters *>(gc_dev));
+    if (prof) prof->end(on, l2 + 1 + (int)ch.n, st);
+    return l + l2 + 1 + (int)ch.n;
 }
 
 constexpr uint32_t PASS_TILE = 1u << 16;
diff --git a/genome-assembly_b200/csrc/capi.cu b/genome-assembly_b200/csrc/capi.cu
--- a/genome-assembly_b200/csrc/capi.cu
+++ b/genome-assembly_b200/csrc/capi.cu
@@ -110,7 +110,7 @@
     uint32_t chunk_bounds[SKR_MAX_CHUNKS + 1];
     uint32_t v3_tickets[2 * SKR_MAX_CHUNKS];
     unsigned long long lsd_totals[SKR_MAX_CHUNKS];
-    uint64_t v3_chunk_sum;
+    uint64_t v3_chunk_sum[2];
     uint32_t split_n_nl, split_n_reads;
     char last_byte;
     unsigned long long digest;
@@ -152,7 +152,7 @@
     DevBuf group_of, run_start, surv_index, id_offset, surv_group, bucket_of;
     DevBuf misc;
     DevBuf skr_a, skr_b, tile_state, inst_prefix, run_excl, skr_run_start, small_prefix, unit_base, units, unit_state, o_kmer_mmer, bucket_excl, big_list, big_k0, big_k1, big_arr, stg_ids, stg_codes, stg_mmer, stg_off, skr_side;
-    DevBuf ent_a, ent_b, piece_n, sorted_info, v3_base64, v3_head_run, v3_unit_out, v3_unit_excl, v3_atoms, v3_lsd_aux, v3_bitmap;
+    DevBuf ent_a, ent_b, piece_n, sorted_info, v3_base64, v3_head_run, v3_unit_out, v3_unit_excl, v3_atoms, v3_lsd_aux, v3_bitmap, v3_src_of, v3_tiles;
     DevBuf x_list_off, x_ids;
     void *donated = nullptr;
     uint64_t donated_bytes = 0;
@@ -675,7 +675,8 @@
     CU(ctx->v3_unit_out.ensure(max_units * v3_unit_out_bytes()));
     CU(ctx->v3_unit_excl.ensure((2 * max_units + 2) * 8));
     CU(ctx->scan_scratch.ensure(group_scan_scratch_bytes(n_runs + max_units + 1024)));
-    V3Chunks ch{1u, dm->v3_tickets, dm->chunk_bounds, &dm->v3_chunk_sum, dm->chunk_totals, dm->lsd_totals, nullptr, nullptr, nullptr};
+    CU(ctx->scan_scratch.ensure(v3_unit_scan_scratch_bytes(max_units)));
+    V3Chunks ch{1u, dm->v3_tickets, dm->chunk_bounds, dm->v3_chunk_sum, dm->chunk_totals, dm->lsd_totals, nullptr, nullptr, nullptr};
     ch.aux = ctx->st_aux;
     ch.ev_fork = ctx->ev_fork;
     ch.ev_join = ctx->ev_join;
@@ -702,9 +703,11 @@
     CU(ctx->stg_codes.ensure((kmer_cap * KW + 1) * sizeof(uint64_t)));
     CU(ctx->stg_mmer.ensure((kmer_cap + 1) * sizeof(uint32_t)));
     CU(ctx->stg_off.ensure((kmer_cap + 1) * sizeof(uint32_t)));
+    CU(ctx->v3_src_of.ensure((kmer_cap + 1) * sizeof(uint32_t)));
+    CU(ctx->v3_tiles.ensure(v3_tile_words(kmer_cap, n) * sizeof(uint32_t)));
     V3Out vo{ctx->o_kmer_codes.as<uint64_t>() + S_off * KW, ctx->o_kmer_mmer.as<uint32_t>() + S_off, ctx->o_kmer_id_off.as<uint64_t>() + S_off,
              ctx->o_read_ids.as<int32_t>() + N_off, kmer_cap, n, ctx->stg_codes.as<uint64_t>(), ctx->stg_mmer.as<uint32_t>(), ctx->stg_off.as<uint32_t>(),
-             ctx->stg_ids.as<int32_t>(), ctx->v3_unit_out.p, N_off};
+             ctx->stg_ids.as<int32_t>(), ctx->v3_unit_out.p, N_off, ctx->v3_src_of.as<uint32_t>(), ctx->v3_tiles.as<uint32_t>()};
     const size_t rb = sizeof(uint64_t) * KW + 8;
     auto lsd_arrays = [&](uint64_t cap) -> int {
         if (cap == 0) return GBIN_OK;
@@ -721,8 +724,8 @@
         uint32_t *aux = ctx->v3_lsd_aux.as<uint32_t>();
         return cap ? V3Lsd{ctx->rec_a.p, aux, aux + (cap + 1), aux + 2 * (cap + 1), aux + 3 * (cap + 1), cap} : V3Lsd{nullptr, nullptr, nullptr, nullptr, nullptr, 0};
     };
-    uint64_t *unit_excl = ctx->v3_unit_excl.as<uint64_t>(), *lsd_excl = unit_excl + max_units + 1;
-    lp = v3_group_launch(skr, ent, ctx->units.p, kl, ctx->v3_cap_eff, cutoff, d_ids, id_base, vo, max_units, unit_excl, lsd_excl, ctx->scan_scratch.p, &dm->gc3, ch,
+    void *unit_excl = ctx->v3_unit_excl.p;
+    lp = v3_group_launch(skr, ent, ctx->units.p, kl, ctx->v3_cap_eff, cutoff, d_ids, id_base, vo, max_units, unit_excl, ctx->scan_scratch.p, &dm->gc3, ch,
                          lsd_view(lsd_cap), false, ctx->sm_count, &ctx->prof, st);
     *launches += lp;
     CU(cudaGetLastError());
@@ -742,7 +745,7 @@
         V3Chunks ch1 = ch;
         ch1.totals_host = ch1.lsd_totals_host = nullptr;
         ch1.done = nullptr;
-        lp = v3_group_launch(skr, ent, ctx->units.p, kl, ctx->v3_cap_eff, cutoff, d_ids, id_base, vo, max_units, unit_excl, lsd_excl, ctx->scan_scratch.p, &dm->gc3, ch1,
+        lp = v3_group_launch(skr, ent, ctx->units.p, kl, ctx->v3_cap_eff, cutoff, d_ids, id_base, vo, max_units, unit_excl, ctx->scan_scratch.p, &dm->gc3, ch1,
                              lsd_view(lsd_cap), true, ctx->sm_count, &ctx->prof, st);
         *launches += lp;
         CU(cudaGetLastError());
@@ -750,6 +753,12 @@
     }
     ctx->rs.n_units += hm->gc3.n_units;
     ctx->rs.n_lsd_kmers += hm->gc3.lsd_kmers;
+    ctx->rs.n_kmers_plain += hm->gc3.placed[0];
+    ctx->rs.n_ids_plain += hm->gc3.placed[1];
+    ctx->rs.n_kmers_short += hm->gc3.placed[2];
+    ctx->rs.n_ids_short += hm->gc3.placed[3];
+    ctx->rs.n_kmers_long += hm->gc3.lsd_kmers;
+    ctx->rs.n_ids_long += hm->gc3.lsd_ids;
     if (hm->gc3.overflow) {
         snprintf(ctx->err, sizeof ctx->err, "pipeline 3 gave the batch up (code %u: a (bucket, d) class larger than a unit)", hm->gc3.overflow);
         return GBIN_OK;
@@ -759,8 +768,8 @@
         CU(ctx->radix_scratch.ensure(radix_scratch_bytes(nl)));
         CU(ctx->run_excl.ensure((nl + 2) * 8));
         CU(ctx->scan_scratch.ensure(group_scan_scratch_bytes(nl + 1024)));
-        lp = v3_lsd_finish(kl, nl, ctx->rec_a.p, ctx->rec_b.p, ctx->radix_scratch.p, ctx->run_excl.as<uint64_t>(), ctx->scan_scratch.p, vo, lsd_view(lsd_cap), ctx->sm_count, &ctx->prof,
-                           st);
+        lp = v3_lsd_finish(kl, nl, ctx->rec_a.p, ctx->rec_b.p, ctx->radix_scratch.p, ctx->run_excl.as<uint64_t>(), ctx->scan_scratch.p, vo, lsd_view(lsd_cap), ch,
+                           &dm->gc3, ctx->sm_count, &ctx->prof, st);
         *launches += lp;
         CU(cudaGetLastError());
     }
diff --git a/genome-assembly_b200/csrc/gbin_internal.h b/genome-assembly_b200/csrc/gbin_internal.h
--- a/genome-assembly_b200/csrc/gbin_internal.h
+++ b/genome-assembly_b200/csrc/gbin_internal.h
@@ -139,6 +139,7 @@
     unsigned long long distinct, total_kmers, total_ids;
     unsigned int overflow, n_units, n_spans, pad;
     unsigned long long lsd_kmers, lsd_ids;
+    unsigned long long placed[4];
 };
 int v3_plan_units(const uint16_t *sorted_info, const uint64_t *ent, const KeyLayout &kl, int cap, const uint32_t *inst_prefix, const uint32_t *run_start, uint64_t n_runs,
                   uint64_t *nunits64, uint64_t *base64, uint32_t *atom3, uint32_t *spanlen, uint32_t *head_run, void *scratch, void *units, uint64_t max_units,
@@ -155,7 +156,11 @@
     int32_t *stg_ids;
     void *unit_out;
     uint64_t id_off_base;
-};
+    uint32_t *src_of;
+    uint32_t *tiles;
+};
+size_t v3_tile_words(uint64_t kmer_cap, uint64_t id_cap);
+size_t v3_unit_scan_scratch_bytes(uint64_t max_units);
 struct V3Lsd {
     void *rec;
     uint32_t *src_off, *cnt, *fidx, *nadj;
@@ -175,10 +180,10 @@
 };
 size_t v3_group_smem_bytes(int KW, int cap);
 int v3_group_launch(const void *skr, const uint64_t *ent, const void *units, const KeyLayout &kl, int cap, int cutoff, const int32_t *ids_by_arrival, int32_t id_base,
-                    const V3Out &o, uint64_t max_units, uint64_t *unit_excl, uint64_t *lsd_excl, void *scan_scratch, void *gc_dev, const V3Chunks &ch, const V3Lsd &lsd,
+                    const V3Out &o, uint64_t max_units, void *unit_excl, void *scan_scratch, void *gc_dev, const V3Chunks &ch, const V3Lsd &lsd,
                     bool finalize_only, int sm_count, KernelProf *prof, cudaStream_t st);
 int v3_lsd_finish(const KeyLayout &kl, uint64_t n, void *rec_a, void *rec_b, void *radix_scratch, uint64_t *dnew, void *scan_scratch, const V3Out &o, const V3Lsd &lsd,
-                  int sm_count, KernelProf *prof, cudaStream_t st);
+                  const V3Chunks &ch, void *gc_dev, int sm_count, KernelProf *prof, cudaStream_t st);
 uint32_t v3_pass_tiles(uint64_t n_ent);
 uint32_t v3_pass_tile_entries();
 int v3_pass_tile_sums(const uint16_t *sorted_info, uint64_t n_ent, unsigned long long *sums_dev, cudaStream_t st);
diff --git a/genome-assembly_b200/csrc/prefix_scan.cuh b/genome-assembly_b200/csrc/prefix_scan.cuh
--- a/genome-assembly_b200/csrc/prefix_scan.cuh
+++ b/genome-assembly_b200/csrc/prefix_scan.cuh
@@ -7,6 +7,11 @@
 constexpr int SCAN_THREADS = 256;
 constexpr int SCAN_ITEMS = 16;
 constexpr int SCAN_TILE = SCAN_THREADS * SCAN_ITEMS;
+template <typename T>
+struct ScanTile {
+    static constexpr int ITEMS = sizeof(T) > 8 ? SCAN_ITEMS / 2 : SCAN_ITEMS;
+    static constexpr int TILE = SCAN_THREADS * ITEMS;
+};
 
 template <typename T>
 __device__ __forceinline__ T warp_inclusive_scan(T v) {
@@ -47,10 +52,11 @@
 
 template <typename TOut, typename InOp>
 __global__ void __launch_bounds__(SCAN_THREADS) scan_reduce_kernel(InOp in, TOut *__restrict__ block_sums, uint64_t n) {
-    const uint64_t base = (uint64_t)blockIdx.x * SCAN_TILE;
+    constexpr int ITEMS = ScanTile<TOut>::ITEMS, TILE = ScanTile<TOut>::TILE;
+    const uint64_t base = (uint64_t)blockIdx.x * TILE;
     TOut s = 0;
 #pragma unroll
-    for (int i = 0; i < SCAN_ITEMS; i++) {
+    for (int i = 0; i < ITEMS; i++) {
         const uint64_t j = base + (uint64_t)i * SCAN_THREADS + threadIdx.x;
         if (j < n) s += (TOut)in(j);
     }
@@ -62,33 +68,34 @@
 template <typename TOut, typename InOp>
 __global__ void __launch_bounds__(SCAN_THREADS)
     scan_apply_kernel(InOp in, TOut *__restrict__ out, const TOut *__restrict__ block_offsets, uint64_t n, TOut *__restrict__ total_out) {
-    __shared__ TOut ex[SCAN_TILE + SCAN_TILE / 16 + 1];
-    const uint64_t base = (uint64_t)blockIdx.x * SCAN_TILE;
+    constexpr int ITEMS = ScanTile<TOut>::ITEMS, TILE = ScanTile<TOut>::TILE;
+    __shared__ TOut ex[TILE + TILE / 16 + 1];
+    const uint64_t base = (uint64_t)blockIdx.x * TILE;
 #pragma unroll
-    for (int i = 0; i < SCAN_ITEMS; i++) {
+    for (int i = 0; i < ITEMS; i++) {
         const uint32_t p = (uint32_t)i * SCAN_THREADS + threadIdx.x;
         const uint64_t j = base + p;
         ex[scan_pad<TOut>(p)] = j < n ? (TOut)in(j) : TOut(0);
     }
     __syncthreads();
-    TOut v[SCAN_ITEMS];
+    TOut v[ITEMS];
     TOut s = 0;
 #pragma unroll
-    for (int i = 0; i < SCAN_ITEMS; i++) {
-        v[i] = ex[scan_pad<TOut>(threadIdx.x * SCAN_ITEMS + i)];
+    for (int i = 0; i < ITEMS; i++) {
+        v[i] = ex[scan_pad<TOut>(threadIdx.x * ITEMS + i)];
         s += v[i];
     }
     TOut total;
     TOut run = block_exclusive_scan<TOut>(s, &total) + (block_offsets ? block_offsets[blockIdx.x] : TOut(0));
 #pragma unroll
-    for (int i = 0; i < SCAN_ITEMS; i++) {
-        ex[scan_pad<TOut>(threadIdx.x * SCAN_ITEMS + i)] = run;
+    for (int i = 0; i < ITEMS; i++) {
+        ex[scan_pad<TOut>(threadIdx.x * ITEMS + i)] = run;
         run += v[i];
     }
     if (total_out && blockIdx.x == gridDim.x - 1 && threadIdx.x == SCAN_THREADS - 1) *total_out = run;
     __syncthreads();
 #pragma unroll
-    for (int i = 0; i < SCAN_ITEMS; i++) {
+    for (int i = 0; i < ITEMS; i++) {
         const uint32_t p = (uint32_t)i * SCAN_THREADS + threadIdx.x;
         const uint64_t j = base + p;
         if (j < n) out[j] = ex[scan_pad<TOut>(p)];
@@ -98,33 +105,34 @@
 template <typename TOut, typename InOp, typename OutOp>
 __global__ void __launch_bounds__(SCAN_THREADS)
     scan_apply_to_kernel(InOp in, OutOp out, const TOut *__restrict__ block_offsets, uint64_t n, TOut *__restrict__ total_out) {
-    __shared__ TOut ex[SCAN_TILE + SCAN_TILE / 16 + 1];
-    const uint64_t base = (uint64_t)blockIdx.x * SCAN_TILE;
+    constexpr int ITEMS = ScanTile<TOut>::ITEMS, TILE = ScanTile<TOut>::TILE;
+    __shared__ TOut ex[TILE + TILE / 16 + 1];
+    const uint64_t base = (uint64_t)blockIdx.x * TILE;
 #pragma unroll
-    for (int i = 0; i < SCAN_ITEMS; i++) {
+    for (int i = 0; i < ITEMS; i++) {
         const uint32_t p = (uint32_t)i * SCAN_THREADS + threadIdx.x;
         const uint64_t j = base + p;
         ex[scan_pad<TOut>(p)] = j < n ? (TOut)in(j) : TOut(0);
     }
     __syncthreads();
-    TOut v[SCAN_ITEMS];
+    TOut v[ITEMS];
     TOut s = 0;
 #pragma unroll
-    for (int i = 0; i < SCAN_ITEMS; i++) {
-        v[i] = ex[scan_pad<TOut>(threadIdx.x * SCAN_ITEMS + i)];
+    for (int i = 0; i < ITEMS; i++) {
+        v[i] = ex[scan_pad<TOut>(threadIdx.x * ITEMS + i)];
         s += v[i];
     }
     TOut total;
     TOut run = block_exclusive_scan<TOut>(s, &total) + (block_offsets ? block_offsets[blockIdx.x] : TOut(0));
 #pragma unroll
-    for (int i = 0; i < SCAN_ITEMS; i++) {
-        ex[scan_pad<TOut>(threadIdx.x * SCAN_ITEMS + i)] = run;
+    for (int i = 0; i < ITEMS; i++) {
+        ex[scan_pad<TOut>(threadIdx.x * ITEMS + i)] = run;
         run += v[i];
     }
     if (total_out && blockIdx.x == gridDim.x - 1 && threadIdx.x == SCAN_THREADS - 1) *total_out = run;
     __syncthreads();
 #pragma unroll
-    for (int i = 0; i < SCAN_ITEMS; i++) {
+    for (int i = 0; i < ITEMS; i++) {
         const uint32_t p = (uint32_t)i * SCAN_THREADS + threadIdx.x;
         const uint64_t j = base + p;
         if (j < n) out(j, ex[scan_pad<TOut>(p)]);
@@ -137,10 +145,12 @@
     __device__ __forceinline__ T operator()(uint64_t j) const { return p[j]; }
 };
 
+template <typename TOut = uint64_t>
 inline uint64_t scan_scratch_elems(uint64_t n) {
+    constexpr uint64_t TILE = ScanTile<TOut>::TILE;
     uint64_t tot = 0;
-    while (n > (uint64_t)SCAN_TILE) {
-        n = (n + SCAN_TILE - 1) / SCAN_TILE;
+    while (n > TILE) {
+        n = (n + TILE - 1) / TILE;
         tot += n;
     }
     return tot + 1;
@@ -152,7 +162,7 @@
         if (total_out) cudaMemsetAsync(total_out, 0, sizeof(TOut), st);
         return 0;
     }
-    const uint64_t blocks = (n + SCAN_TILE - 1) / SCAN_TILE;
+    const uint64_t blocks = (n + ScanTile<TOut>::TILE - 1) / ScanTile<TOut>::TILE;
     if (blocks == 1) {
         scan_apply_kernel<TOut, InOp><<<1, SCAN_THREADS, 0, st>>>(in, out, nullptr, n, total_out);
         return 1;
@@ -171,7 +181,7 @@
         if (total_out) cudaMemsetAsync(total_out, 0, sizeof(TOut), st);
         return 0;
     }
-    const uint64_t blocks = (n + SCAN_TILE - 1) / SCAN_TILE;
+    const uint64_t blocks = (n + ScanTile<TOut>::TILE - 1) / ScanTile<TOut>::TILE;
     if (blocks == 1) {
         scan_apply_to_kernel<TOut, InOp, OutOp><<<1, SCAN_THREADS, 0, st>>>(in, out, nullptr, n, total_out);
         return 1;
diff --git a/include/gbin.h b/include/gbin.h
--- a/include/gbin.h
+++ b/include/gbin.h
@@ -98,6 +98,8 @@
     uint32_t key_nc, key_h;
     uint32_t n_passes;
     uint32_t reserved;
+    uint64_t n_kmers_plain, n_kmers_short, n_kmers_long;
+    uint64_t n_ids_plain, n_ids_short, n_ids_long;
 } gbin_run_stats;
 int gbin_get_run_stats(const gbin_ctx *ctx, gbin_run_stats *out);
 int gbin_set_pipeline(gbin_ctx *ctx, int pipeline);
```

Measured after the change: 22.94 billion, median of 6. 1.9% lower.
